# abusch/rustracer

Hardware: AMD Instinct MI355X
Metric: Msamples/s (higher is better)
Workload: dtype f32; 1 GPU; cornell-box (synthetic S1, 32 triangles, 2 area lights) 1024x1024 PathIntegrator maxdepth=5 1024spp 02sequence box-filter; sampler_mode=pixel-keyed, light_distribution=cached across frames; first-frame build 18.3 ms

## Files before the change

include/rtx_hip.h:

```cpp
#ifndef RTX_HIP_H
#define RTX_HIP_H

#include <stdint.h>

#ifdef __cplusplus
extern "C" {
#endif

#define RT_OK 0
#define RT_ERR_INVALID (-1)
#define RT_ERR_NO_DEVICE (-2)
#define RT_ERR_HIP (-3)
#define RT_ERR_OOM (-4)
#define RT_ERR_UNSUPPORTED (-5)

typedef struct rt_bvh_node {
  float bmin[3];
  float bmax[3];
  uint32_t offset;
  uint16_t n_prims;
  uint8_t axis;
  uint8_t pad;
} rt_bvh_node;

// ... 98 lines not shown
  uint32_t n_materials; const rt_material* materials;
  uint32_t n_lights; const rt_light* lights;
  uint32_t n_instances; const rt_instance* instances;
  uint32_t n_top_nodes, n_top_prims;
  uint32_t n_unlisted_lights;
} rt_scene_desc;

typedef struct rt_camera {
  float raster_to_camera[16];
  float camera_to_world[16];
  float dx_camera[3], dy_camera[3];
  float lens_radius, focal_distance;
} rt_camera;
typedef struct rt_film_desc {
  int32_t cropped_pixel_bounds[4];
  int32_t sample_bounds[4];
  float filter_radius[2];
  float filter_table[256];
  float max_sample_luminance;
} rt_film_desc;
typedef struct rt_sampler_desc {
  int32_t spp;
  int32_t dimensions;
} rt_sampler_desc;
typedef struct rt_path_desc {
  int32_t max_depth;
  float rr_threshold;
  int32_t light_strategy;
  int32_t pixel_bounds[4];
} rt_path_desc;
typedef struct rt_shard { int32_t rank, world_size; } rt_shard;
#define RT_SHARD_ROWS(H, world_size) ((world_size) > 1 ? 4 : 16)

typedef struct rt_stats {
  uint64_t camera_rays;
  uint64_t rays_closest, rays_shadow, rays_mis;
  uint64_t nodes_closest, nodes_shadow, nodes_mis;
  uint64_t tris_closest, tris_shadow, tris_mis;
  uint64_t paths_scrubbed;
  double ms_total;
  double ms_sampler, ms_raygen, ms_trace_closest, ms_trace_any, ms_trace_mis, ms_shade, ms_resolve, ms_film, ms_lightdist;
  uint64_t launches_trace_closest;
  uint64_t n_passes;
  uint64_t vertices_lambert_const, vertices_lambert, vertices_two_lobe, vertices_generic;
  double ms_shade_lambert_const, ms_shade_lambert, ms_shade_two_lobe, ms_shade_generic, ms_shade_bin, ms_shade_miss;
  uint64_t shade_section_cycles[32];
  uint64_t rays_mis_any, nodes_mis_any, tris_mis_any;
  double ms_trace_mis_any;
  double ms_gather;
  uint64_t rays_mis_not_cast;
  uint64_t rays_tail_not_cast;
  uint64_t launches_trace_path, launches_trace_shadow, launches_trace_mis, launches_trace_mis_any, launches_shade;
  uint64_t rays_shadow_not_cast;
} rt_stats;

#define RT_FLAG_COUNT_TRAVERSAL 1u
#define RT_FLAG_FILM_ON_DEVICE 2u
#define RT_FLAG_TIME_KERNELS 4u
#define RT_FLAG_COUNT_AS_RENDERED 8u
#define RT_FLAG_REF_STREAM 16u
#define RT_FLAG_FRAME_STATS 32u

typedef struct rt_scene rt_scene;

int rt_scene_create(const rt_scene_desc* desc, int device, rt_scene** out);
void rt_scene_destroy(rt_scene* scene);

int rt_bvh_build(const float* tri_p, uint32_t n_tris, int32_t max_prims_per_node, rt_bvh_node* nodes, uint32_t* n_nodes, int32_t* ordered,
                 float* ms_device );

int rt_mip_build(const float* rgb, int32_t width, int32_t height, int32_t px, int32_t py, const int32_t* s_first, const float* s_wts, const int32_t* t_first,
                 const float* t_wts, int32_t wrap, int32_t n_levels, const int32_t* lvl_w, const int32_t* lvl_h, const uint64_t* lvl_off, float* texels_out);
int rt_env_distribution(const rt_image* image, int32_t width, int32_t height, int32_t mode, int32_t il, float delta, const float* sin_theta,
                        float* func, float* cdf, float* func_int, float* marg_cdf, float* marg_func_int);

int rt_render(rt_scene* scene, const rt_camera* camera, const rt_film_desc* film, const rt_sampler_desc* sampler,
              const rt_path_desc* path, const rt_shard* shard, uint32_t flags, void* stream, float* film_xyzw, rt_stats* stats);

typedef struct rt_multi rt_multi;
int rt_multi_create(const rt_scene_desc* desc, const int32_t* devices, int32_t n_devices, rt_multi** out);
void rt_multi_destroy(rt_multi* multi);
int rt_multi_render(rt_multi* multi, const rt_camera* camera, const rt_film_desc* film, const rt_sampler_desc* sampler, const rt_path_desc* path,
                    int32_t chunks_per_device, uint32_t flags, float* film_xyzw, rt_stats* total, rt_stats* per_device);

int rt_trace_closest(rt_scene* scene, const float* rays, uint64_t n, float* hits, uint64_t counters[2]);
int rt_trace_any(rt_scene* scene, const float* rays, uint64_t n, uint32_t* occluded, uint64_t counters[2]);
int rt_trace_closest_device(rt_scene* scene, const void* d_rays, uint64_t n, void* d_hits, int reps, void* stream, float* ms_per_launch);

int rt_sampler_tables(int32_t spp, int32_t dimensions, uint64_t pixel0, uint64_t n_pixels, uint32_t* scrambles, uint16_t* perms);
int rt_sampler_tables_plain(int32_t spp, int32_t dimensions, uint64_t pixel0, uint64_t n_pixels, uint32_t* scrambles, uint16_t* perms);

int rt_offset_ray_origin(const float* p, const float* p_error, const float* n, const float* w, uint64_t count, float* out);

int rt_fourier_eval(rt_scene* scene, int32_t material, uint64_t n, const float* wo, const float* wi, const float* u, float* out);

int rt_texture_eval(rt_scene* scene, int32_t texture, uint64_t n, const float* records, float* rgb_out);

enum { RT_BSDF_FRONT_AUTO = 0, RT_BSDF_FRONT_GENERIC = 1, RT_BSDF_FRONT_LAMBERT = 2, RT_BSDF_FRONT_TWO_LOBE = 3, RT_BSDF_FRONT_TWO_LOBE_WIDE = 4 };
#define RT_BSDF_SURFACE_FLOATS 40
#define RT_BSDF_OUT_FLOATS 13
int rt_bsdf_eval(rt_scene* scene, int32_t material, int32_t front_end, uint64_t n, const float* surface, const float* wo, const float* wi, const float* u,
                 float* out);

#define RT_SAMPLES_MAX 134217728
int rt_render_samples(rt_scene* scene, const rt_camera* camera, const rt_film_desc* film, const rt_sampler_desc* sampler, const rt_path_desc* path,
                      uint32_t flags, void* stream, float* radiance, float* p_film, rt_stats* stats);

enum { RT_FRAME_XYZW = 0, RT_FRAME_RGB = 1, RT_FRAME_RGB8 = 2, RT_FRAME_STATS = 3 };
enum { RT_FRAME_SAMPLES_DONE = 0, RT_FRAME_SPP = 1, RT_FRAME_TABLES_RESIDENT = 2, RT_FRAME_STATE_BYTES = 3, RT_FRAME_SAMPLES_TAKEN = 4, RT_FRAME_ACTIVE_PIXELS = 5 };
typedef struct rt_frame rt_frame;
int rt_frame_begin(rt_scene* scene, const rt_camera* camera, const rt_film_desc* film, const rt_sampler_desc* sampler, const rt_path_desc* path,
                   const rt_shard* shard , uint32_t flags, uint64_t table_budget_bytes, rt_frame** out);
int rt_frame_advance(rt_frame* frame, int32_t n_samples, void* stream, rt_stats* stats );
int rt_frame_advance_adaptive(rt_frame* frame, int32_t n_samples, float threshold, float floor_y, int32_t min_samples, void* stream, rt_stats* stats );
int rt_frame_read(rt_frame* frame, int32_t what, float scale, uint32_t flags, void* stream, void* out);
int rt_frame_query(rt_frame* frame, int32_t what, uint64_t* value);
void rt_frame_end(rt_frame* frame);

typedef struct rt_multi_frame rt_multi_frame;
int rt_multi_frame_begin(rt_multi* multi, const rt_camera* camera, const rt_film_desc* film, const rt_sampler_desc* sampler, const rt_path_desc* path,
                         uint32_t flags, uint64_t table_budget_bytes, rt_multi_frame** out);
int rt_multi_frame_advance(rt_multi_frame* frame, int32_t n_samples, rt_stats* total , rt_stats* per_device );
int rt_multi_frame_advance_adaptive(rt_multi_frame* frame, int32_t n_samples, float threshold, float floor_y, int32_t min_samples, rt_stats* total, rt_stats* per_device);
int rt_multi_frame_read(rt_multi_frame* frame, int32_t what, float scale, uint32_t flags, void* out);
int rt_multi_frame_query(rt_multi_frame* frame, int32_t what, uint64_t* value);
void rt_multi_frame_end(rt_multi_frame* frame);

int rt_light_distribution(rt_scene* scene, int32_t n_voxels[3], float* func, float* cdf, float* func_int);

enum { RT_QUERY_LDS_RESIDENT = 0, RT_QUERY_LDS_NODES_TESTED = 1 ,
       RT_QUERY_LDS_OCCLUSION = 2 ,
       RT_QUERY_SHADOW_PAIRS = 3 ,
       RT_QUERY_SHADOW_EMPTY = 4 ,
       RT_QUERY_BSDF_LAUNCHED = 5  };
int rt_scene_query(rt_scene* scene, int32_t what);
int rt_link_tables(const rt_scene_desc* desc, int32_t mid, uint32_t* link_kept, uint32_t* link_full, uint64_t capacity_words, double* stats);
int rt_shadow_sets(const rt_scene_desc* desc, uint32_t* words, uint64_t capacity_words, int32_t n_voxels[3], uint64_t* stats);
int rt_sizeof(const char* struct_name);

const char* rt_last_error(void);
int rt_device_available(void);
const char* rt_version(void);

#ifdef __cplusplus
}
#endif
#endif
```

include/rtx_host.h:

```cpp
#ifndef RTX_HOST_H
#define RTX_HOST_H
#include <stdint.h>
#include "rtx_hip.h"

#ifdef __cplusplus
extern "C" {
#endif

typedef struct rtxh_scene rtxh_scene;

typedef struct rtxh_render_params {
  int32_t xres, yres;
  float crop[4];
  int32_t filter_kind;
  float filter_params[4];
  float film_scale, max_sample_luminance;
  float cam_to_world[16], cam_to_world_inv[16];
  float fov, lens_radius, focal_distance;
  int32_t spp, sampler_dims;
  int32_t max_depth; float rr_threshold; int32_t light_strategy;
  int32_t pixel_bounds[4];
  int32_t rank, world_size;
  uint32_t flags;
  float screen_window[4];
// ... 25 lines not shown
int rtxh_scene_add_texture_mapped(rtxh_scene*, int32_t kind, const float* value3, int32_t tex1, int32_t tex2, int32_t amount, const float* words, int32_t n_words);
int rtxh_texture_words(rtxh_scene*, int32_t texture, float* out, int32_t capacity);
int rtxh_scene_add_material(rtxh_scene*, int32_t kind, const int32_t* slots16, int32_t remap_roughness, int32_t bump_texture );
int rtxh_scene_add_light(rtxh_scene*, int32_t kind, int32_t tri, const float* rgb3, int32_t two_sided, const float* vec3, int32_t mip,
                         const float* l2w16, const float* w2l16);
int rtxh_scene_commit(rtxh_scene*, int32_t max_prims_per_node);
int rtxh_scene_commit_device_bvh(rtxh_scene*, int32_t max_prims_per_node, float* ms_device);
int rtxh_scene_upload(rtxh_scene*, int32_t device);

int rtxh_scene_bvh_sizes(rtxh_scene*, int32_t* n_nodes, int32_t* n_prims);
int rtxh_scene_bvh_get(rtxh_scene*, float* bounds6, uint32_t* offset, uint16_t* n_prims, uint8_t* axis, int32_t* ordered);
int rtxh_camera_film_setup(const rtxh_render_params*, float* raster_to_camera16, float* dxdy6, float* filter_table256, int32_t* sample_bounds4,
                           int32_t* cropped4);
int rtxh_mip_level(rtxh_scene*, int32_t mip, int32_t level, int32_t* w, int32_t* h, float* rgb_out );
enum { RTXH_TABLE_TEXTURES = 0, RTXH_TABLE_MATERIALS, RTXH_TABLE_LIGHTS, RTXH_TABLE_P, RTXH_TABLE_N, RTXH_TABLE_UV, RTXH_TABLE_S, RTXH_TABLE_INDICES,
       RTXH_TABLE_TRI_MATERIAL, RTXH_TABLE_TRI_LIGHT, RTXH_TABLE_TRI_FLAGS,
       RTXH_TABLE_ENV_FUNC, RTXH_TABLE_ENV_CDF, RTXH_TABLE_ENV_ROW_INT, RTXH_TABLE_ENV_MARG_CDF,
       RTXH_TABLE_INSTANCES,
       RTXH_TABLE_EMITTERS,
       RTXH_TABLE_QUADRICS,
       RTXH_TABLE_OBJECT_BASE = 1000 ,
       RTXH_TABLE_OBJECT_EXTRA_BASE = 100000  };
typedef struct rtxh_emitter_info { float rgb[3]; int32_t two_sided; } rtxh_emitter_info;
typedef struct rtxh_instance_info { int32_t object; float o2w[16], w2o[16]; } rtxh_instance_info;
typedef struct rtxh_light_info { int32_t kind, tri; float rgb[3]; int32_t two_sided; float vec[3]; int32_t mip; float l2w[12], w2l[12]; } rtxh_light_info;
int rtxh_scene_inspect(rtxh_scene*, int32_t table, void* out, uint64_t capacity_bytes, uint64_t* n_items);
int rtxh_look_at(const float* pos, const float* look, const float* up, float* m16, float* m_inv16);

int rtxh_render(rtxh_scene*, const rtxh_render_params*, void* hip_stream, float* film_xyzw, rt_stats* stats);
int rtxh_render_samples(rtxh_scene*, const rtxh_render_params*, void* hip_stream, float* radiance, float* p_film, rt_stats* stats);
typedef struct rtxh_frame rtxh_frame;
int rtxh_frame_begin(rtxh_scene*, const rtxh_render_params*, uint64_t table_budget_bytes, rtxh_frame** out);
int rtxh_frame_advance(rtxh_frame*, int32_t n_samples, void* hip_stream, rt_stats* stats );
int rtxh_frame_advance_adaptive(rtxh_frame*, int32_t n_samples, float threshold, float floor_y, int32_t min_samples, void* hip_stream, rt_stats* stats );
int rtxh_frame_read(rtxh_frame*, int32_t what, float scale, uint32_t flags, void* hip_stream, void* out);
int rtxh_frame_query(rtxh_frame*, int32_t what, uint64_t* value);
void rtxh_frame_end(rtxh_frame*);
int rtxh_render_multi(rtxh_scene*, const rtxh_render_params*, const int32_t* devices, int32_t n_devices, int32_t chunks_per_device, float* film_xyzw,
                      rt_stats* total, rt_stats* per_device );
typedef struct rtxh_multi_frame rtxh_multi_frame;
int rtxh_multi_frame_begin(rtxh_scene*, const rtxh_render_params*, const int32_t* devices, int32_t n_devices, uint64_t table_budget_bytes, rtxh_multi_frame** out);
int rtxh_multi_frame_advance(rtxh_multi_frame*, int32_t n_samples, rt_stats* total, rt_stats* per_device);
int rtxh_multi_frame_advance_adaptive(rtxh_multi_frame*, int32_t n_samples, float threshold, float floor_y, int32_t min_samples, rt_stats* total, rt_stats* per_device);
int rtxh_multi_frame_read(rtxh_multi_frame*, int32_t what, float scale, uint32_t flags, void* out);
int rtxh_multi_frame_query(rtxh_multi_frame*, int32_t what, uint64_t* value);
void rtxh_multi_frame_end(rtxh_multi_frame*);
int rtxh_trace(rtxh_scene*, const float* rays, uint64_t n, int32_t any_hit, float* hits4_or_occ, uint64_t counters[2]);
int rtxh_trace_device(rtxh_scene*, const void* d_rays, uint64_t n, void* d_hits, int32_t reps, void* hip_stream, float* ms_per_launch);
int rtxh_light_distribution(rtxh_scene*, int32_t n_voxels[3], float* func, float* cdf, float* func_int);
int rtxh_scene_query(rtxh_scene*, int32_t what);
int rtxh_scene_device(rtxh_scene*, rt_scene** out);
int rtxh_scene_link_tables(rtxh_scene*, int32_t mid, uint32_t* link_kept, uint32_t* link_full, uint64_t capacity_words, double* stats);
int rtxh_scene_shadow_sets(rtxh_scene*, uint32_t* words, uint64_t capacity_words, int32_t n_voxels[3], uint64_t* stats);
int rtxh_sizeof(const char* struct_name);
const char* rtxh_last_error(void);

typedef struct rtxh_ply {
  int32_t n_verts, n_tris;
  float* P;
  float* N;
  float* UV;
  int32_t* idx;
  int32_t n_dropped_faces;
} rtxh_ply;
int rtxh_ply_read(const char* path, rtxh_ply* out);
void rtxh_ply_free(rtxh_ply* ply);
int rtxh_pfm_read(const char* path, int32_t* width, int32_t* height, float** rgb);
void rtxh_free(void* p);
int rtxh_image_read(const char* path, int32_t* width, int32_t* height, float** rgb);

int rtxh_spectrum_from_sampled(const float* lambda_nm, const float* values, int32_t n, float rgb[3]);
int rtxh_spectrum_blackbody(float temperature_kelvin, float scale, float rgb[3]);
void rtxh_copper(float eta_rgb[3], float k_rgb[3]);

typedef struct rtxh_pbrt_result {
  rtxh_scene* scene;
  rtxh_render_params params;
  int32_t max_prims_per_node;
  int32_t n_warnings;
  char film_filename[512];
} rtxh_pbrt_result;
int rtxh_pbrt_load(const char* path, rtxh_pbrt_result* out);
int rtxh_pbrt_parse(const char* text, const char* base_dir, rtxh_pbrt_result* out);
int rtxh_pbrt_tokens(const char* text, char* out, uint64_t capacity);

#ifdef __cplusplus
}
#endif
#endif
```

rustracer_amd/csrc/rtx_hip.hip:

```cpp
#include <hip/hip_runtime.h>
#include <chrono>
#include <cmath>
#include <cstdio>
#include <cstring>
#include <string>
#include <vector>
#include <limits>
#include <algorithm>
#include <memory>
#include <atomic>
#include <mutex>
#include <thread>

#include "../../include/rtx_hip.h"
#include "rtx_kernels.h"
#include "rtx_shade_launch.h"
#include "rtx_ref_launch.h"

using namespace rtx;
#include "rtx_scene_plan.h"

static thread_local std::string g_err;
static int fail(int code, const std::string& msg) { g_err = msg; return code; }
static bool env_is(const char* name, char c) { const char* e = getenv(name); return e && e[0] == c; }
// ... 10 lines not shown
  hipError_t ensure(size_t n) {
    if (n <= bytes && p) return hipSuccess;
    if (p) { (void)hipFree(p); p = nullptr; bytes = 0; }
    hipError_t e = hipMalloc(&p, n > 0 ? n : 16);
    if (e == hipSuccess) bytes = n;
    return e;
  }
  void release() { if (p) (void)hipFree(p); p = nullptr; bytes = 0; }
  template <class T> T* as() const { return (T*)p; }
};

struct SamplerPlan {
  unsigned spp = 0, dims = 0, seg_len = 0, n_segs = 0;
  DevBuf segs, magic, dirty, partners;
};

struct rt_scene {
  int device = 0;
  SamplerPlan sampler_plan;
  DScene d{};
  bool small = false;
  bool lambert_materials = false;
  bool lds_records_q = false;
  bool lds_tables = false;
  bool lds_mats = false;
  bool lds_records = false;
  bool lambert_only = false;
  bool lean_qlights = false;
  bool lean_shade = false;
  int stack_depth = 64;
  unsigned n_nodes = 0, n_tris = 0; int n_lights = 0;
  DevBuf link8, link8_full; unsigned lds_nodes_tested = 0;
  DevBuf pairs, tmin_stack;
  DevBuf top_pairs, deep_stack; bool use_top = false;
  bool top_for_closest = false;
  bool use_pairs = false;
  bool deep_column = false;
  DevBuf quads; bool use_quads = false; int quad_stack_depth = 0;
  DevBuf tri_rec;
  DevBuf nodes, tri_p, tri_n, tri_uv, tri_s, tri_alpha, spheres, textures, images, materials, lights, texels, dist, guides, prim_class;
  DevBuf fourier;
  std::vector<int> mat_kind, mat_table;
  std::vector<uint64_t> fourier_at;
  bool has_spheres = false;
  bool has_instances = false;
  DevBuf instances;
  bool mid = false;
  bool general_prims = false;
  bool obj_general = false;
  bool has_masks = false;
  bool masked_emitters = false;
  DevBuf ld_func, ld_cdf, ld_int, ld_mark, ld_list, ld_slot, ld_guide, ld_rows8, ld_dense8;
  bool shadow_sets = false; RtShadowSets shadow; DevBuf ld_shadow;
  DevBuf self;
  int ld_strategy_built = -1; bool ld_all_voxels = false;
  std::mutex render_mutex;
  DevBuf ws[32];
  DevBuf film_acc, own_acc, film_out, counters, stats, filter_table, ref_samples, ref_stack;
  DevBuf samples_rad, samples_pf;
  DevBuf bsdf_self, bsdf_tris;
  int bsdf_launched = -1;
  std::vector<int> mat_class;
  DevBuf bin_words, bin_sorted, bin_at;
  unsigned n_materials = 0, n_code_classes = 0, n_lambert_classes = 0, n_small_classes = 0, n_wide_classes = 0;
  DevBuf scrambles[2], perms[2];
  hipStream_t aux_stream = nullptr;
  hipEvent_t ev_tables[2][3] = {{nullptr, nullptr, nullptr}, {nullptr, nullptr, nullptr}}, ev_batch_done[2] = {nullptr, nullptr}, ev_frame_begin = nullptr;
  int n_cu = 256;
  std::vector<hipEvent_t> event_pool;
  ~rt_scene() {
    for (hipEvent_t e : event_pool) (void)hipEventDestroy(e);
    for (int i = 0; i < 2; ++i) { for (int g = 0; g < 3; ++g) if (ev_tables[i][g]) (void)hipEventDestroy(ev_tables[i][g]); if (ev_batch_done[i]) (void)hipEventDestroy(ev_batch_done[i]); }
    if (ev_frame_begin) (void)hipEventDestroy(ev_frame_begin);
    if (aux_stream) (void)hipStreamDestroy(aux_stream);
  }
};

extern "C" const char* rt_last_error(void) { return g_err.c_str(); }
extern "C" const char* rt_version(void) { return "rtx-mi355x 0.5 (gfx950 wavefront path tracer)"; }
extern "C" int rt_sizeof(const char* name) {
  if (!name) return -1;
#define RT_SZ(T) if (!strcmp(name, #T)) return (int)sizeof(T);
  RT_SZ(rt_bvh_node) RT_SZ(rt_tri_meta) RT_SZ(rt_sphere) RT_SZ(rt_instance) RT_SZ(rt_texture) RT_SZ(rt_image) RT_SZ(rt_material) RT_SZ(rt_light) RT_SZ(rt_scene_desc)
  RT_SZ(rt_camera) RT_SZ(rt_film_desc) RT_SZ(rt_sampler_desc) RT_SZ(rt_path_desc) RT_SZ(rt_shard) RT_SZ(rt_stats)
#undef RT_SZ
  return -1;
}
extern "C" int rt_device_available(void) {
  int n = 0;
  if (hipGetDeviceCount(&n) != hipSuccess || n <= 0) return 0;
  return 1;
}

static int upload(DevBuf& b, const void* src, size_t bytes) {
  HIP_TRY(b.ensure(bytes));
  if (bytes) HIP_TRY(hipMemcpy(b.p, src, bytes, hipMemcpyHostToDevice));
  return RT_OK;
}

static void fill_ewa_lut() {
  float lut[128];
  for (int i = 0; i < 128; ++i) {
    float alpha = 2.0f;
    float r2 = (float)i / (128.0f - 1.0f);
    lut[i] = expf(-alpha * r2) - expf(-alpha);
  }
// ... 150 lines not shown
  scene->bsdf_launched = 2 * mode + (const_tex ? 1 : 0);
  HIP_TRY(hipMemcpy(out, b[3].p, no, hipMemcpyDeviceToHost));
  return RT_OK;
}
extern "C" int rt_link_tables(const rt_scene_desc* desc, int32_t mid, uint32_t* link_kept, uint32_t* link_full, uint64_t capacity_words, double* stats) {
  if (!desc || !desc->nodes || desc->n_nodes == 0 || !desc->tri_p || !desc->tri_meta || !link_kept || !link_full) return fail(RT_ERR_INVALID, "null argument");
  const size_t words = (size_t)9 * desc->n_nodes + 9;
  if (desc->n_nodes > (mid ? RT_MID_NODES : RT_SMALL_NODES) || desc->n_tris > (uint64_t)(mid ? RT_MID_TRIS : RT_SMALL_TRIS) || desc->n_instances != 0) return fail(RT_ERR_INVALID, "not an LDS-sized scene");
  if (capacity_words < words) return fail(RT_ERR_INVALID, "link table capacity too small");
  {
    const uint32_t nn = desc->n_nodes;
    std::vector<uint32_t> size(nn, 1u);
    for (uint32_t i = nn; i-- > 0;) {
      const rt_bvh_node& n = desc->nodes[i];
      if (n.n_prims != 0) {
        if ((uint64_t)n.offset + n.n_prims > desc->n_tris) return fail(RT_ERR_INVALID, "leaf range out of bounds");
        if (n.n_prims >= (1u << (15 - RT_LINK_OFF_BITS(mid ? RT_MID_NODES : RT_SMALL_NODES)))) return fail(RT_ERR_INVALID, "a leaf holds more primitives than a link word can name");
        continue;
      }
      if (i + 1 >= nn || n.offset != i + 1 + size[i + 1] || n.offset >= nn) return fail(RT_ERR_INVALID, "nodes are not a pre-order tree");
      size[i] = 1u + size[i + 1] + size[n.offset];
    }
    if (size[0] != nn) return fail(RT_ERR_INVALID, "nodes are not one tree");
    for (uint64_t t = 0; t < desc->n_tris; ++t)
      if (desc->tri_meta[t].flags & RT_PRIM_SPHERE) {
        uint32_t k; memcpy(&k, desc->tri_p + 9 * t + 6, 4);
        if (!desc->spheres || k >= desc->n_spheres) return fail(RT_ERR_INVALID, "sphere index out of range");
      }
  }
  RtLinkTables lt;
  rt_build_link_tables(desc, mid != 0, stats != nullptr, lt);
  memcpy(link_kept, lt.link_kept.data(), words * 4); memcpy(link_full, lt.link_full.data(), words * 4);
  if (stats) for (int w = 0; w < 9; ++w) { stats[w] = (double)lt.n_rays[w]; stats[9 + w] = lt.tests_all[w]; stats[18 + w] = lt.tests_kept[w]; }
  return RT_OK;
}
extern "C" int rt_shadow_sets(const rt_scene_desc* desc, uint32_t* words, uint64_t capacity_words, int32_t n_voxels[3], uint64_t* stats) {
  if (!desc || !desc->nodes || desc->n_nodes == 0 || !desc->tri_p || !desc->tri_meta) return fail(RT_ERR_INVALID, "null argument");
  bool plain = desc->n_instances == 0 && desc->n_spheres == 0 && desc->n_nodes <= RT_SMALL_NODES && desc->n_tris <= RT_SMALL_TRIS;
  for (uint32_t i = 0; i < desc->n_tris && plain; ++i) if (desc->tri_meta[i].flags & ~(uint32_t)RT_SHADOW_PLAIN_FLAGS) plain = false;
  if (!shadow_sets_apply(desc, plain)) return fail(RT_ERR_INVALID, "not a scene the shadow sets serve (LDS-resident plain triangles, two triangle lights)");
  int32_t lp[2] = {0, 0};
  for (uint32_t k = 0; k < desc->n_lights; ++k) lp[k] = desc->lights[k].prim;
  RtShadowSets ss;
  rt_build_shadow_sets(desc->tri_p, desc->n_tris, lp, (int)desc->n_lights, desc->nodes[0].bmin, desc->nodes[0].bmax, ss);
  if (n_voxels) { n_voxels[0] = ss.nvox[0]; n_voxels[1] = ss.nvox[1]; n_voxels[2] = ss.nvox[2]; }
  if (stats) { stats[0] = ss.pairs; stats[1] = ss.empty; }
  if (words) {
    if (capacity_words < ss.word.size()) return fail(RT_ERR_INVALID, "rt_shadow_sets: capacity too small");
    std::memcpy(words, ss.word.data(), ss.word.size() * 4);
  }
  return RT_OK;
}

extern "C" int rt_scene_query(rt_scene* s, int32_t what) {
  if (!s) return fail(RT_ERR_INVALID, "null scene");
  if (what == RT_QUERY_LDS_RESIDENT) return s->small ? 1 : 0;
  if (what == RT_QUERY_LDS_NODES_TESTED) return (s->small || s->mid) ? (int)s->lds_nodes_tested : 0;
  if (what == RT_QUERY_LDS_OCCLUSION) return s->mid ? 1 : 0;
  if (what == RT_QUERY_SHADOW_PAIRS) return s->shadow_sets ? (int)s->shadow.pairs : 0;
  if (what == RT_QUERY_SHADOW_EMPTY) return s->shadow_sets ? (int)s->shadow.empty : 0;
  if (what == RT_QUERY_BSDF_LAUNCHED) return s->bsdf_launched < 0 ? 0 : s->bsdf_launched + 1;
  return fail(RT_ERR_INVALID, "unknown rt_scene_query item");
}

static int build_light_distribution(rt_scene* s, int strategy, hipStream_t stream, bool all_voxels = false) {
  DScene& d = s->d;
  if (s->ld_strategy_built == strategy && (s->ld_all_voxels || !all_voxels)) return RT_OK;
  s->ld_strategy_built = -1;
  const int nl = s->n_lights;
  size_t ld_rows_built = 1;
  const bool uniform = strategy == 1 || nl == 1 || nl == 0;
  int glog = -1;
  if (nl >= 64 && nl <= 65534) { const long q = guide_quarters(); glog = 0; while (glog < 16 && (long)(2 << glog) * q <= 4l * nl) ++glog; }
  d.ld_glog = glog; d.ld_guide = nullptr;
  if (uniform) {
    const int n = nl > 0 ? nl : 1;
    std::vector<float> func(n, 1.0f), cdf(n + 1, 0.0f);
    for (int i = 1; i < n + 1; ++i) cdf[i] = cdf[i - 1] + func[i - 1] / (float)n;
    float func_int = cdf[n];
    if (func_int == 0.0f) for (int i = 1; i < n + 1; ++i) cdf[i] = (float)i / (float)n;
    else for (int i = 1; i < n + 1; ++i) cdf[i] /= func_int;
    int rc;
    if ((rc = upload(s->ld_func, func.data(), func.size() * 4)) != RT_OK) return rc;
    if ((rc = upload(s->ld_cdf, cdf.data(), cdf.size() * 4)) != RT_OK) return rc;
    if ((rc = upload(s->ld_int, &func_int, 4)) != RT_OK) return rc;
    if (glog >= 0) {
      const int G = 1 << glog; std::vector<unsigned short> g((size_t)G + 1); int i = 0;
      for (int k = 0; k <= G; ++k) { const float x = (float)k / (float)G; while (i <= n && cdf[i] <= x) ++i; g[k] = (unsigned short)i; }
      if ((rc = upload(s->ld_guide, g.data(), g.size() * 2)) != RT_OK) return rc;
    }
    d.ld_uniform = 1; d.nvox[0] = d.nvox[1] = d.nvox[2] = 1;
  } else {
    float diag[3] = {d.wb_max.x - d.wb_min.x, d.wb_max.y - d.wb_min.y, d.wb_max.z - d.wb_min.z};
    int ext = diag[0] > diag[1] ? (diag[0] > diag[2] ? 0 : 2) : (diag[1] > diag[2] ? 1 : 2);
    float b_max = diag[ext];
    size_t total = 1;
    for (int i = 0; i < 3; ++i) {
      float r = roundf(diag[i] / b_max * 64.0f);
      unsigned v = (r != r || r <= 0.0f) ? 0u : (unsigned)r;
      d.nvox[i] = (int)(v > 1u ? v : 1u);
      total *= (size_t)d.nvox[i];
    }
    d.ld_uniform = 0;
    HIP_TRY(s->ld_mark.ensure(total)); HIP_TRY(s->ld_list.ensure((total + 1) * 4)); HIP_TRY(s->ld_slot.ensure(total * 4));
    unsigned* n_list = s->ld_list.as<unsigned>(); unsigned* list = n_list + 1;
    HIP_TRY(hipMemsetAsync(s->ld_slot.p, 0xff, total * 4, stream));
    if (all_voxels) hipLaunchKernelGGL(k_lightdist_iota, dim3((unsigned)((total + 255) / 256)), dim3(256), 0, stream, (unsigned)total, list, n_list);
    else {
      HIP_TRY(hipMemsetAsync(s->ld_mark.p, 0, total, stream)); HIP_TRY(hipMemsetAsync(n_list, 0, 4, stream));
      hipLaunchKernelGGL(k_lightdist_mark, dim3((s->n_tris + 255u) / 256u), dim3(256), 0, stream, d, s->ld_mark.as<unsigned char>());
      hipLaunchKernelGGL(k_lightdist_compact, dim3((unsigned)((total + 255) / 256)), dim3(256), 0, stream, s->ld_mark.as<unsigned char>(), (unsigned)total, 0, list, n_list);
    }
    unsigned n_built = 0;
    HIP_TRY(hipMemcpyAsync(&n_built, n_list, 4, hipMemcpyDeviceToHost, stream)); HIP_TRY(hipStreamSynchronize(stream));
    const size_t rows = std::max<size_t>(n_built, 1);
    ld_rows_built = rows;
    if (s->ld_func.ensure(rows * nl * 4) != hipSuccess || s->ld_cdf.ensure(rows * (nl + 1) * 4) != hipSuccess || s->ld_int.ensure(rows * 4) != hipSuccess)
      return fail(RT_ERR_OOM, "light distribution tables do not fit (built voxels x lights)");
    if (glog >= 0 && s->ld_guide.ensure(rows * (((size_t)1 << glog) + 1) * 2) != hipSuccess) return fail(RT_ERR_OOM, "light distribution guide tables do not fit");
    d.ld_func = s->ld_func.as<float>(); d.ld_cdf = s->ld_cdf.as<float>(); d.ld_int = s->ld_int.as<float>(); d.ld_slot = s->ld_slot.as<int>();
    unsigned lights_pad = 1; while (lights_pad < (unsigned)nl) lights_pad <<= 1;
    const unsigned long long contrib_blocks = lights_pad <= 128u ? (rows + 128u / lights_pad - 1) / (128u / lights_pad) : (unsigned long long)rows * (unsigned)((nl + 127) / 128);
    if (contrib_blocks > 0x7fffffffull) return fail(RT_ERR_INVALID, "light distribution grid too large");
    if (s->has_spheres) hipLaunchKernelGGL(k_lightdist_contrib<true>, dim3((unsigned)contrib_blocks), dim3(128), 0, stream, d, list, n_list, lights_pad, (unsigned)((nl + 127) / 128), s->ld_func.as<float>());
    else hipLaunchKernelGGL(k_lightdist_contrib<false>, dim3((unsigned)contrib_blocks), dim3(128), 0, stream, d, list, n_list, lights_pad, (unsigned)((nl + 127) / 128), s->ld_func.as<float>());
    hipLaunchKernelGGL(k_lightdist_finish, dim3((unsigned)((rows + 127) / 128)), dim3(128), 0, stream, d, list, n_list, s->ld_func.as<float>(), s->ld_cdf.as<float>(), s->ld_int.as<float>(), s->ld_slot.as<int>(),
                       glog >= 0 ? s->ld_guide.as<unsigned short>() : nullptr, glog);
    HIP_TRY(hipGetLastError());
  }
  d.ld_func = s->ld_func.as<float>(); d.ld_cdf = s->ld_cdf.as<float>(); d.ld_int = s->ld_int.as<float>(); d.ld_slot = s->ld_slot.as<int>();
  d.ld_guide = glog >= 0 ? s->ld_guide.as<unsigned short>() : nullptr;
  d.ld_rows8 = nullptr; d.ld_dense8 = nullptr;
  if (nl >= 1 && nl <= 3 && !(env_is("RTX_LD_ROWS8", '0'))) {
    const size_t n_rows = ld_rows_built;
    HIP_TRY(s->ld_rows8.ensure(n_rows * 32));
    hipLaunchKernelGGL(k_lightdist_rows8, dim3((unsigned)((n_rows + 255) / 256)), dim3(256), 0, stream, s->ld_func.as<float>(), s->ld_cdf.as<float>(), s->ld_int.as<float>(), (int)nl, (unsigned)n_rows, s->ld_rows8.as<float4>());
    HIP_TRY(hipGetLastError());
    d.ld_rows8 = s->ld_rows8.as<float4>();
    const unsigned long long n_vox = (unsigned long long)d.nvox[0] * d.nvox[1] * d.nvox[2];
    const int dense_mb = env_int("RTX_LD_DENSE_MB", 16);
    if (!uniform && n_vox * 32ull <= (unsigned long long)dense_mb << 20) {
      HIP_TRY(s->ld_dense8.ensure((size_t)n_vox * 32));
      hipLaunchKernelGGL(k_lightdist_dense8, dim3((unsigned)((n_vox + 255) / 256)), dim3(256), 0, stream, s->ld_rows8.as<float4>(), s->ld_slot.as<int>(), n_vox, s->ld_dense8.as<float4>());
      HIP_TRY(hipGetLastError());
      d.ld_dense8 = s->ld_dense8.as<float4>();
    }
  }
  if (d.ld_rows8 != nullptr && !uniform && s->shadow_sets && nl == 2 && d.nvox[0] == s->shadow.nvox[0] && d.nvox[1] == s->shadow.nvox[1] && d.nvox[2] == s->shadow.nvox[2]) {
    const unsigned long long n_vox = (unsigned long long)d.nvox[0] * d.nvox[1] * d.nvox[2];
    int rc = upload(s->ld_shadow, s->shadow.word.data(), s->shadow.word.size() * 4);
    if (rc != RT_OK) return rc;
    hipLaunchKernelGGL(k_lightdist_shadow_words, dim3((unsigned)((n_vox + 255) / 256)), dim3(256), 0, stream, s->ld_shadow.as<unsigned>(), s->ld_slot.as<int>(), n_vox, s->ld_rows8.as<float4>(),
                       d.ld_dense8 != nullptr ? s->ld_dense8.as<float4>() : nullptr);
    HIP_TRY(hipGetLastError());
  }
  s->ld_strategy_built = strategy; s->ld_all_voxels = all_voxels;
  HIP_TRY(hipMemcpyAsync(s->self.p, &s->d, sizeof(DScene), hipMemcpyHostToDevice, stream));
  return RT_OK;
}

extern "C" int rt_light_distribution(rt_scene* s, int32_t n_voxels[3], float* func, float* cdf, float* func_int) {
  if (!s) return fail(RT_ERR_INVALID, "null scene");
  HIP_TRY(hipSetDevice(s->device));
  int rc = build_light_distribution(s, 0, nullptr, true);
  if (rc != RT_OK) return rc;
  HIP_TRY(hipDeviceSynchronize());
  if (s->d.ld_uniform) { n_voxels[0] = n_voxels[1] = n_voxels[2] = 0; return RT_OK; }
  n_voxels[0] = s->d.nvox[0]; n_voxels[1] = s->d.nvox[1]; n_voxels[2] = s->d.nvox[2];
  size_t total = (size_t)s->d.nvox[0] * s->d.nvox[1] * s->d.nvox[2];
  if (func) HIP_TRY(hipMemcpy(func, s->ld_func.p, total * s->n_lights * 4, hipMemcpyDeviceToHost));
  if (cdf) HIP_TRY(hipMemcpy(cdf, s->ld_cdf.p, total * (s->n_lights + 1) * 4, hipMemcpyDeviceToHost));
  if (func_int) HIP_TRY(hipMemcpy(func_int, s->ld_int.p, total * 4, hipMemcpyDeviceToHost));
  return RT_OK;
}

template <bool ANY, bool SMALL, int BLOCK, int DEPTH>
static unsigned trace_grid(const rt_scene* s, bool links = false) {
  unsigned lds = (unsigned)(DEPTH * BLOCK * (SMALL ? 2 : 4) + (SMALL ? (8 * RT_SMALL_NODES + 10 * RT_SMALL_TRIS) * 4 : 32));
  unsigned waves = 8;
  if (SMALL && links) { lds = (unsigned)((8 * RT_SMALL_NODES + 10 * RT_SMALL_TRIS) * 4 + (ANY ? 1 : 8) * RT_SMALL_NODES * 4 + 32); waves = ANY ? RT_LDS_ANY_WAVES : RT_LDS_TRACE_WAVES; }
  unsigned per_cu = (160u * 1024u) / lds; if (per_cu * BLOCK > waves * 256u) per_cu = waves * 256u / BLOCK; if (per_cu < 1) per_cu = 1;
  return (unsigned)s->n_cu * per_cu;
}
#define RT_TOP_BLOCK 512
static unsigned top_grid(const rt_scene* s, bool any = false) {
  (void)any;
  const unsigned fit = (160u * 1024u) / (16384u + (unsigned)RT_TOP_LDS_DEPTH * RT_TOP_BLOCK * 4u);
  return (unsigned)s->n_cu * std::max(1u, std::min(3u, fit));
}
static size_t tmin_stack_bytes(const rt_scene* s) {
  if (s->small || !s->use_pairs) return 0;
  const size_t a = s->stack_depth <= 32 ? (size_t)trace_grid<false, false, 128, 32>(s) * 128 * 32 * 4 : (size_t)trace_grid<false, false, 128, 64>(s) * 128 * 64 * 4;
  const size_t b = s->use_top ? (size_t)std::max(top_grid(s), top_grid(s, true)) * RT_TOP_BLOCK * (size_t)s->stack_depth * 4 : 0;
  return std::max(a, b);
}
static size_t deep_stack_bytes(const rt_scene* s) {
  if (!s->use_top) return 0;
  return (size_t)std::max(top_grid(s), top_grid(s, true)) * RT_TOP_BLOCK * (size_t)std::max(1, s->stack_depth - RT_TOP_LDS_DEPTH) * 4;
}
static int scene_from_plan(const RtScenePlan& p, const rt_scene_desc* desc, int device, rt_scene** out) {
  if (device >= 0) HIP_TRY(hipSetDevice(device));
  int dev = 0; HIP_TRY(hipGetDevice(&dev));
  std::unique_ptr<rt_scene> owner(new rt_scene());
  rt_scene* s = owner.get();
  s->device = dev;
  hipDeviceProp_t prop; if (hipGetDeviceProperties(&prop, dev) == hipSuccess) s->n_cu = prop.multiProcessorCount;
  s->n_nodes = desc->n_nodes; s->n_tris = desc->n_tris; s->n_lights = (int)desc->n_lights; s->n_materials = desc->n_materials;
  s->small = p.small; s->mid = p.mid; s->general_prims = p.general_prims; s->obj_general = p.obj_general; s->has_masks = p.has_masks; s->has_spheres = p.has_spheres;
  s->has_instances = p.has_instances; s->masked_emitters = p.masked_emitters; s->lambert_only = p.lambert_only; s->lambert_materials = p.lambert_materials;
  s->lean_shade = p.lean_shade; s->lean_qlights = p.lean_qlights; s->lds_records = p.lds_records; s->lds_records_q = p.lds_records_q; s->lds_tables = p.lds_tables;
  s->lds_mats = p.lds_mats; s->use_pairs = p.use_pairs; s->use_top = p.use_top; s->top_for_closest = p.top_for_closest; s->use_quads = p.use_quads;
  s->deep_column = p.deep_column; s->shadow_sets = p.shadow_sets; s->shadow = p.shadow; s->stack_depth = p.stack_depth; s->quad_stack_depth = p.quad_stack_depth;
  s->mat_kind = p.mat_kind; s->mat_table = p.mat_table; s->mat_class = p.mat_class; s->fourier_at = p.fourier_at;
  s->n_code_classes = p.n_code_classes; s->n_lambert_classes = p.n_lambert_classes; s->n_small_classes = p.n_small_classes; s->n_wide_classes = p.n_wide_classes;
  if (s->mid) {
    int fit_any = 0, fit_closest = 0;
    if (hipOccupancyMaxActiveBlocksPerMultiprocessor(&fit_any, (const void*)(k_trace<true, false, 1024, 16, 0, 1>), 1024, 0) != hipSuccess) fit_any = 0;
    if (hipOccupancyMaxActiveBlocksPerMultiprocessor(&fit_closest, (const void*)(k_trace<false, false, 1024, 16, 0, 1>), 1024, 0) != hipSuccess) fit_closest = 0;
    (void)hipGetLastError();
    if (fit_any < 1 || fit_closest < 1) s->mid = false;
  }
  const bool links = s->small || s->mid;
  if (links) s->lds_nodes_tested = p.links.nodes_tested;
  int rc = RT_OK;
  auto up = [&rc](DevBuf& b, const void* src, size_t bytes) { if (rc == RT_OK) rc = upload(b, src, bytes); };
  auto up_all = [&up](DevBuf& b, const auto& v) { up(b, v.data(), v.size() * sizeof(v[0])); };
  auto room = [&rc](DevBuf& b, size_t bytes, const char* what) { if (rc == RT_OK && bytes && b.ensure(bytes) != hipSuccess) rc = fail(RT_ERR_OOM, what); };
  up(s->nodes, desc->nodes, sizeof(rt_bvh_node) * (size_t)desc->n_nodes);
  up_all(s->tri_p, p.tri_p);
  if (desc->tri_n) up(s->tri_n, desc->tri_n, (size_t)desc->n_tris * 36);
  if (desc->tri_uv) up(s->tri_uv, desc->tri_uv, (size_t)desc->n_tris * 24);
  if (desc->tri_s) up(s->tri_s, desc->tri_s, (size_t)desc->n_tris * 36);
  if (p.has_masks) up(s->tri_alpha, desc->tri_alpha, (size_t)desc->n_tris * 8);
  if (p.has_spheres) up(s->spheres, desc->spheres, (size_t)desc->n_spheres * sizeof(rt_sphere));
  if (p.has_instances) up_all(s->instances, p.instances);
  up_all(s->texels, p.texels); up_all(s->fourier, p.fourier);
  std::vector<DImage> images = p.images;
  for (DImage& im : images) im.texels = s->texels.as<float4>();
  up_all(s->images, images); up_all(s->textures, p.textures); up_all(s->materials, p.materials); up_all(s->prim_class, p.prim_class);
  up_all(s->dist, p.dist); up_all(s->guides, p.guides);
  std::vector<DLight> lights = p.lights;
  for (DLight& l : lights)
    if (l.kind == RT_LIGHT_INFINITE) {
      rt_blob_rebase(l.cf, s->dist.p); rt_blob_rebase(l.func_int, s->dist.p); rt_blob_rebase(l.mfunc, s->dist.p); rt_blob_rebase(l.mcdf, s->dist.p);
      rt_blob_rebase(l.guide, s->guides.p); rt_blob_rebase(l.mguide, s->guides.p);
    }
  up_all(s->lights, lights);
  if (links) { up_all(s->link8_full, p.links.link_full); up_all(s->link8, p.links.link_kept); }
  if (p.use_pairs) up_all(s->pairs, p.pairs);
  if (p.use_top) up_all(s->top_pairs, p.top_pairs);
  if (p.use_quads) up_all(s->quads, p.quads);
  room(s->tmin_stack, tmin_stack_bytes(s), "traversal stack allocation failed");
  room(s->deep_stack, deep_stack_bytes(s), "traversal stack allocation failed");
  room(s->tri_rec, (size_t)desc->n_tris * 128, "shade record allocation failed");
  room(s->self, sizeof(DScene), "scene record allocation failed");
  if (rc != RT_OK) return rc;
  DScene& d = s->d;
  d.nodes = s->nodes.as<float4>(); d.n_nodes = desc->n_nodes;
  d.tri_p = s->tri_p.as<float4>(); d.n_tris = desc->n_tris;
  d.tri_n = s->tri_n.as<float>(); d.tri_uv = s->tri_uv.as<float>(); d.tri_s = s->tri_s.as<float>();
  d.tri_alpha = s->tri_alpha.as<int2>();
  d.spheres = s->spheres.as<DSphere>();
  d.instances = s->instances.as<DInstance>(); d.n_instances = s->has_instances ? desc->n_instances : 0u; d.n_top_prims = p.n_top_prims;
  d.textures = s->textures.as<DTexture>(); d.images = s->images.as<DImage>(); d.materials = s->materials.as<DMaterial>(); d.lights = s->lights.as<DLight>();
  d.fourier = s->fourier.as<unsigned>();
// ... 128 lines not shown
  }
  if (s->small) {
    if (s->stack_depth <= 16) hipLaunchKernelGGL((k_trace<ANY, true, 256, 16>), dim3(trace_grid<ANY, true, 256, 16>(s)), dim3(256), 0, stream, RT_KARGS, st_nodes, st_tris);
    else if (s->stack_depth <= 32) hipLaunchKernelGGL((k_trace<ANY, true, 256, 32>), dim3(trace_grid<ANY, true, 256, 32>(s)), dim3(256), 0, stream, RT_KARGS, st_nodes, st_tris);
    else hipLaunchKernelGGL((k_trace<ANY, true, 128, 64>), dim3(trace_grid<ANY, true, 128, 64>(s)), dim3(128), 0, stream, RT_KARGS, st_nodes, st_tris);
  } else {
    if (s->stack_depth <= 32) launch_trace_hbm<ANY, COUNT, 128, 32>(RT_ARGS);
    else launch_trace_hbm<ANY, COUNT, 128, 64>(RT_ARGS);
  }
#undef RT_KARGS
#undef RT_ARGS
}
template <bool ANY>
static void launch_trace(rt_scene* s, bool count, const TraceIO& io, const unsigned* queue, const unsigned* count_ptr, unsigned shard_cap, unsigned count_static,
                         unsigned long long* stats, int st_rays, int st_nodes, int st_tris, hipStream_t stream) {
  if (count) launch_trace_c<ANY, true>(s, io, queue, count_ptr, shard_cap, count_static, stats, st_rays, st_nodes, st_tris, stream);
  else launch_trace_c<ANY, false>(s, io, queue, count_ptr, shard_cap, count_static, stats, st_rays, st_nodes, st_tris, stream);
}
static TraceIO trace_io_planar(const float4* ro, const float4* rd, float4* hits, unsigned* occ) {
  TraceIO io{}; io.ray_o = ro; io.ray_d = rd; io.ray_stride = 1; io.hits = hits; io.hit_stride = 1; io.hit_b2 = 0; io.occluded = occ; io.occ_stride = 1;
  io.shadow_masks = 1;
  return io;
}

static int trace_batch(rt_scene* s, const float* rays, uint64_t n, bool any, float* hits, uint32_t* occluded, uint64_t counters[2]) {
  if (!s || !rays || n == 0 || n > 0x7fffffffull) return fail(RT_ERR_INVALID, "bad trace batch");
  HIP_TRY(hipSetDevice(s->device));
  DevBuf ro, rd, out, st;
  HIP_TRY(ro.ensure(n * 16)); HIP_TRY(rd.ensure(n * 16)); HIP_TRY(out.ensure(n * 16)); HIP_TRY(st.ensure(ST_COUNT * 8));
  std::vector<float> o(n * 4), d(n * 4);
  for (uint64_t i = 0; i < n; ++i) {
    const float* r = rays + 8 * i;
    o[4 * i] = r[0]; o[4 * i + 1] = r[1]; o[4 * i + 2] = r[2]; o[4 * i + 3] = r[3];
    d[4 * i] = r[4]; d[4 * i + 1] = r[5]; d[4 * i + 2] = r[6]; d[4 * i + 3] = 0.0f;
  }
  HIP_TRY(hipMemcpy(ro.p, o.data(), n * 16, hipMemcpyHostToDevice));
  HIP_TRY(hipMemcpy(rd.p, d.data(), n * 16, hipMemcpyHostToDevice));
  HIP_TRY(hipMemset(st.p, 0, ST_COUNT * 8));
  const TraceIO io = trace_io_planar(ro.as<float4>(), rd.as<float4>(), any ? nullptr : out.as<float4>(), any ? out.as<unsigned>() : nullptr);
  if (any) launch_trace<true>(s, counters != nullptr, io, nullptr, nullptr, 0, (unsigned)n, st.as<unsigned long long>(), ST_RAYS_SHADOW, ST_NODES_SHADOW, ST_TRIS_SHADOW, nullptr);
  else launch_trace<false>(s, counters != nullptr, io, nullptr, nullptr, 0, (unsigned)n, st.as<unsigned long long>(), ST_RAYS_CLOSEST, ST_NODES_CLOSEST, ST_TRIS_CLOSEST, nullptr);
  HIP_TRY(hipGetLastError());
  HIP_TRY(hipDeviceSynchronize());
  if (any) HIP_TRY(hipMemcpy(occluded, out.p, n * 4, hipMemcpyDeviceToHost));
  else HIP_TRY(hipMemcpy(hits, out.p, n * 16, hipMemcpyDeviceToHost));
  if (counters) {
    unsigned long long h[ST_COUNT];
    HIP_TRY(hipMemcpy(h, st.p, sizeof(h), hipMemcpyDeviceToHost));
    counters[0] = any ? h[ST_NODES_SHADOW] : h[ST_NODES_CLOSEST];
    counters[1] = any ? h[ST_TRIS_SHADOW] : h[ST_TRIS_CLOSEST];
  }
  return RT_OK;
}
extern "C" int rt_trace_closest(rt_scene* s, const float* rays, uint64_t n, float* hits, uint64_t counters[2]) { return trace_batch(s, rays, n, false, hits, nullptr, counters); }
extern "C" int rt_trace_any(rt_scene* s, const float* rays, uint64_t n, uint32_t* occluded, uint64_t counters[2]) { return trace_batch(s, rays, n, true, nullptr, occluded, counters); }

extern "C" int rt_trace_closest_device(rt_scene* s, const void* d_rays, uint64_t n, void* d_hits, int reps, void* stream_, float* ms_per_launch) {
  if (!s || !d_rays || !d_hits || n == 0 || reps <= 0) return fail(RT_ERR_INVALID, "bad arguments");
  HIP_TRY(hipSetDevice(s->device));
  hipStream_t stream = (hipStream_t)stream_;
  const float4* ro = (const float4*)d_rays; const float4* rd = ro + n;
  hipEvent_t e0, e1; HIP_TRY(hipEventCreate(&e0)); HIP_TRY(hipEventCreate(&e1));
  HIP_TRY(hipEventRecord(e0, stream));
  const TraceIO io = trace_io_planar(ro, rd, (float4*)d_hits, nullptr);
  for (int i = 0; i < reps; ++i) launch_trace<false>(s, false, io, nullptr, nullptr, 0, (unsigned)n, nullptr, 0, 0, 0, stream);
  HIP_TRY(hipEventRecord(e1, stream));
  HIP_TRY(hipEventSynchronize(e1));
  float ms = 0; HIP_TRY(hipEventElapsedTime(&ms, e0, e1));
  if (ms_per_launch) *ms_per_launch = ms / (float)reps;
  (void)hipEventDestroy(e0); (void)hipEventDestroy(e1);
  return RT_OK;
}

static unsigned next_pow2(unsigned v) { unsigned p = 1; while (p < v) p <<= 1; return p; }
static unsigned sampler_lanes_per_block(unsigned spp) {
  unsigned l = (32u * 1024u) / ((spp + 2u) * 2u);
  if (l >= 64u) return 64u;
  if (l >= 32u) return 32u;
  if (l >= 16u) return 16u;
  if (l >= 8u) return 8u;
  return 4u;
}

static void pcg_advance_constants(unsigned long long n, unsigned long long& mul, unsigned long long& sum) {
  unsigned long long cur_mul = 0x5851f42d4c957f2dULL, cur_sum = 1ull;
  mul = 1ull; sum = 0ull;
  while (n) {
    if (n & 1ull) { sum = sum * cur_mul + cur_sum; mul *= cur_mul; }
    cur_sum = (cur_mul + 1ull) * cur_sum; cur_mul *= cur_mul;
    n >>= 1;
  }
}
static int sampler_plan_prepare(SamplerPlan& pl, unsigned spp_, unsigned dims_) {
  unsigned &spp = pl.spp, &dims = pl.dims, &seg_len = pl.seg_len, &n_segs = pl.n_segs;
  DevBuf &segs = pl.segs, &magic = pl.magic, &dirty = pl.dirty;
  {
    if (spp == spp_ && dims == dims_ && segs.p) return RT_OK;
    seg_len = spp_ < 256u ? spp_ : 256u;
    const unsigned per_half = spp_ / seg_len;
    std::vector<SamplerSeg> h;
    unsigned long long pos = 0;
    for (unsigned t = 0; t < 2u * dims_; ++t) {
      const unsigned n_scr = t < dims_ ? 1u : 2u;
      for (unsigned half = 0; half < 2u; ++half)
        for (unsigned g = 0; g < per_half; ++g) {
          SamplerSeg sg{};
// ... 303 lines not shown
      else { want.push_back({&s->samples_rad, (size_t)n_window_samples * 16}); if (samples_pf) want.push_back({&s->samples_pf, (size_t)n_window_samples * 8}); }
    }
    size_t grow = 0;
    for (const Want& w : want) if (!w.buf->p || w.buf->bytes < w.bytes) grow += w.bytes;
    size_t held = 0;
    for (const Want& w : want) if (w.buf->p && w.buf->bytes < w.bytes) held += w.buf->bytes;
    size_t mem_free = 0, mem_total = 0;
    HIP_TRY(hipMemGetInfo(&mem_free, &mem_total));
    if (grow > mem_free + held - std::min<size_t>(mem_free + held, (size_t)256 << 20)) continue;
    bool ok = true;
    for (const Want& w : want) if (w.buf->ensure(w.bytes) != hipSuccess) { ok = false; break; }
    if (ok) break;
    (void)hipGetLastError();
  }
  if (!s->aux_stream) {
    int lo = 0, hi = 0; (void)hipDeviceGetStreamPriorityRange(&lo, &hi);
    HIP_TRY(hipStreamCreateWithPriority(&s->aux_stream, hipStreamNonBlocking, lo));
    for (int i = 0; i < 2; ++i) { for (int g = 0; g < 3; ++g) HIP_TRY(hipEventCreateWithFlags(&s->ev_tables[i][g], hipEventDisableTiming)); HIP_TRY(hipEventCreateWithFlags(&s->ev_batch_done[i], hipEventDisableTiming)); }
    HIP_TRY(hipEventCreateWithFlags(&s->ev_frame_begin, hipEventDisableTiming));
  }
  float4* const d_out = (flags & RT_FLAG_FILM_ON_DEVICE) ? (float4*)film_xyzw : s->film_out.as<float4>();
  float4* const d_samples_rad = (flags & RT_FLAG_FILM_ON_DEVICE) ? (float4*)samples_rad : s->samples_rad.as<float4>();
  float2* const d_samples_pf = !samples_pf ? nullptr : ((flags & RT_FLAG_FILM_ON_DEVICE) ? (float2*)samples_pf : s->samples_pf.as<float2>());
  if (!samples && !fr) {
    HIP_TRY(hipMemcpyAsync(s->filter_table.p, film->filter_table, 1024, hipMemcpyHostToDevice, stream));
    HIP_TRY(hipMemsetAsync(s->film_acc.p, 0, (size_t)cw * ch * 16, stream));
  }
  HIP_TRY(hipMemsetAsync(s->stats.p, 0, ST_COUNT * 8, stream));

  PassState ps{};
  ps.spp = spp; ps.spp_log2 = spp_log2; ps.dims = dims;
  auto gen_of = [&](int b) { PathGen g; char* p = (char*)s->ws[b].p; g.o = (float4*)p; g.d = (float4*)(p + n_slots * 16); g.beta = (float4*)(p + n_slots * 32); g.st = (uint4*)(p + n_slots * 48); return g; };
  const PathGen gen0 = gen_of(B_GEN0), gen1 = gen_of(B_GEN1);
  ps.hit = s->ws[B_HIT].as<float4>(); ps.lacc = s->ws[B_LACC].as<float4>(); ps.pfilm = s->ws[B_PFILM].as<float2>();
  { char* p = (char*)s->ws[B_SH].p; ps.sh.o = (float4*)p; ps.sh.d = (float4*)(p + cap * 16); ps.sh.add = (float4*)(p + cap * 32);
    char* q = (char*)s->ws[B_MI].p; ps.mi.o = (float4*)q; ps.mi.d = (float4*)(q + cap * 16); ps.mi.hit = (float4*)(q + cap * 32); ps.mi.a = (float4*)(q + cap * 48);
    ps.mi.b = (float4*)(q + cap * 64); ps.mi.c = (float4*)(q + cap * 80); ps.mi.flags = (unsigned*)(q + cap * 96); }
  ps.occ_sh = s->ws[B_OCCSH].as<unsigned char>(); ps.occ_mi = s->ws[B_OCCMI].as<unsigned char>();
  ps.q_shadow = s->ws[B_QSH].as<unsigned>(); ps.q_mis = s->ws[B_QMI].as<unsigned>(); ps.q_misany = s->ws[B_QMA].as<unsigned>();
  ps.own_acc = s->own_acc.as<float4>(); ps.shard_cap = shard_cap;
  ps.stats = s->stats.as<unsigned long long>();

  if ((rc = sampler_plan_prepare(s->sampler_plan, spp, dims)) != RT_OK) return rc;
  if ((rc = sampler_set_lds_limits(spp)) != RT_OK) return rc;
  TraceIO io_path{}, io_shadow{}, io_mis{}, io_mis_any{};
  {
    io_path.ray_stride = 1; io_path.hits = ps.hit; io_path.hit_stride = 1; io_path.hit_b2 = 1; io_path.queue_is_slots = 1;
    io_shadow.ray_o = ps.sh.o; io_shadow.ray_d = ps.sh.d; io_shadow.ray_stride = 1; io_shadow.occluded = (unsigned*)ps.occ_sh; io_shadow.occ_stride = 0;
    io_shadow.shadow_masks = 1; io_shadow.lacc = ps.lacc; io_shadow.lacc_stride = 1; io_shadow.direct_add = ps.sh.add; io_shadow.add_stride = 1;
    io_mis.ray_o = ps.mi.o; io_mis.ray_d = ps.mi.d; io_mis.ray_stride = 1; io_mis.hits = ps.mi.hit; io_mis.hit_stride = 1; io_mis.hit_b2 = 0;
    io_mis_any = io_mis; io_mis_any.shadow_masks = 0; io_mis_any.hits = nullptr; io_mis_any.occluded = (unsigned*)ps.occ_mi; io_mis_any.occ_stride = 0;
  }
  const bool count = (flags & RT_FLAG_COUNT_TRAVERSAL) != 0;
  const unsigned pgrid = (unsigned)s->n_cu * 8u;
  const unsigned sblock = 256u, sgrid = pgrid;
  unsigned long long* dstats = s->stats.as<unsigned long long>();

  const char* ov = getenv("RTX_K0_OVERLAP");
  hipStream_t aux = (ov && ov[0] == '0') ? stream : s->aux_stream;
  if (build_tables) {
    HIP_TRY(hipEventRecord(s->ev_frame_begin, stream));
    HIP_TRY(hipStreamWaitEvent(aux, s->ev_frame_begin, 0));
  }
  int tables_rc = RT_OK;
  std::vector<std::pair<unsigned long long, unsigned long long>> batches;
  for (unsigned long long first = 0; first < owned_pixels;) {
    const unsigned long long npx = (first == 0 && lead_pixels) ? lead_pixels : std::min(chunk_pixels, owned_pixels - first);
    batches.push_back({first, npx}); first += npx;
  }
  if (resident && !fr->tables_built) {
    fr->scr_off.clear(); fr->perm_off.clear();
    size_t so = 0, po = 0;
    for (const auto& b : batches) {
      fr->scr_off.push_back(so); fr->perm_off.push_back(po);
      so += ((size_t)b.second * 3 * dims * 4 + 255) & ~(size_t)255; po += ((size_t)(b.second * table_bytes_per_pixel) + 255) & ~(size_t)255;
    }
    if (so > fr->scrambles.bytes || po > fr->perms.bytes) return fail(RT_ERR_INVALID, "rt_frame_advance: the batches' sampler tables do not fit the frame's buffers");
  }
  if (resident && fr->scr_off.size() != batches.size()) return fail(RT_ERR_INVALID, "rt_frame_advance: the batch cut changed under resident sampler tables");
  auto scrambles_of = [&](size_t b, int buf) { return resident ? (unsigned*)((char*)fr->scrambles.p + fr->scr_off[b]) : s->scrambles[buf].as<unsigned>(); };
  auto perms_of = [&](size_t b, int buf) { return resident ? (unsigned short*)((char*)fr->perms.p + fr->perm_off[b]) : s->perms[buf].as<unsigned short>(); };
  TableGroups tgroups = table_groups_frame(dims, !(fp.lens_radius > 0.0f));
  auto launch_tables = [&](size_t b, int buf) {
    FrameParams f2 = fp; f2.chunk_first = batches[b].first;
    tm.begin(&stats.ms_sampler, aux);
    const int trc = launch_sampler_tables(s->sampler_plan, f2, (unsigned)batches[b].second, 0ull, 0, scrambles_of(b, buf), perms_of(b, buf), aux, tgroups, s->ev_tables[buf]);
    if (trc != RT_OK && tables_rc == RT_OK) tables_rc = trc;
    tm.end(aux);
  };
  if (!batches.empty() && build_tables) launch_tables(0, 0);
  for (size_t batch_no = 0; batch_no < batches.size(); ++batch_no) {
    const unsigned long long first = batches[batch_no].first, npx = batches[batch_no].second;
    const int buf = (int)(batch_no & 1ull);
    fp.chunk_first = first;
    ps.n_pixels = (unsigned)npx; ps.n_pixels_recip = npx > 1 ? (unsigned)((1ull << 32) / npx) : 0xffffffffu;
    ps.scrambles = scrambles_of(batch_no, buf); ps.perms = perms_of(batch_no, buf);
    if (build_tables && batch_no + 1 < batches.size()) {
      if (batch_no >= 1 && !resident) HIP_TRY(hipStreamWaitEvent(aux, s->ev_batch_done[buf ^ 1], 0));
      launch_tables(batch_no + 1, buf ^ 1);
    }
    const unsigned batch_pass_samples = (unsigned)std::min<unsigned long long>(spp, std::max<unsigned long long>(pass_samples, cap / npx));
    if (tables_rc != RT_OK) { (void)hipDeviceSynchronize(); return tables_rc; }
    if (build_tables) HIP_TRY(hipStreamWaitEvent(stream, s->ev_tables[buf][0], 0));
    for (unsigned s0 = s_begin; s0 < s_end; s0 += batch_pass_samples) {
      ps.s0 = s0; ps.n_samples = std::min(batch_pass_samples, s_end - s0); ps.cap = (unsigned)(npx * ps.n_samples);
      ps.q_in = nullptr; ps.in = gen1; ps.out = gen0;
// ... 56 lines not shown
        tm.end();
        tm.begin(&stats.ms_trace_mis);
        launch_trace<false>(s, count, io_mis, ps.q_mis, ps.cnt_out + 2 * RT_QSHARDS * RT_CNT_STRIDE, ps.shard_cap, 0, dstats, ST_RAYS_MIS, ST_NODES_MIS, ST_TRIS_MIS, stream);
        tm.end();
        if (ps.mis_any) {
          tm.begin(&stats.ms_trace_mis_any);
          launch_trace<true>(s, count, io_mis_any, ps.q_misany, ps.cnt_out + 3 * RT_QSHARDS * RT_CNT_STRIDE, ps.shard_cap, 0, dstats, ST_RAYS_MISANY, ST_NODES_MISANY, ST_TRIS_MISANY, stream);
          tm.end();
        }
        tm.begin(&stats.ms_resolve);
        if (s->has_spheres || s->has_instances) hipLaunchKernelGGL(k_resolve<true>, dim3(pgrid), dim3(256), 0, stream, s->d, ps);
        else hipLaunchKernelGGL(k_resolve<false>, dim3(pgrid), dim3(256), 0, stream, s->d, ps);
        tm.end();
        stats.launches_trace_closest += 2; stats.launches_trace_path += 1; stats.launches_trace_mis += 1; stats.launches_trace_shadow += 1; stats.launches_trace_mis_any += ps.mis_any ? 1 : 0;
      }
      tm.begin(&stats.ms_film);
      if (samples) hipLaunchKernelGGL(k_sample_store, dim3(pgrid), dim3(256), 0, stream, fp, ps, wx0, wy0, wx1 - wx0, d_samples_rad, d_samples_pf);
      else if (fr && fr->stats) hipLaunchKernelGGL(k_film_accumulate_frame_stats, dim3(pgrid), dim3(256), 0, stream, fp, ps, fr->filter_table.as<float>(), fr->film_acc.as<float4>(), fr->own_acc.as<float4>(), fr->moments.as<PixMoments>());
      else if (fr) hipLaunchKernelGGL(k_film_accumulate_frame, dim3(pgrid), dim3(256), 0, stream, fp, ps, fr->filter_table.as<float>(), fr->film_acc.as<float4>(), fr->own_acc.as<float4>());
      else hipLaunchKernelGGL(k_film_accumulate, dim3(pgrid), dim3(256), 0, stream, fp, ps, s->filter_table.as<float>(), s->film_acc.as<float4>());
      tm.end();
      stats.n_passes += 1;
      HIP_TRY(hipGetLastError());
    }
    HIP_TRY(hipEventRecord(s->ev_batch_done[buf], stream));
  }
  if (fr) {
    if (resident && build_tables) {
      HIP_TRY(hipStreamSynchronize(aux));
      fr->tables_built = true; fr->batch_pixels = batch_pixels; fr->lead_pixels = lead_pixels;
    }
  } else if (!samples) {
    tm.begin(&stats.ms_film);
    {
      unsigned long long n = (unsigned long long)cw * ch;
      hipLaunchKernelGGL(k_film_finalize, dim3((unsigned)((n + 255) / 256)), dim3(256), 0, stream, s->film_acc.as<float4>(), d_out, n);
    }
    tm.end();
    HIP_TRY(hipGetLastError());
    if (!(flags & RT_FLAG_FILM_ON_DEVICE)) HIP_TRY(hipMemcpyAsync(film_xyzw, d_out, (size_t)cw * ch * 16, hipMemcpyDeviceToHost, stream));
  } else if (!(flags & RT_FLAG_FILM_ON_DEVICE)) {
    HIP_TRY(hipMemcpyAsync(samples_rad, d_samples_rad, (size_t)n_window_samples * 16, hipMemcpyDeviceToHost, stream));
    if (samples_pf) HIP_TRY(hipMemcpyAsync(samples_pf, d_samples_pf, (size_t)n_window_samples * 8, hipMemcpyDeviceToHost, stream));
  }
  HIP_TRY(hipStreamSynchronize(stream));
  tm.collect();
  stats.ms_shade = stats.ms_shade_lambert_const + stats.ms_shade_lambert + stats.ms_shade_two_lobe + stats.ms_shade_generic + stats.ms_shade_bin + stats.ms_shade_miss;
  unsigned long long h[ST_COUNT];
  HIP_TRY(hipMemcpy(h, s->stats.p, sizeof(h), hipMemcpyDeviceToHost));
  { unsigned ovf = 0; HIP_TRY(hipMemcpy(&ovf, s->sampler_plan.dirty.as<unsigned>() + 1 + RT_DIRTY_CAP, 4, hipMemcpyDeviceToHost));
    if (ovf) { (void)hipMemset(s->sampler_plan.dirty.p, 0, (2 + RT_DIRTY_CAP) * 4); return fail(RT_ERR_INVALID, "sampler retry list overflow"); } }
  stats.camera_rays = h[ST_CAMERA];
  stats.rays_mis_any = h[ST_RAYS_MISANY]; stats.nodes_mis_any = h[ST_NODES_MISANY]; stats.tris_mis_any = h[ST_TRIS_MISANY];
  stats.rays_closest = h[ST_RAYS_CLOSEST] + h[ST_TAIL_UNCAST]; stats.rays_tail_not_cast = h[ST_TAIL_UNCAST]; stats.rays_shadow = h[ST_RAYS_SHADOW] + h[ST_SHADOW_SETS]; stats.rays_shadow_not_cast = h[ST_SHADOW_SETS]; stats.rays_mis = h[ST_RAYS_MIS] + h[ST_RAYS_MISANY] + h[ST_MIS_UNREACHED];
  stats.rays_mis_not_cast = h[ST_MIS_UNREACHED];
  stats.nodes_closest = h[ST_NODES_CLOSEST]; stats.nodes_shadow = h[ST_NODES_SHADOW]; stats.nodes_mis = h[ST_NODES_MIS] + h[ST_NODES_MISANY];
  stats.tris_closest = h[ST_TRIS_CLOSEST]; stats.tris_shadow = h[ST_TRIS_SHADOW]; stats.tris_mis = h[ST_TRIS_MIS] + h[ST_TRIS_MISANY];
  stats.ms_trace_mis += stats.ms_trace_mis_any;
  stats.paths_scrubbed = h[ST_SCRUBBED];
  for (int k = 0; k < 32; ++k) stats.shade_section_cycles[k] = h[ST_STAMP + k];
  stats.vertices_lambert_const = h[ST_SHADED]; stats.vertices_lambert = h[ST_SHADED + 1]; stats.vertices_two_lobe = h[ST_SHADED + 2]; stats.vertices_generic = h[ST_SHADED + 3];
  if (h[ST_UNBUILT_VOXEL]) return fail(RT_ERR_INVALID, "a path looked up a light-distribution voxel that holds no surface (voxel marking bug)");
  stats.ms_total = std::chrono::duration<double, std::milli>(std::chrono::steady_clock::now() - t_begin).count();
  if (stats_out) *stats_out = stats;
  return RT_OK;
}
extern "C" int rt_render(rt_scene* s, const rt_camera* cam, const rt_film_desc* film, const rt_sampler_desc* smp, const rt_path_desc* path,
                         const rt_shard* shard, uint32_t flags, void* stream_, float* film_xyzw, rt_stats* stats_out) {
  if (!s || !cam || !film || !smp || !path || !film_xyzw) return fail(RT_ERR_INVALID, "null argument");
  return render_frame(s, cam, film, smp, path, shard, flags, stream_, film_xyzw, stats_out, nullptr, nullptr);
}
extern "C" int rt_render_samples(rt_scene* s, const rt_camera* cam, const rt_film_desc* film, const rt_sampler_desc* smp, const rt_path_desc* path,
                                 uint32_t flags, void* stream_, float* radiance, float* p_film, rt_stats* stats_out) {
  if (!s || !cam || !film || !smp || !path || !radiance) return fail(RT_ERR_INVALID, "rt_render_samples: null argument");
  return render_frame(s, cam, film, smp, path, nullptr, flags, stream_, nullptr, stats_out, radiance, p_film);
}

extern "C" int rt_frame_begin(rt_scene* s, const rt_camera* cam, const rt_film_desc* film, const rt_sampler_desc* smp, const rt_path_desc* path, const rt_shard* shard,
                              uint32_t flags, uint64_t table_budget_bytes, rt_frame** out) {
  if (!out) return fail(RT_ERR_INVALID, "rt_frame_begin: NULL out");
  *out = nullptr;
  if (!s || !cam || !film || !smp || !path) return fail(RT_ERR_INVALID, "rt_frame_begin: null argument");
  if (flags & RT_FLAG_REF_STREAM) return fail(RT_ERR_INVALID, "rt_frame_begin: the reference-stream frame cannot be rendered in steps");
  const unsigned long long spp_r = next_pow2((unsigned)(smp->spp > 0 ? smp->spp : 1));
  if (smp->spp > 16384 || spp_r > 16384ull) return fail(RT_ERR_INVALID, "rt_frame_begin: spp > 16384 unsupported");
  const unsigned dims = (unsigned)smp->dimensions;
  if (smp->dimensions < 2 || smp->dimensions > 8) return fail(RT_ERR_INVALID, "rt_frame_begin: sampler dimensions must be in [2, 8]");
  const int rank = shard ? shard->rank : 0, world = shard ? shard->world_size : 1;
  if (world < 1 || rank < 0 || rank >= world) return fail(RT_ERR_INVALID, "rt_frame_begin: bad shard");
  const int W = film->sample_bounds[2] - film->sample_bounds[0], H = film->sample_bounds[3] - film->sample_bounds[1];
  const int cw = film->cropped_pixel_bounds[2] - film->cropped_pixel_bounds[0], ch = film->cropped_pixel_bounds[3] - film->cropped_pixel_bounds[1];
  if (W <= 0 || H <= 0 || cw <= 0 || ch <= 0) return fail(RT_ERR_INVALID, "rt_frame_begin: empty film");
  if (film->filter_radius[0] > 8.0f || film->filter_radius[1] > 8.0f) return fail(RT_ERR_INVALID, "rt_frame_begin: filter radius > 8");

  std::unique_ptr<rt_frame> fr(new rt_frame());
  fr->scene = s; fr->cam = *cam; fr->film = *film; fr->smp = *smp; fr->path = *path; fr->shard = rt_shard{rank, world}; fr->flags = flags;
  fr->spp = (unsigned)spp_r;
  const int band = RT_SHARD_ROWS(H, world);
  for (int row = 0; row < H; ++row) if (((row / band) % world) == rank) fr->owned_pixels += (unsigned long long)W;
  std::lock_guard<std::mutex> render_lock(s->render_mutex);
  HIP_TRY(hipSetDevice(s->device));
  int rc = build_light_distribution(s, path->light_strategy, nullptr);
  if (rc != RT_OK) return rc;
  HIP_TRY(hipStreamSynchronize(nullptr));
  size_t mem_free = 0, mem_total = 0;
  HIP_TRY(hipMemGetInfo(&mem_free, &mem_total));
  const unsigned long long budget = table_budget_bytes ? table_budget_bytes : std::min<unsigned long long>(32ull << 30, (unsigned long long)mem_free / 4ull);
// ... 78 lines not shown
  }
  fr->done = end; fr->samples_taken += st.camera_rays;
  if (stats_out) *stats_out = st;
  return RT_OK;
}
extern "C" int rt_frame_read(rt_frame* fr, int32_t what, float scale, uint32_t flags, void* stream_, void* out) {
  if (!fr || !out) return fail(RT_ERR_INVALID, "rt_frame_read: null argument");
  if (what != RT_FRAME_XYZW && what != RT_FRAME_RGB && what != RT_FRAME_RGB8 && what != RT_FRAME_STATS) return fail(RT_ERR_INVALID, "rt_frame_read: unknown read-out");
  if (what == RT_FRAME_STATS && !fr->stats) return fail(RT_ERR_INVALID, "rt_frame_read: RT_FRAME_STATS needs a frame begun with RT_FLAG_FRAME_STATS");
  rt_scene* s = fr->scene;
  std::lock_guard<std::mutex> render_lock(s->render_mutex);
  HIP_TRY(hipSetDevice(s->device));
  hipStream_t stream = (hipStream_t)stream_;
  const FrameParams fp = frame_pixel_params(fr);
  const unsigned long long n = (unsigned long long)(fp.crop_x1 - fp.crop_x0) * (unsigned long long)(fp.crop_y1 - fp.crop_y0);
  const size_t bytes = (size_t)n * (what == RT_FRAME_STATS ? 24 : (what == RT_FRAME_XYZW ? 16 : (what == RT_FRAME_RGB ? 12 : 3)));
  const bool on_device = (flags & RT_FLAG_FILM_ON_DEVICE) != 0;
  if (!on_device) HIP_TRY(fr->out.ensure((size_t)n * (what == RT_FRAME_STATS ? 24 : 16)));
  void* const d_out = on_device ? out : fr->out.p;
  if (what == RT_FRAME_STATS) hipLaunchKernelGGL(k_frame_stats_read, dim3((unsigned)((n + 255) / 256)), dim3(256), 0, stream, fp, fr->moments.as<PixMoments>(), (double*)d_out, n);
  else hipLaunchKernelGGL(k_frame_resolve, dim3((unsigned)((n + 255) / 256)), dim3(256), 0, stream, fp, fr->film_acc.as<float4>(), fr->own_acc.as<float4>(), (int)what, scale, d_out, n);
  HIP_TRY(hipGetLastError());
  if (!on_device) HIP_TRY(hipMemcpyAsync(out, d_out, bytes, hipMemcpyDeviceToHost, stream));
  HIP_TRY(hipStreamSynchronize(stream));
  return RT_OK;
}
extern "C" int rt_frame_query(rt_frame* fr, int32_t what, uint64_t* value) {
  if (!fr || !value) return fail(RT_ERR_INVALID, "rt_frame_query: null argument");
  switch (what) {
    case RT_FRAME_SAMPLES_DONE: *value = fr->done; return RT_OK;
    case RT_FRAME_SPP: *value = fr->spp; return RT_OK;
    case RT_FRAME_TABLES_RESIDENT: *value = fr->resident ? 1u : 0u; return RT_OK;
    case RT_FRAME_STATE_BYTES: *value = fr->state_bytes(); return RT_OK;
    case RT_FRAME_SAMPLES_TAKEN: *value = fr->samples_taken; return RT_OK;
    case RT_FRAME_ACTIVE_PIXELS: *value = fr->active_pixels; return RT_OK;
    default: return fail(RT_ERR_INVALID, "rt_frame_query: unknown query");
  }
}
extern "C" void rt_frame_end(rt_frame* fr) {
  if (!fr) return;
  std::lock_guard<std::mutex> render_lock(fr->scene->render_mutex);
  (void)hipSetDevice(fr->scene->device);
  (void)hipDeviceSynchronize();
  delete fr;
}

__global__ void k_film_add(float4* __restrict__ dst, const float4* __restrict__ src, unsigned long long n) {
  const unsigned long long i = (unsigned long long)blockIdx.x * blockDim.x + threadIdx.x;
  if (i >= n) return;
  const float4 a = dst[i], b = src[i];
  dst[i] = make_float4(a.x + b.x, a.y + b.y, a.z + b.z, a.w + b.w);
}
static void stats_add(rt_stats& a, const rt_stats& b) {
  a.camera_rays += b.camera_rays; a.rays_closest += b.rays_closest; a.rays_shadow += b.rays_shadow; a.rays_mis += b.rays_mis; a.rays_mis_not_cast += b.rays_mis_not_cast; a.rays_tail_not_cast += b.rays_tail_not_cast; a.rays_shadow_not_cast += b.rays_shadow_not_cast;
  a.nodes_closest += b.nodes_closest; a.nodes_shadow += b.nodes_shadow; a.nodes_mis += b.nodes_mis;
  a.tris_closest += b.tris_closest; a.tris_shadow += b.tris_shadow; a.tris_mis += b.tris_mis; a.paths_scrubbed += b.paths_scrubbed;
  a.ms_total += b.ms_total; a.ms_sampler += b.ms_sampler; a.ms_raygen += b.ms_raygen; a.ms_trace_closest += b.ms_trace_closest; a.ms_trace_any += b.ms_trace_any;
  a.ms_trace_mis += b.ms_trace_mis; a.ms_shade += b.ms_shade; a.ms_resolve += b.ms_resolve; a.ms_film += b.ms_film; a.ms_lightdist += b.ms_lightdist;
  a.launches_trace_closest += b.launches_trace_closest; a.n_passes += b.n_passes;
  a.launches_trace_path += b.launches_trace_path; a.launches_trace_shadow += b.launches_trace_shadow; a.launches_trace_mis += b.launches_trace_mis; a.launches_trace_mis_any += b.launches_trace_mis_any; a.launches_shade += b.launches_shade;
  a.vertices_lambert_const += b.vertices_lambert_const; a.vertices_lambert += b.vertices_lambert; a.vertices_two_lobe += b.vertices_two_lobe; a.vertices_generic += b.vertices_generic;
  a.ms_shade_lambert_const += b.ms_shade_lambert_const; a.ms_shade_lambert += b.ms_shade_lambert; a.ms_shade_two_lobe += b.ms_shade_two_lobe;
  a.ms_shade_generic += b.ms_shade_generic; a.ms_shade_bin += b.ms_shade_bin; a.ms_shade_miss += b.ms_shade_miss;
  for (int k = 0; k < 32; ++k) a.shade_section_cycles[k] += b.shade_section_cycles[k];
  a.rays_mis_any += b.rays_mis_any; a.nodes_mis_any += b.nodes_mis_any; a.tris_mis_any += b.tris_mis_any; a.ms_trace_mis_any += b.ms_trace_mis_any;
}
struct rt_multi {
  std::vector<int> devices; std::vector<rt_scene*> replicas; std::vector<hipStream_t> streams; std::vector<DevBuf*> chunk_film;
  DevBuf acc; std::vector<DevBuf*> staging;
  hipStream_t add_stream = nullptr;
  std::vector<hipEvent_t> chunk_done;
  std::vector<int> chunk_done_dev;
  std::string warnings;
  ~rt_multi() {
    for (size_t i = 0; i < replicas.size(); ++i) {
      (void)hipSetDevice(devices[i]);
      if (i < streams.size() && streams[i]) (void)hipStreamDestroy(streams[i]);
      if (i < chunk_film.size()) delete chunk_film[i];
      if (replicas[i]) rt_scene_destroy(replicas[i]);
    }
    for (size_t c = 0; c < chunk_done.size(); ++c) { (void)hipSetDevice(chunk_done_dev[c]); (void)hipEventDestroy(chunk_done[c]); }
    if (!devices.empty()) (void)hipSetDevice(devices[0]);
    if (add_stream) (void)hipStreamDestroy(add_stream);
    for (DevBuf* b : staging) delete b;
  }
};
extern "C" int rt_multi_create(const rt_scene_desc* desc, const int32_t* devices, int32_t n_devices, rt_multi** out) {
  if (!desc || !devices || n_devices < 1 || !out) return fail(RT_ERR_INVALID, "bad rt_multi_create arguments");
  RtScenePlan plan; std::string why;
  if (const int rc = rt_plan_scene(desc, plan, why)) return fail(rc, why);
  int n_visible = 0;
  if (hipGetDeviceCount(&n_visible) != hipSuccess || n_visible <= 0) return fail(RT_ERR_NO_DEVICE, "no HIP device visible; this backend has no CPU fallback");
  std::unique_ptr<rt_multi> m(new rt_multi());
  for (int i = 0; i < n_devices; ++i) {
    if (devices[i] < 0 || devices[i] >= n_visible) return fail(RT_ERR_INVALID, "device index out of range");
    m->devices.push_back(devices[i]); m->replicas.push_back(nullptr); m->streams.push_back(nullptr); m->chunk_film.push_back(new DevBuf());
  }
  for (int i = 0; i < n_devices; ++i) {
    const int rc = scene_from_plan(plan, desc, devices[i], &m->replicas[i]);
    if (rc != RT_OK) return rc;
    if (hipStreamCreateWithFlags(&m->streams[i], hipStreamNonBlocking) != hipSuccess) return fail(RT_ERR_HIP, "stream creation failed");
    if (devices[i] != devices[0]) {
      int can = 0; (void)hipDeviceCanAccessPeer(&can, devices[i], devices[0]);
      hipError_t e = can ? hipDeviceEnablePeerAccess(devices[0], 0) : hipErrorPeerAccessUnsupported;
      if (e != hipSuccess) (void)hipGetLastError();
      if (e != hipSuccess && e != hipErrorPeerAccessAlreadyEnabled)
        m->warnings += "device " + std::to_string(devices[i]) + " cannot write into device " + std::to_string(devices[0]) + " directly (" + hipGetErrorString(e) + "): film rows are staged by the runtime; ";
// ... 299 lines not shown
```

rustracer_amd/csrc/rtx_host.cpp:

```cpp
#include "../../include/rtx_host.h"

#include <algorithm>
#include <array>
#include <initializer_list>
#include <map>
#include <atomic>
#include <thread>
#include <cmath>
#include <cstdio>
#include <cstdlib>
#include <cstring>
#include <limits>
#include <sstream>
#include <string>
#include <vector>

namespace {

thread_local std::string g_err;
int fail(int code, const std::string& m) { g_err = m; return code; }

struct Box { float lo[3], hi[3]; };
const float kFmax = std::numeric_limits<float>::max();
inline Box box_empty() { return Box{{kFmax, kFmax, kFmax}, {-kFmax, -kFmax, -kFmax}}; }
// ... 1320 lines not shown
  if (!f || !value) return fail(RT_ERR_INVALID, "rtxh_multi_frame_query: null argument");
  g_err.clear();
  return rt_multi_frame_query(f->f, what, value);
}
void rtxh_multi_frame_end(rtxh_multi_frame* f) {
  if (!f) return;
  rt_multi_frame_end(f->f);
  f->scene->multi_frames -= 1;
  delete f;
}
int rtxh_trace(rtxh_scene* s, const float* rays, uint64_t n, int32_t any_hit, float* out, uint64_t counters[2]) {
  if (!s) return fail(RT_ERR_INVALID, "null scene");
  g_err.clear();
  if (!s->dev) { int rc = rtxh_scene_upload(s, -1); if (rc != RT_OK) return rc; }
  return any_hit ? rt_trace_any(s->dev, rays, n, (uint32_t*)out, counters) : rt_trace_closest(s->dev, rays, n, out, counters);
}
int rtxh_trace_device(rtxh_scene* s, const void* d_rays, uint64_t n, void* d_hits, int32_t reps, void* stream, float* ms) {
  if (!s) return fail(RT_ERR_INVALID, "null scene");
  g_err.clear();
  if (!s->dev) { int rc = rtxh_scene_upload(s, -1); if (rc != RT_OK) return rc; }
  return rt_trace_closest_device(s->dev, d_rays, n, d_hits, reps, stream, ms);
}
int rtxh_light_distribution(rtxh_scene* s, int32_t n_voxels[3], float* func, float* cdf, float* func_int) {
  if (!s) return fail(RT_ERR_INVALID, "null scene");
  g_err.clear();
  if (!s->dev) { int rc = rtxh_scene_upload(s, -1); if (rc != RT_OK) return rc; }
  return rt_light_distribution(s->dev, n_voxels, func, cdf, func_int);
}
int rtxh_scene_query(rtxh_scene* s, int32_t what) {
  if (!s) return fail(RT_ERR_INVALID, "null scene");
  g_err.clear();
  if (!s->dev) { int rc = rtxh_scene_upload(s, -1); if (rc != RT_OK) return rc; }
  return rt_scene_query(s->dev, what);
}
int rtxh_scene_device(rtxh_scene* s, rt_scene** out) {
  if (!s || !out) return fail(RT_ERR_INVALID, "null argument");
  g_err.clear();
  if (!s->dev) { int rc = rtxh_scene_upload(s, -1); if (rc != RT_OK) return rc; }
  *out = s->dev;
  return RT_OK;
}
int rtxh_scene_link_tables(rtxh_scene* s, int32_t mid, uint32_t* link_kept, uint32_t* link_full, uint64_t capacity_words, double* stats) {
  if (!s || !s->committed) return fail(RT_ERR_INVALID, "scene not committed");
  g_err.clear();
  rt_scene_desc d = make_desc(s);
  return rt_link_tables(&d, mid, link_kept, link_full, capacity_words, stats);
}
int rtxh_scene_shadow_sets(rtxh_scene* s, uint32_t* words, uint64_t capacity_words, int32_t n_voxels[3], uint64_t* stats) {
  if (!s || !s->committed) return fail(RT_ERR_INVALID, "scene not committed");
  g_err.clear();
  rt_scene_desc d = make_desc(s);
  return rt_shadow_sets(&d, words, capacity_words, n_voxels, stats);
}
int rtxh_sizeof(const char* name) {
  if (!name) return -1;
#define RTXH_SZ(T) if (!strcmp(name, #T)) return (int)sizeof(T);
  RTXH_SZ(rtxh_render_params) RTXH_SZ(rtxh_emitter_info) RTXH_SZ(rtxh_instance_info) RTXH_SZ(rtxh_light_info) RTXH_SZ(rtxh_ply) RTXH_SZ(rtxh_pbrt_result)
#undef RTXH_SZ
  return rt_sizeof(name);
}


namespace {
struct PlyProp { std::string name; int type = -1; bool is_list = false; int count_type = -1; };
struct PlyElem { std::string name; size_t count = 0; std::vector<PlyProp> props; };
int ply_type_id(const std::string& t) {
  static const char* names[][2] = {{"char", "int8"}, {"uchar", "uint8"}, {"short", "int16"}, {"ushort", "uint16"}, {"int", "int32"}, {"uint", "uint32"}, {"float", "float32"}, {"double", "float64"}};
  for (int i = 0; i < 8; ++i) if (t == names[i][0] || t == names[i][1]) return i;
  return -1;
}
const int kPlySize[8] = {1, 1, 2, 2, 4, 4, 4, 8};
struct PlyReader {
  FILE* f = nullptr; int format = 0;
  bool read_scalar(int type, double& out) {
    if (format == 0) { return fscanf(f, "%lf", &out) == 1; }
    unsigned char b[8]; const int n = kPlySize[type];
    if (fread(b, 1, (size_t)n, f) != (size_t)n) return false;
    if (format == 2) for (int i = 0; i < n / 2; ++i) std::swap(b[i], b[n - 1 - i]);
    switch (type) {
      case 0: { int8_t v; memcpy(&v, b, 1); out = v; break; }
      case 1: { uint8_t v; memcpy(&v, b, 1); out = v; break; }
      case 2: { int16_t v; memcpy(&v, b, 2); out = v; break; }
      case 3: { uint16_t v; memcpy(&v, b, 2); out = v; break; }
      case 4: { int32_t v; memcpy(&v, b, 4); out = v; break; }
      case 5: { uint32_t v; memcpy(&v, b, 4); out = v; break; }
      case 6: { float v; memcpy(&v, b, 4); out = v; break; }
      default: { double v; memcpy(&v, b, 8); out = v; break; }
    }
    return true;
  }
};
}

static int ply_read_unguarded(const char* path, rtxh_ply* out);
int rtxh_ply_read(const char* path, rtxh_ply* out) {
  if (!path || !out) return fail(RT_ERR_INVALID, "null argument");
  g_err.clear();
  memset(out, 0, sizeof(*out));
  try { return ply_read_unguarded(path, out); }
  catch (const std::bad_alloc&) { rtxh_ply_free(out); return fail(RT_ERR_OOM, std::string("out of memory while reading ") + path); }
  catch (const std::exception& e) { rtxh_ply_free(out); return fail(RT_ERR_INVALID, std::string(e.what()) + " (" + path + ")"); }
}
static int ply_read_unguarded(const char* path, rtxh_ply* out) {
  PlyReader rd; rd.f = fopen(path, "rb");
  if (!rd.f) return fail(RT_ERR_INVALID, std::string("cannot open ") + path);
  struct Closer { FILE* f; ~Closer() { if (f) fclose(f); } } closer{rd.f};
// ... 180 lines not shown
```

rustracer_amd/csrc/rtx_kernels.h:

```cpp
#pragma once
#include <type_traits>
#include "rtx_dev_shading.h"

namespace rtx {


#ifndef RT_NT_STREAMS
#define RT_NT_STREAMS 1
#endif
#if RT_NT_STREAMS
typedef float nt_v4f __attribute__((ext_vector_type(4)));
typedef unsigned nt_v4u __attribute__((ext_vector_type(4)));
typedef float nt_v2f __attribute__((ext_vector_type(2)));
RT_DEV float4 nt_ld(const float4* p) { const nt_v4f v = __builtin_nontemporal_load((const nt_v4f*)p); return make_float4(v.x, v.y, v.z, v.w); }
RT_DEV uint4 nt_ld(const uint4* p) { const nt_v4u v = __builtin_nontemporal_load((const nt_v4u*)p); return make_uint4(v.x, v.y, v.z, v.w); }
RT_DEV float2 nt_ld(const float2* p) { const nt_v2f v = __builtin_nontemporal_load((const nt_v2f*)p); return make_float2(v.x, v.y); }
RT_DEV unsigned nt_ld(const unsigned* p) { return __builtin_nontemporal_load(p); }
RT_DEV unsigned char nt_ld(const unsigned char* p) { return __builtin_nontemporal_load(p); }
RT_DEV void nt_st(float4 a, float4* p) { nt_v4f v; v.x = a.x; v.y = a.y; v.z = a.z; v.w = a.w; __builtin_nontemporal_store(v, (nt_v4f*)p); }
RT_DEV void nt_st(uint4 a, uint4* p) { nt_v4u v; v.x = a.x; v.y = a.y; v.z = a.z; v.w = a.w; __builtin_nontemporal_store(v, (nt_v4u*)p); }
RT_DEV void nt_st(float2 a, float2* p) { nt_v2f v; v.x = a.x; v.y = a.y; __builtin_nontemporal_store(v, (nt_v2f*)p); }
RT_DEV void nt_st(unsigned a, unsigned* p) { __builtin_nontemporal_store(a, p); }
RT_DEV void nt_st(unsigned char a, unsigned char* p) { __builtin_nontemporal_store(a, p); }
template <class T> struct NtRef {
// ... 14 lines not shown
};
template <class T> using SPtr = NtPtr<T>;
#define RT_SPTR_R(T) NtPtr<T>
template <class T> __host__ __device__ T* sraw(NtPtr<T> q) { return q.p; }
template <bool NT, class T> RT_DEV typename std::conditional<NT, NtPtr<T>, T*>::type sp(NtPtr<T> q) { if constexpr (NT) return q; else return q.p; }
#else
template <class T> using SPtr = T*;
#define RT_SPTR_R(T) T* __restrict__
template <class T> __host__ __device__ T* sraw(T* q) { return q; }
template <bool NT, class T> RT_DEV T* sp(T* q) { return q; }
#endif
struct PathGen { SPtr<float4> o; SPtr<float4> d; SPtr<float4> beta; SPtr<uint4> st; };
struct ShadowPlanes { SPtr<float4> o; SPtr<float4> d; SPtr<float4> add; };
struct MisPlanes { SPtr<float4> o; SPtr<float4> d; SPtr<float4> hit; SPtr<float4> a; SPtr<float4> b; SPtr<float4> c; SPtr<unsigned> flags; };
#define RT_PEND_SHADOW 1u
#define RT_PEND_MIS_ANY 0x40000000u
struct PassState {
  unsigned cap;
  unsigned spp, spp_log2, dims;
  unsigned n_pixels;
  unsigned n_pixels_recip;
  unsigned s0, n_samples;
  float4* own_acc;
  const unsigned* scrambles;
  const unsigned short* perms;
  PathGen in, out;
  SPtr<float4> hit;
  float4* lacc;
  SPtr<float2> pfilm;
  ShadowPlanes sh; MisPlanes mi;
  unsigned char* occ_sh; unsigned char* occ_mi;
  const unsigned* q_in; unsigned* q_shadow; unsigned* q_mis; unsigned* q_misany;
  const unsigned* cnt_in; unsigned* cnt_out; unsigned shard_cap;
  int all_in_bounds;
  int fresh;
#ifndef RT_FRESH_RECORDS
#define RT_FRESH_RECORDS 3
#endif
#ifndef RT_FRESH_RECORDS_LDS
#define RT_FRESH_RECORDS_LDS 2
#endif
#define RT_FRESH_BETA(ps) (((ps).fresh & 1) != 0)
#define RT_FRESH_ST(ps) (((ps).fresh & 2) != 0)
  int shadow_sets;
  int mis_any;
  int skip_unreachable_mis;
  int skip_dead_tail;
  const unsigned* range;
  unsigned long long* stats;
};
#define RT_NQ 4
#define RT_SHADOW_WALK 0u
#define RT_SHADOW_EMPTY 1u
#define RT_SHADOW_KIND(w) ((w) & 3u)
enum { ST_CAMERA = 0, ST_RAYS_CLOSEST, ST_RAYS_SHADOW, ST_RAYS_MIS, ST_NODES_CLOSEST, ST_NODES_SHADOW, ST_NODES_MIS,
       ST_TRIS_CLOSEST, ST_TRIS_SHADOW, ST_TRIS_MIS, ST_SCRUBBED, ST_UNBUILT_VOXEL,
       ST_RAYS_MISANY, ST_NODES_MISANY, ST_TRIS_MISANY,
       ST_MIS_UNREACHED,
       ST_TAIL_UNCAST,
       ST_SHADED,
       ST_STAMP = ST_SHADED + 4,
       ST_SHADOW_SETS = ST_STAMP + 32,
       ST_COUNT };
#ifdef RT_ABLATE
#define RT_STAMP(k) do { const unsigned long long t_ = clock64(); stamp_acc[k] += t_ - stamp_last; stamp_last = t_; } while (0)
#else
#define RT_STAMP(k) do { } while (0)
#endif

RT_DEV void split_path_id(const PassState& ps, unsigned pid, unsigned& sl, unsigned& pix) {
  unsigned q = __umulhi(pid, ps.n_pixels_recip), r = pid - q * ps.n_pixels;
  if (r >= ps.n_pixels) { q += 1u; r -= ps.n_pixels; }
  sl = q; pix = r;
}

struct FrameParams {
  float r2c[16]; float c2w[16]; f3 dx_camera, dy_camera; float lens_radius, focal_distance;
  int crop_x0, crop_y0, crop_x1, crop_y1; int sb_x0, sb_y0, sb_x1, sb_y1;
  float radius_x, radius_y, max_sample_luminance;
  int max_depth; float rr_threshold; int pb_x0, pb_y0, pb_x1, pb_y1;
  int rank, world, shard_log2;
  unsigned long long chunk_first;
  unsigned w_recip;
};

#define RT_STATE_OUT_OF_BOUNDS (1u << 17)
RT_DEV unsigned pack_state(int bounces, bool spec, int c1, int c2) { return (unsigned)bounces | ((unsigned)spec << 8) | ((unsigned)c1 << 9) | ((unsigned)c2 << 13); }

RT_DEV unsigned wave_push(unsigned* counter, bool pred) {
  unsigned long long mask = __ballot(pred);
  if (mask == 0ull) return 0u;
  unsigned lane = __lane_id();
  int leader = __ffsll((long long)mask) - 1;
  unsigned base = 0;
  if ((int)lane == leader) base = atomicAdd(counter, (unsigned)__popcll(mask));
  base = __shfl(base, leader);
  return base + (unsigned)__popcll(mask & ((1ull << lane) - 1ull));
}

#define RT_QSHARDS 8
#ifndef RT_CNT_STRIDE
#define RT_CNT_STRIDE 64
#endif
struct QView {
  const unsigned* ids; unsigned pre[RT_QSHARDS + 1]; unsigned shard_cap;
  RT_DEV void init(const unsigned* ids_, const unsigned* counts, unsigned cap) {
    ids = ids_; shard_cap = cap; pre[0] = 0;
#pragma unroll
    for (int k = 0; k < RT_QSHARDS; ++k) pre[k + 1] = pre[k] + counts[k * RT_CNT_STRIDE];
  }
  RT_DEV unsigned total() const { return pre[RT_QSHARDS]; }
  RT_DEV unsigned get(unsigned i) const {
    unsigned k = 0, base = 0;
#pragma unroll
    for (int j = 1; j < RT_QSHARDS; ++j) { const bool ge = i >= pre[j]; k += ge ? 1u : 0u; base = ge ? pre[j] : base; }
// ... 480 lines not shown
    const float4 v = sc.nodes[i]; const unsigned n = i >> 1, h = (i & 1u) * 4u;
    if (h == 0u) { s_nodes[n] = v.x; s_nodes[2 * N + n] = v.y; s_nodes[4 * N + n] = v.z; s_nodes[N + n] = v.w; }
    else if (BOUNDS_ONLY) { s_nodes[3 * N + n] = v.x; s_nodes[5 * N + n] = v.y; }
    else { s_nodes[3 * N + n] = v.x; s_nodes[5 * N + n] = v.y; s_nodes[6 * N + n] = v.z; s_nodes[7 * N + n] = __uint_as_float(lds_node_ctl(__float_as_uint(v.w))); }
  }
  if (BOUNDS_ONLY) return;
  for (unsigned i = threadIdx.x; i < 3u * sc.n_tris; i += BLOCK) {
    const float4 v = sc.tri_p[i]; const unsigned t = i / 3u, r = i - 3u * t;
    s_tris[(3u * r) * T + t] = v.x; s_tris[(3u * r + 1u) * T + t] = v.y; s_tris[(3u * r + 2u) * T + t] = v.z;
    if (r == 2u) s_tris[9 * T + t] = v.w;
  }
}

#ifndef RT_ANY_EARLY_SIGN
#define RT_ANY_EARLY_SIGN 1
#endif
#define RT_LINK_OFF_BITS(N) ((N) > 256 ? 11 : 7)
#define RT_LINK_LEAF_OFF(lk, N) ((int)(((lk) >> 16) & ((1u << RT_LINK_OFF_BITS(N)) - 1u)))
#define RT_LINK_LEAF_N(lk, N) ((int)(((lk) & 0x7fffffffu) >> (16 + RT_LINK_OFF_BITS(N))))
template <int N, int T, bool FINITE, int GENERAL = 0>
RT_DEV bool occluded_small_links(const float* __restrict__ s_nodes, const float* __restrict__ s_tris, const unsigned* __restrict__ link , const int n_nodes, const int start, const Ray ray, const GeneralCtx gen = GeneralCtx{nullptr, false}) {
  const f3 inv_dir = mk3(1.0f / ray.d.x, 1.0f / ray.d.y, 1.0f / ray.d.z);
  const RayPre rp = ray_pre(ray);
  const float* const tpx = s_tris + rp.kx * T; const float* const tpy = s_tris + rp.ky * T; const float* const tpz = s_tris + rp.kz * T;
  const f3 op = permute(ray.o, rp.kx, rp.ky, rp.kz);
  bool found = false;
  int cur = start;
  for (;;) {
    if (cur < n_nodes) {
      const float* nd = s_nodes + cur;
      const float4 n0 = make_float4(nd[0], nd[2 * N], nd[4 * N], nd[N]), n1 = make_float4(nd[3 * N], nd[5 * N], 0.0f, 0.0f);
      const unsigned lk = link[cur];
      const bool hit = slab_test_t<FINITE>(n0, n1, ray, inv_dir, inv_dir.x < 0.0f, inv_dir.y < 0.0f, inv_dir.z < 0.0f);
      int next = (int)(lk & 0xffffu);
      if (hit) {
        const int n_prims = (int)(lk >> 31) * RT_LINK_LEAF_N(lk, N);
        if (n_prims != 0) {
          const int off = RT_LINK_LEAF_OFF(lk, N);
          for (int i = 0; i < n_prims; ++i) {
            const int t = off + i;
            TriHit h;
            if (GENERAL) { if (leaf_prim_test<GENERAL>(LdsSrcT<N, T>{s_nodes, s_tris}, gen, t, ray, rp, h)) { found = true; next = n_nodes; break; } }
            else { const f3 p0t = mk3(tpx[t] - op.x, tpy[t] - op.y, tpz[t] - op.z), p1t = mk3(tpx[3 * T + t] - op.x, tpy[3 * T + t] - op.y, tpz[3 * T + t] - op.z), p2t = mk3(tpx[6 * T + t] - op.x, tpy[6 * T + t] - op.y, tpz[6 * T + t] - op.z);
              if (tri_test_permuted<RT_ANY_EARLY_SIGN != 0>(p0t, p1t, p2t, rp.sx, rp.sy, rp.sz, ray.t_max, h)) { found = true; next = n_nodes; break; } }
          }
        } else next = (int)(lk >> 16);
      }
      cur = next;
    }
    if (__ballot(cur < n_nodes) == 0ull) break;
  }
  return found;
}
template <int N, int T, bool FINITE, int LEAF_MIN, int GENERAL = 0, bool TRIS_GLOBAL = false>
RT_DEV bool closest_small_links(const float* __restrict__ s_nodes, const float* __restrict__ s_tris, const unsigned* __restrict__ link8 , const int row, const int n_nodes, Ray ray, int& prim_out, TriHit& hit_out, const GeneralCtx gen = GeneralCtx{nullptr, false}, const float4* __restrict__ tri_p = nullptr) {
  const f3 inv_dir = mk3(1.0f / ray.d.x, 1.0f / ray.d.y, 1.0f / ray.d.z);
  const int neg_x = inv_dir.x < 0.0f, neg_y = inv_dir.y < 0.0f, neg_z = inv_dir.z < 0.0f;
  const unsigned oct = (neg_x ? 1u : 0u) | (neg_y ? 2u : 0u) | (neg_z ? 4u : 0u);
  const unsigned* const link = link8 + oct * row;
  const RayPre rp = ray_pre(ray);
  const float* const tpx = s_tris + rp.kx * T; const float* const tpy = s_tris + rp.ky * T; const float* const tpz = s_tris + rp.kz * T;
  const f3 op = permute(ray.o, rp.kx, rp.ky, rp.kz);
  bool found = false;
  int cur = (int)link8[8 * row + oct], leaf_off = 0, leaf_n = 0;
  for (;;) {
    unsigned long long holders = 0ull;
    for (;;) {
      if (leaf_n == 0 && cur < n_nodes) {
        const float* nd = s_nodes + cur;
        const float4 n0 = make_float4(nd[0], nd[2 * N], nd[4 * N], nd[N]), n1 = make_float4(nd[3 * N], nd[5 * N], 0.0f, 0.0f);
        const unsigned lk = link[cur];
        int next = (int)(lk & 0xffffu);
        if (slab_test_t<FINITE>(n0, n1, ray, inv_dir, neg_x, neg_y, neg_z)) {
          if ((int)lk < 0) { leaf_off = RT_LINK_LEAF_OFF(lk, N); leaf_n = RT_LINK_LEAF_N(lk, N); }
          else next = (int)(lk >> 16);
        }
        cur = next;
      }
      holders = __ballot(leaf_n > 0);
      if (__ballot(leaf_n == 0 && cur < n_nodes) == 0ull) break;
      if (__builtin_popcount((unsigned)holders) + __builtin_popcount((unsigned)(holders >> 32)) >= LEAF_MIN) break;
    }
    if (holders == 0ull) break;
    if (leaf_n > 0) {
      const int t = leaf_off;
      TriHit h;
      if (GENERAL) { if (leaf_prim_test<GENERAL>(LdsSrcT<N, T>{s_nodes, s_tris}, gen, t, ray, rp, h)) { found = true; ray.t_max = h.t; prim_out = t; hit_out = h; } }
      else if (TRIS_GLOBAL) { f3 q0, q1, q2; load_tri(tri_p, t, q0, q1, q2); if (tri_test_pre(q0, q1, q2, ray, rp, h)) { found = true; ray.t_max = h.t; prim_out = t; hit_out = h; } }
      else { const f3 p0t = mk3(tpx[t] - op.x, tpy[t] - op.y, tpz[t] - op.z), p1t = mk3(tpx[3 * T + t] - op.x, tpy[3 * T + t] - op.y, tpz[3 * T + t] - op.z), p2t = mk3(tpx[6 * T + t] - op.x, tpy[6 * T + t] - op.y, tpz[6 * T + t] - op.z);
        if (tri_test_permuted(p0t, p1t, p2t, rp.sx, rp.sy, rp.sz, ray.t_max, h)) { found = true; ray.t_max = h.t; prim_out = t; hit_out = h; } }
      leaf_off += 1; leaf_n -= 1;
    }
  }
  return found;
}
template <int N, int T, bool FINITE, int LEAF_MIN, int GENERAL = 0>
RT_DEV bool occluded_small_links_rounds(const float* __restrict__ s_nodes, const float* __restrict__ s_tris, const unsigned* __restrict__ link, const int n_nodes, const int start, const Ray ray, const GeneralCtx gen = GeneralCtx{nullptr, false}) {
  const f3 inv_dir = mk3(1.0f / ray.d.x, 1.0f / ray.d.y, 1.0f / ray.d.z);
  const int neg_x = inv_dir.x < 0.0f, neg_y = inv_dir.y < 0.0f, neg_z = inv_dir.z < 0.0f;
  const RayPre rp = ray_pre(ray);
  const float* const tpx = s_tris + rp.kx * T; const float* const tpy = s_tris + rp.ky * T; const float* const tpz = s_tris + rp.kz * T;
  const f3 op = permute(ray.o, rp.kx, rp.ky, rp.kz);
  bool found = false;
  int cur = start, leaf_off = 0, leaf_n = 0;
  for (;;) {
    unsigned long long holders = 0ull;
    for (;;) {
      if (leaf_n == 0 && cur < n_nodes) {
        const float* nd = s_nodes + cur;
        const float4 n0 = make_float4(nd[0], nd[2 * N], nd[4 * N], nd[N]), n1 = make_float4(nd[3 * N], nd[5 * N], 0.0f, 0.0f);
        const unsigned lk = link[cur];
        int next = (int)(lk & 0xffffu);
        if (slab_test_t<FINITE>(n0, n1, ray, inv_dir, neg_x, neg_y, neg_z)) {
          if ((int)lk < 0) { leaf_off = RT_LINK_LEAF_OFF(lk, N); leaf_n = RT_LINK_LEAF_N(lk, N); }
          else next = (int)(lk >> 16);
        }
        cur = next;
      }
      holders = __ballot(leaf_n > 0);
      if (__ballot(leaf_n == 0 && cur < n_nodes) == 0ull) break;
      if (__builtin_popcount((unsigned)holders) + __builtin_popcount((unsigned)(holders >> 32)) >= LEAF_MIN) break;
    }
    if (holders == 0ull) break;
    if (leaf_n > 0) {
      const int t = leaf_off;
      TriHit h;
      leaf_off += 1; leaf_n -= 1;
      if (GENERAL) { if (leaf_prim_test<GENERAL>(LdsSrcT<N, T>{s_nodes, s_tris}, gen, t, ray, rp, h)) { found = true; cur = n_nodes; leaf_n = 0; } }
      else { const f3 p0t = mk3(tpx[t] - op.x, tpy[t] - op.y, tpz[t] - op.z), p1t = mk3(tpx[3 * T + t] - op.x, tpy[3 * T + t] - op.y, tpz[3 * T + t] - op.z), p2t = mk3(tpx[6 * T + t] - op.x, tpy[6 * T + t] - op.y, tpz[6 * T + t] - op.z);
        if (tri_test_permuted<RT_ANY_EARLY_SIGN != 0>(p0t, p1t, p2t, rp.sx, rp.sy, rp.sz, ray.t_max, h)) { found = true; cur = n_nodes; leaf_n = 0; } }
    }
  }
  return found;
}


struct TraceIO {
  SPtr<const float4> ray_o; SPtr<const float4> ray_d; unsigned ray_stride;
  SPtr<float4> hits; unsigned hit_stride; int hit_b2;
  unsigned* occluded; unsigned occ_stride;
  float4* lacc; unsigned lacc_stride; SPtr<const float4> direct_add; unsigned add_stride;
  int shadow_masks;
  int queue_is_slots;
};
template <class AddPtr>
RT_DEV void trace_write_any(float4* __restrict__ lacc, size_t ls, const AddPtr direct_add, size_t as, unsigned* __restrict__ occluded, size_t os,
                            unsigned pid, float dw, bool found) {
  if (lacc != nullptr && (__float_as_uint(dw) >> 31) != 0u) {
    if (!found) { const size_t path = __float_as_uint(dw) & 0x7fffffffu; float4 a = direct_add[pid * as]; float4 l = lacc[path * ls]; lacc[path * ls] = make_float4(l.x + a.x, l.y + a.y, l.z + a.z, l.w); }
  } else if (os == 0) ((unsigned char*)occluded)[pid] = found ? (unsigned char)1 : (unsigned char)0;
  else occluded[pid * os] = found ? 1u : 0u;
}

#ifndef RT_LDS_TRACE_WAVES
#define RT_LDS_TRACE_WAVES 7
#endif
#ifndef RT_LDS_ANY_WAVES
#define RT_LDS_ANY_WAVES 8
#endif
#ifndef RT_MID_LEAF_MIN_ANY
#define RT_MID_LEAF_MIN_ANY 8
#endif
#ifndef RT_LDS_LEAF_MIN_CLOSEST_GENERAL
#define RT_LDS_LEAF_MIN_CLOSEST_GENERAL 16
#endif
#ifndef RT_LDS_LEAF_MIN_ANY_GENERAL
#define RT_LDS_LEAF_MIN_ANY_GENERAL 56
#endif
#ifndef RT_MID_LEAF_MIN_CLOSEST
#define RT_MID_LEAF_MIN_CLOSEST 16
#endif
#define RT_MID_NODES 2816
#define RT_MID_TRIS 1408
template <bool ANY, bool COUNT, int BLOCK, int DEPTH, int GENERAL = 0, int MID = 0>
__global__ void __launch_bounds__(BLOCK, MID ? 4 : ((GENERAL == 0 && !COUNT) ? (ANY ? RT_LDS_ANY_WAVES : RT_LDS_TRACE_WAVES) : RT_GEN_MIN_WAVES(GENERAL))) k_trace(DScene sc, TraceIO io, const unsigned* __restrict__ queue, const unsigned* __restrict__ shard_counts, unsigned shard_cap,
                                                 unsigned count_static, unsigned long long* stats, int st_rays, int st_nodes, int st_tris) {
  const float4* __restrict__ ray_o = sraw(io.ray_o); const float4* __restrict__ ray_d = sraw(io.ray_d); const size_t rs = io.ray_stride;
  float4* __restrict__ hits = sraw(io.hits); const size_t hs = io.hit_stride; const bool hit_b2 = io.hit_b2 != 0;
  unsigned* __restrict__ occluded = io.occluded; const size_t os = io.occ_stride;
  float4* __restrict__ lacc = io.lacc; const size_t ls = io.lacc_stride; const float4* __restrict__ direct_add = sraw(io.direct_add); const size_t as = io.add_stride;
  typedef unsigned short StackT;
  constexpr bool LINKS = !COUNT;
  __shared__ StackT stack[LINKS ? 1 : DEPTH * BLOCK];
  constexpr int NN = MID ? RT_MID_NODES : RT_SMALL_NODES, NT = MID ? RT_MID_TRIS : RT_SMALL_TRIS;
  static_assert(!MID || (!COUNT && GENERAL == 0), "mid-size LDS scenes: plain triangles, no visit counts");
  constexpr bool MIDC = MID != 0 && !ANY;
  typedef LdsSrcT<NN, NT> LdsS;
  __shared__ float s_nodes[(MIDC ? 6 : 8) * NN];
  __shared__ float s_tris[MIDC ? 1 : 10 * NT];
  QView qv; if (queue) qv.init(io.queue_is_slots ? nullptr : queue, shard_counts, shard_cap);
  const unsigned count = queue ? qv.total() : count_static;
  if (blockIdx.x * BLOCK >= count) return;
  __shared__ unsigned s_link[LINKS ? (ANY ? 1 : 8) * NN + 8 : 1];
  stage_small_scene<BLOCK, NN, NT, MIDC>(sc, s_nodes, s_tris); __syncthreads();
  if (LINKS) {
    if (ANY) { for (unsigned k = threadIdx.x; k < sc.n_nodes; k += BLOCK) s_link[k] = sc.link8[8u * sc.n_nodes + 8u + k]; if (threadIdx.x == 0u) s_link[NN] = sc.link8[9u * sc.n_nodes + 8u]; }
    else {
      for (unsigned i = threadIdx.x; i < 8u * sc.n_nodes; i += BLOCK) { const unsigned o = i / sc.n_nodes, k = i - o * sc.n_nodes; s_link[o * NN + k] = sc.link8[i]; }
      if (threadIdx.x < 8u) s_link[8 * NN + threadIdx.x] = sc.link8[8u * sc.n_nodes + threadIdx.x];
    }
    __syncthreads();
  }
  const unsigned stride = gridDim.x * BLOCK;
  unsigned n_nodes = 0, n_tris = 0, n_rays = 0;
  auto trace_one = [&](unsigned pid) {
    float4 o4 = ray_o[pid * rs], d4 = ray_d[pid * rs];
    Ray ray; ray.o = mk3(o4.x, o4.y, o4.z); ray.d = mk3(d4.x, d4.y, d4.z); ray.t_max = o4.w;
    int prim = -1; TriHit h; h.t = kInf; h.b0 = h.b1 = h.b2 = 0.0f;
    bool found;
    constexpr int LM = ANY ? (MID ? RT_MID_LEAF_MIN_ANY : (GENERAL ? RT_LDS_LEAF_MIN_ANY_GENERAL : RT_LDS_LEAF_MIN_ANY)) : (MID ? RT_MID_LEAF_MIN_CLOSEST : (GENERAL ? RT_LDS_LEAF_MIN_CLOSEST_GENERAL : RT_LDS_LEAF_MIN_CLOSEST));
    const GeneralCtx gen{sc.self, ANY && io.shadow_masks != 0};
    constexpr bool FIN_FORMS = !COUNT;
    const bool fin = FIN_FORMS && __ballot(!inv_dir_finite(mk3(1.0f / ray.d.x, 1.0f / ray.d.y, 1.0f / ray.d.z))) == 0ull;
    if (LINKS) {
      static_assert(!LINKS || ANY || (LM > 1 && LM < 64), "the closest-hit link walk tests its leaves in phases: 1 < LEAF_MIN < 64");
      if (!ANY) {
        if (fin) found = closest_small_links<NN, NT, true, LM, GENERAL, MIDC>(s_nodes, s_tris, s_link, NN, (int)sc.n_nodes, ray, prim, h, gen, sc.tri_p);
        else found = closest_small_links<NN, NT, false, LM, GENERAL, MIDC>(s_nodes, s_tris, sc.link8_full, (int)sc.n_nodes, (int)sc.n_nodes, ray, prim, h, gen, sc.tri_p);
      } else if (LM > 1 && LM < 64) {
        found = fin ? occluded_small_links_rounds<NN, NT, true, LM, GENERAL>(s_nodes, s_tris, s_link, (int)sc.n_nodes, (int)s_link[NN], ray, gen)
                    : occluded_small_links_rounds<NN, NT, false, LM, GENERAL>(s_nodes, s_tris, sc.link8_full + 8u * sc.n_nodes + 8u, (int)sc.n_nodes, (int)sc.link8_full[9u * sc.n_nodes + 8u], ray, gen);
      } else {
        found = fin ? occluded_small_links<NN, NT, true, GENERAL>(s_nodes, s_tris, s_link, (int)sc.n_nodes, (int)s_link[NN], ray, gen)
                    : occluded_small_links<NN, NT, false, GENERAL>(s_nodes, s_tris, sc.link8_full + 8u * sc.n_nodes + 8u, (int)sc.n_nodes, (int)sc.link8_full[9u * sc.n_nodes + 8u], ray, gen);
      }
    }
    else {
      LdsS src{s_nodes, s_tris};
      found = traverse<ANY, COUNT, LdsS, StackT, GENERAL>(src, ray, stack + threadIdx.x, BLOCK, prim, h, n_nodes, n_tris, gen);
    }
    n_rays += 1;
    if (ANY) trace_write_any(lacc, ls, direct_add, as, occluded, os, pid, d4.w, found);
    else hits[pid * hs] = make_float4(hit_b2 ? h.b2 : (found ? h.t : kInf), __int_as_float(found ? prim : -1), h.b0, h.b1);
  };
  for (unsigned i = blockIdx.x * BLOCK + threadIdx.x; i < count; i += stride) trace_one(queue ? qv.get(i) : i);
  if (stats) {
    for (int off = 32; off > 0; off >>= 1) { n_rays += __shfl_down(n_rays, off); if (COUNT) { n_nodes += __shfl_down(n_nodes, off); n_tris += __shfl_down(n_tris, off); } }
    if ((threadIdx.x & 63u) == 0u) {
      if (n_rays) atomicAdd(&stats[st_rays], (unsigned long long)n_rays);
      if (COUNT) { atomicAdd(&stats[st_nodes], (unsigned long long)n_nodes); atomicAdd(&stats[st_tris], (unsigned long long)n_tris); }
    }
  }
}

struct TraceOut { SPtr<float4> hits; size_t hs; bool hit_b2; unsigned* occluded; size_t os; float4* lacc; size_t ls; SPtr<const float4> direct_add; size_t as; };
RT_DEV TraceOut trace_out_of(const TraceIO& io) {
  TraceOut o; o.hits = io.hits; o.hs = io.hit_stride; o.hit_b2 = io.hit_b2 != 0; o.occluded = io.occluded; o.os = io.occ_stride;
  o.lacc = io.lacc; o.ls = io.lacc_stride; o.direct_add = io.direct_add; o.as = io.add_stride; return o;
}

#ifndef RT_REFILL_MIN
#define RT_REFILL_MIN 16
#endif
struct NestedCtx { const float4* pairs; float* tstack; size_t grid_lanes; };
template <bool ANY, class StackT>
RT_DEV bool nested_pair_walk(const float4* __restrict__ pairs, const float4* __restrict__ nodes, const float4* __restrict__ tri_p, Ray& r, StackT* stack, int stack_stride,
                             float* tstack, size_t grid_lanes, int& prim_out, TriHit& hit_out);
struct ObjWalkOut { int found, prim; float t, b0, b1, b2; unsigned n_nodes, n_tris; };
template <bool ANY, bool COUNT, class StackT, int G>
RT_DEVN ObjWalkOut object_walk_general(const DScene* self, unsigned node_base, unsigned prim_base, float ox, float oy, float oz, float dx, float dy, float dz, float t_max,
                                       StackT* stack, int stack_stride, bool shadow_masks) {
  const DScene& sc = *self;
  Ray r; r.o = mk3(ox, oy, oz); r.d = mk3(dx, dy, dz); r.t_max = t_max;
  const GlobalSrc src{sc.nodes + 2 * (size_t)node_base, sc.tri_p + 3 * (size_t)prim_base};
  const GeneralCtx gen{self, shadow_masks, (int)prim_base};
  ObjWalkOut o{}; TriHit h; h.t = kInf; h.b0 = h.b1 = h.b2 = 0.0f;
  o.found = traverse<ANY, COUNT, GlobalSrc, StackT, G>(src, r, stack, stack_stride, o.prim, h, o.n_nodes, o.n_tris, gen) ? 1 : 0;
  o.t = h.t; o.b0 = h.b0; o.b1 = h.b1; o.b2 = h.b2;
  return o;
}
template <bool ANY, bool COUNT, class StackT, bool MASKS = false, bool QUADRICS = false>
RT_DEV bool instance_intersect(const DScene& sc, unsigned inst, f3 o, f3 d, float& t_max, int& prim_out, TriHit& hit_out, unsigned& n_nodes, unsigned& n_tris,
                               StackT* stack, int stack_stride, NestedCtx nc = NestedCtx{nullptr, nullptr, 0}, bool shadow_masks = false) {
  const DInstance& in = sc.instances[inst];
  Ray r; r.o = xf34_point(in.w2o, o); r.d = xf34_vector(in.w2o, d); r.t_max = t_max;
  bool found;
  constexpr int OBJ_GENERAL = MASKS ? RT_GEN_ALL : (QUADRICS ? RT_GEN_NO_MASKS : 0);
  if (in.n_nodes == 0u) {
    const float4 pa = sc.tri_p[3 * (size_t)in.prim_base], pb = sc.tri_p[3 * (size_t)in.prim_base + 1], pc = sc.tri_p[3 * (size_t)in.prim_base + 2];
    const f3 p0 = mk3(pa.x, pa.y, pa.z), p1 = mk3(pb.x, pb.y, pb.z), p2 = mk3(pc.x, pc.y, pc.z);
    const unsigned flags = __float_as_uint(pc.w);
    if (COUNT) n_tris += 1;
    TriHit h;
    if (OBJ_GENERAL != 0 && (flags & (RT_FLAG_SPHERE | RT_FLAG_GENERAL_TRI))) found = general_prim_test<MASKS, QUADRICS>(*sc.self, (int)in.prim_base, p0, p1, p2, flags, r, ray_pre(r), shadow_masks, h);
    else found = tri_test(p0, p1, p2, r, h);
    if (found) { prim_out = 0; hit_out = h; r.t_max = h.t; }
  } else if (OBJ_GENERAL != 0 && sc.obj_general) {
    const ObjWalkOut w = object_walk_general<ANY, COUNT, StackT, OBJ_GENERAL>(sc.self, in.node_base, in.prim_base, r.o.x, r.o.y, r.o.z, r.d.x, r.d.y, r.d.z, r.t_max, stack, stack_stride, shadow_masks);
    found = w.found != 0;
    if (COUNT) { n_nodes += w.n_nodes; n_tris += w.n_tris; }
    if (found) { prim_out = w.prim; hit_out.t = w.t; hit_out.b0 = w.b0; hit_out.b1 = w.b1; hit_out.b2 = w.b2; if (!ANY) r.t_max = w.t; }
  } else {
    if (!COUNT && nc.pairs != nullptr) {
// ... 1437 lines not shown
```

rustracer_amd/csrc/rtx_scene_plan.h:

```cpp
#pragma once
#include <map>
#include <string>
#include "rtx_link_tables.h"
#include "rtx_shadow_sets.h"

struct RtScenePlan {
  std::vector<float> tri_p;
  std::vector<DInstance> instances;
  std::vector<float> texels; std::vector<DImage> images;
  std::vector<uint32_t> fourier; std::vector<uint64_t> fourier_at;
  std::vector<DTexture> textures;
  std::vector<DMaterial> materials; std::vector<int> mat_kind, mat_table, mat_class;
  unsigned n_code_classes = 0, n_lambert_classes = 0, n_small_classes = 0, n_wide_classes = 0;
  std::vector<uint16_t> prim_class;
  std::vector<DLight> lights; std::vector<float> dist; std::vector<unsigned short> guides;
  int n_infinite = 0, infinite_ids[4] = {0, 0, 0, 0};
  std::vector<float> pairs, top_pairs, quads;
  RtLinkTables links; RtShadowSets shadow;
  uint32_t n_top_nodes = 0, n_top_prims = 0, n_all_lights = 0;
  int stack_depth = 64, quad_stack_depth = 0, needs_differentials = 0, obj_pairs = 0, route_quadric_hits = 0;
  bool small = false, mid = false, general_prims = false, obj_general = false, has_masks = false, has_spheres = false, has_instances = false, masked_emitters = false;
  bool lambert_only = false, lambert_materials = false, lean_shade = false, lean_qlights = false, lds_records = false, lds_records_q = false, lds_tables = false, lds_mats = false;
  bool use_pairs = false, use_top = false, top_for_closest = false, use_quads = false, deep_column = false, shadow_sets = false;
};

static int rt_refuse(std::string& why, int code, const std::string& msg) { why = msg; return code; }
template <class T> static const T* rt_blob_offset(size_t n) { return reinterpret_cast<const T*>(n * sizeof(T)); }
template <class T> static void rt_blob_rebase(const T*& p, const void* blob) { p = reinterpret_cast<const T*>((const char*)blob + reinterpret_cast<uintptr_t>(p)); }
static bool is_const_texture(const rt_scene_desc* desc, int id) { return id >= 0 && (uint32_t)id < desc->n_textures && desc->textures[id].kind == RT_TEX_CONST; }
static long guide_quarters() { return 4; }

static bool sphere_lights_clear(const rt_scene_desc* desc) {
  std::vector<uint32_t> emitters;
  for (uint32_t i = 0; i < desc->n_lights; ++i) {
    const rt_light& l = desc->lights[i];
    if (l.kind != RT_LIGHT_DIFFUSE_AREA || l.prim < 0 || (uint32_t)l.prim >= desc->n_tris) continue;
    if (!(desc->tri_meta[l.prim].flags & RT_PRIM_SPHERE)) continue;
    uint32_t k; memcpy(&k, &desc->tri_p[9 * (size_t)l.prim + 6], 4);
    if (k >= desc->n_spheres || desc->spheres[k].kind != 0) return false;
    emitters.push_back(k);
  }
  if ((double)emitters.size() * (double)desc->n_tris > 2e8) return false;
  for (uint32_t k : emitters) {
    const rt_sphere& sp = desc->spheres[k];
    const double c[3] = {sp.o2w[3], sp.o2w[7], sp.o2w[11]};
    const double r = (double)sp.radius * 1.001 + 1e-6 * std::max(std::max(fabs(c[0]), fabs(c[1])), fabs(c[2])), r2 = r * r;
    for (uint32_t t = 0; t < desc->n_tris; ++t) {
      if (desc->tri_meta[t].flags & (RT_PRIM_SPHERE | RT_PRIM_INSTANCE)) continue;
      const float* q = desc->tri_p + 9 * (size_t)t;
      double a[3], b[3], cc[3];
      for (int j = 0; j < 3; ++j) { a[j] = q[j] - c[j]; b[j] = q[3 + j] - c[j]; cc[j] = q[6 + j] - c[j]; }
      auto dot3 = [](const double* x, const double* y) { return x[0] * y[0] + x[1] * y[1] + x[2] * y[2]; };
      double ab[3], ac[3]; for (int j = 0; j < 3; ++j) { ab[j] = b[j] - a[j]; ac[j] = cc[j] - a[j]; }
      double best[3];
      const double d1 = -dot3(ab, a), d2 = -dot3(ac, a);
      const double d3 = -dot3(ab, b), d4 = -dot3(ac, b), d5 = -dot3(ab, cc), d6 = -dot3(ac, cc);
      const double vc = d1 * d4 - d3 * d2, vb = d5 * d2 - d1 * d6, va = d3 * d6 - d5 * d4;
      if (d1 <= 0 && d2 <= 0) { for (int j = 0; j < 3; ++j) best[j] = a[j]; }
      else if (d3 >= 0 && d4 <= d3) { for (int j = 0; j < 3; ++j) best[j] = b[j]; }
      else if (vc <= 0 && d1 >= 0 && d3 <= 0) { const double v = d1 / (d1 - d3); for (int j = 0; j < 3; ++j) best[j] = a[j] + v * ab[j]; }
      else if (d6 >= 0 && d5 <= d6) { for (int j = 0; j < 3; ++j) best[j] = cc[j]; }
      else if (vb <= 0 && d2 >= 0 && d6 <= 0) { const double w = d2 / (d2 - d6); for (int j = 0; j < 3; ++j) best[j] = a[j] + w * ac[j]; }
      else if (va <= 0 && (d4 - d3) >= 0 && (d5 - d6) >= 0) { const double w = (d4 - d3) / ((d4 - d3) + (d5 - d6)); for (int j = 0; j < 3; ++j) best[j] = b[j] + w * (cc[j] - b[j]); }
      else { const double den = 1.0 / (va + vb + vc), v = vb * den, w = vc * den; for (int j = 0; j < 3; ++j) best[j] = a[j] + ab[j] * v + ac[j] * w; }
      if (!(dot3(best, best) > r2)) return false;
    }
  }
  return true;
}

#define RT_SHADOW_PLAIN_FLAGS (RT_TRI_FLIP | RT_TRI_HAS_N | RT_TRI_HAS_UV | RT_TRI_HAS_S)
static bool shadow_sets_apply(const rt_scene_desc* desc, bool plain) {
  if (!plain || desc->n_lights != 2 || !desc->lights) return false;
  for (uint32_t k = 0; k < desc->n_lights; ++k) {
    const rt_light& l = desc->lights[k];
    if (l.kind != 0 || l.prim < 0 || (uint32_t)l.prim >= desc->n_tris || (desc->tri_meta[l.prim].flags & ~(uint32_t)RT_SHADOW_PLAIN_FLAGS)) return false;
  }
  return true;
}

#define RT_FOURIER_MAX_WORDS (1ull << 28)
static std::string fourier_table_error(const rt_image& im, uint64_t& words) {
  if (!im.texels) return "Fourier BSDF table without words";
  if (im.n_texels > RT_FOURIER_MAX_WORDS) return "Fourier BSDF table larger than 2^28 words";
  const uint64_t cap = 3 * im.n_texels;
  if (cap < 5) return "Fourier BSDF table shorter than its header";
  const uint32_t* w = (const uint32_t*)im.texels;
  const uint64_t n_mu = w[0], m_max = w[1], n_ch = w[2], n_coeffs = w[3];
  float eta; memcpy(&eta, &w[4], 4);
  if (n_mu < 2 || n_mu > 8192) return "Fourier BSDF table: nMu must lie in [2, 8192]";
  if (n_ch != 1 && n_ch != 3) return "Fourier BSDF table: nChannels must be 1 or 3";
  if (n_coeffs > RT_FOURIER_MAX_WORDS) return "Fourier BSDF table: nCoeffs larger than 2^28";
  if (!std::isfinite(eta)) return "Fourier BSDF table: eta is not finite";
  words = 5 + n_mu + 3 * n_mu * n_mu + n_coeffs;
  if ((words + 2) / 3 != im.n_texels) return "Fourier BSDF table: sizes do not add up (" + std::to_string(words) + " words for " + std::to_string(im.n_texels) + " texels)";
  const float* mu = (const float*)(w + 5);
  for (uint64_t i = 0; i < n_mu; ++i) if (!std::isfinite(mu[i]) || (i > 0 && !(mu[i - 1] < mu[i]))) return "Fourier BSDF table: mu is not strictly ascending";
  const uint32_t* ol = w + 5 + n_mu + n_mu * n_mu;
  for (uint64_t c = 0; c < n_mu * n_mu; ++c) {
    const uint64_t off = ol[2 * c], len = ol[2 * c + 1];
    if (len > m_max) return "Fourier BSDF table: a cell's length exceeds mMax";
    if (off + len * n_ch > n_coeffs) return "Fourier BSDF table: a cell's coefficients run past nCoeffs";
  }
  return "";
}
static bool tex_mapped(int kind) { return kind == RT_TEX_CHECKER_PLANAR || kind == RT_TEX_FBM_MAPPED; }
static std::vector<char> word_blocks(const rt_scene_desc* desc) {
  std::vector<char> b(desc->images ? desc->n_images : 0, 0);
  for (uint32_t i = 0; i < desc->n_textures && desc->textures; ++i) {
    const rt_texture& t = desc->textures[i];
    if (tex_mapped(t.kind) && t.image >= 0 && (size_t)t.image < b.size()) b[t.image] = 1;
  }
  return b;
}
static std::string fourier_desc_error(const rt_scene_desc* desc) {
  const std::vector<char> block = word_blocks(desc);
  auto is_block = [&](int id) { return id >= 0 && (size_t)id < block.size() && block[id]; };
  auto is_table = [&](int id) { return id >= 0 && (uint32_t)id < desc->n_images && desc->images && desc->images[id].n_levels == 0 && !is_block(id); };
  uint64_t total = 0;
  for (uint32_t i = 0; i < desc->n_images; ++i) {
    if (!desc->images || desc->images[i].n_levels != 0 || is_block((int)i)) continue;
    uint64_t words = 0;
    const std::string why = fourier_table_error(desc->images[i], words);
    if (!why.empty()) return "image " + std::to_string(i) + ": " + why;
// ... 453 lines not shown
    if (desc->lights[i].kind != RT_LIGHT_DIFFUSE_AREA) all_area_lights = false;
    else if (desc->tri_meta[desc->lights[i].prim].flags & RT_TRI_HAS_ALPHA) p.masked_emitters = true;
  }
  if (p.has_spheres || p.has_instances) p.masked_emitters = true;
  p.lean_shade = !p.masked_emitters && all_area_lights && all_const_textures;
  p.lean_qlights = p.has_spheres && !p.has_instances && !p.has_masks && all_area_lights && all_const_textures && sphere_lights_clear(desc);
  if (!all_area_lights || p.masked_emitters) p.lambert_only = false;
  p.route_quadric_hits = (p.lean_qlights && p.n_code_classes > 1 && !p.lambert_materials) ? 1 : 0;
  p.small = desc->n_nodes <= RT_SMALL_NODES && desc->n_tris <= RT_SMALL_TRIS && !p.has_instances;
  p.mid = !p.small && !p.general_prims && !p.has_instances && desc->n_nodes <= RT_MID_NODES && desc->n_tris <= RT_MID_TRIS;
  for (uint32_t i = 0; i < desc->n_nodes && p.mid; ++i) if (desc->nodes[i].n_prims > 15) p.mid = false;
  const char* ldsrec = getenv("RTX_SHADE_LDSREC");
  p.lds_mats = desc->n_materials <= RT_LDS_MATERIALS && desc->n_textures <= RT_LDS_TEXTURES && !(ldsrec && ldsrec[0] == '0');
  p.lds_tables = p.lds_mats && p.n_all_lights <= RT_LDS_LIGHTS && desc->n_images <= RT_LDS_IMAGES;
  p.lds_records_q = p.lds_mats && p.n_all_lights <= RT_LDS_LIGHTS && desc->n_tris <= RT_SMALL_TRIS && !p.has_instances;
  p.lds_records = p.lds_records_q && p.small && !p.has_spheres;
}

static void pair_record(const rt_bvh_node& a, const rt_bvh_node& b, uint32_t ca, uint32_t cb, float* q) {
  q[0] = a.bmin[0]; q[1] = a.bmin[1]; q[2] = a.bmin[2]; q[3] = a.bmax[0]; q[4] = a.bmax[1]; q[5] = a.bmax[2]; memcpy(q + 6, &ca, 4); memcpy(q + 7, &cb, 4);
  q[8] = b.bmin[0]; q[9] = b.bmin[1]; q[10] = b.bmin[2]; q[11] = b.bmax[0]; q[12] = b.bmax[1]; q[13] = b.bmax[2];
}
static int plan_trees(const rt_scene_desc* desc, RtScenePlan& p, std::string& why) {
  const uint32_t n_top_nodes = p.n_top_nodes, n_top_prims = p.n_top_prims;
  auto tree_depth = [&](uint32_t base, uint32_t nn, uint32_t np, int& maxd) -> bool {
    std::vector<int> depth(nn, 0); maxd = 0;
    for (uint32_t i = 0; i < nn; ++i) {
      const rt_bvh_node& n = desc->nodes[base + i];
      if (n.n_prims == 0) {
        if (i + 1 >= nn || n.offset >= nn || n.offset <= i) return false;
        depth[i + 1] = depth[i] + 1; depth[n.offset] = depth[i] + 1;
      } else if ((uint64_t)n.offset + n.n_prims > np) return false;
      if (depth[i] > maxd) maxd = depth[i];
    }
    return true;
  };
  int maxd = 0;
  if (!tree_depth(0, n_top_nodes, n_top_prims, maxd)) return rt_refuse(why, RT_ERR_INVALID, "malformed BVH");
  if (maxd + 1 > 64) return rt_refuse(why, RT_ERR_INVALID, "BVH deeper than the 64-entry traversal stack");
  int max_obj_depth = 0;
  for (uint32_t k = 0; k < desc->n_instances; ++k) {
    const rt_instance& in = desc->instances[k];
    int od = 0;
    if (in.n_nodes && (!tree_depth(in.node_base, in.n_nodes, in.n_prims, od) || od + 1 > 64)) return rt_refuse(why, RT_ERR_INVALID, "malformed or too deep object BVH");
    if (in.n_nodes) max_obj_depth = std::max(max_obj_depth, od + 1);
  }
  p.stack_depth = maxd + 1 + max_obj_depth;
  p.deep_column = p.stack_depth > 64;
  if (p.small || p.mid) rt_build_link_tables(desc, p.mid, false, p.links);
  const char* sets = getenv("RTX_SHADOW_SETS");
  if (shadow_sets_apply(desc, p.small && !p.general_prims && !p.has_instances) && !(sets && sets[0] == '0')) {
    int32_t lp[2] = {0, 0};
    for (uint32_t k = 0; k < desc->n_lights; ++k) lp[k] = desc->lights[k].prim;
    rt_build_shadow_sets(desc->tri_p, desc->n_tris, lp, (int)desc->n_lights, desc->nodes[0].bmin, desc->nodes[0].bmax, p.shadow);
    p.shadow_sets = p.shadow.empty > 0;
  }
  if (p.small || p.deep_column) return RT_OK;
  const uint32_t n_pair_nodes = n_top_nodes;
  const bool gen = p.general_prims;
  auto general_leaf = [&](const rt_bvh_node& n) {
    for (uint32_t t = n.offset; t < n.offset + n.n_prims; ++t)
      if (desc->tri_meta[t].flags & (RT_TRI_HAS_ALPHA | RT_TRI_HAS_SHADOW_ALPHA | RT_PRIM_SPHERE | RT_PRIM_INSTANCE)) return true;
    return false;
  };
  bool ok = n_pair_nodes < (1u << 29) && n_top_prims < (gen ? (1u << 25) : (1u << 26)) && desc->nodes[0].n_prims <= 32;
  auto code_of = [&](uint32_t base, uint32_t c, bool& good) -> uint32_t {
    const rt_bvh_node& n = desc->nodes[base + c];
    if (n.n_prims > 0) { if (n.n_prims > 32) good = false; return 0x80000000u | n.offset | ((uint32_t)(n.n_prims - 1) << 26) | (base == 0 && gen && general_leaf(n) ? RT_PAIR_GENERAL : 0u); }
    return c | ((uint32_t)n.axis << 29);
  };
  auto pair_tree = [&](uint32_t base, uint32_t nn, bool& good) {
    for (uint32_t i = 0; i < nn && good; ++i) {
      const rt_bvh_node& n = desc->nodes[base + i];
      if (n.n_prims != 0) continue;
      const uint32_t ca = code_of(base, i + 1, good), cb = code_of(base, n.offset, good);
      pair_record(desc->nodes[base + i + 1], desc->nodes[base + n.offset], ca, cb, p.pairs.data() + (size_t)(base + i) * 16);
    }
  };
  p.pairs.assign((size_t)(p.has_instances ? desc->n_nodes : n_pair_nodes) * 16, 0.0f);
  pair_tree(0, n_pair_nodes, ok);
  bool obj_ok = ok && p.has_instances;
  if (obj_ok) {
    std::vector<char> done(desc->n_nodes, 0);
    for (uint32_t k = 0; k < desc->n_instances && obj_ok; ++k) {
      const rt_instance& in = desc->instances[k];
      if (in.n_nodes == 0 || done[in.node_base]) continue;
      done[in.node_base] = 1;
      if (in.n_nodes >= (1u << 29) || in.n_prims >= (1u << 26) || desc->nodes[in.node_base].n_prims > 32) { obj_ok = false; break; }
      pair_tree(in.node_base, in.n_nodes, obj_ok);
    }
  }
  if (!ok) { p.pairs.clear(); return RT_OK; }
  p.use_pairs = true;
  p.obj_pairs = (obj_ok && !p.obj_general) ? 1 : 0;
  if (n_pair_nodes < (1u << 28) && desc->nodes[0].n_prims == 0 && !p.has_instances) {
    std::vector<uint32_t> top; std::vector<int> slot_of(n_pair_nodes, -1);
    top.push_back(0); slot_of[0] = 0;
    for (size_t head = 0; head < top.size(); ++head) {
      const uint32_t P = top[head]; const uint32_t kids[2] = {P + 1, desc->nodes[P].offset};
      for (uint32_t c : kids)
        if (desc->nodes[c].n_prims == 0 && top.size() < RT_TOP_MAX) { slot_of[c] = (int)top.size(); top.push_back(c); }
    }
    p.top_pairs.assign(top.size() * 16, 0.0f);
    for (size_t k = 0; k < top.size(); ++k) {
      uint32_t code[2]; memcpy(code, p.pairs.data() + (size_t)top[k] * 16 + 6, 8);
      for (int side = 0; side < 2; ++side)
        if (!(code[side] & 0x80000000u) && slot_of[code[side] & 0x0fffffffu] >= 0) code[side] = (code[side] & 0x60000000u) | RT_PAIR_TOP | (uint32_t)slot_of[code[side] & 0x0fffffffu];
      pair_record(desc->nodes[top[k] + 1], desc->nodes[desc->nodes[top[k]].offset], code[0], code[1], p.top_pairs.data() + 16 * k);
// ... 51 lines not shown
```

rustracer_amd/csrc/rtx_shade_kernels.h:

```cpp
#pragma once
#include "rtx_kernels.h"

namespace rtx {

struct PathSampler {
  Tables tb; unsigned pix, s; int c1, c2; Pcg32 rng;
  RT_DEV float get_1d() {
    if (c1 < (int)tb.dims) return table_1d(tb, pix, (unsigned)c1++, s);
    return rng.next_f32();
  }
  RT_DEV f2 get_2d() {
    if (c2 < (int)tb.dims) return table_2d(tb, pix, (unsigned)c2++, s);
    float x = rng.next_f32();
    float y = rng.next_f32();
    return mk2(y, x);
  }
};

struct GenericBsdf {
  Bsdf b;
  RT_DEV void build(const DScene& sc, int mat, SurfaceInteraction& si) { build_bsdf(sc, mat, si, b); }
  RT_DEV int num_nonspecular() const { return bsdf_num_components(b, BSDF_ALL & ~BSDF_SPECULAR); }
  RT_DEV rgb3 f(f3 wo, f3 wi, unsigned flags) const { return bsdf_f(b, wo, wi, flags); }
  RT_DEV float pdf(f3 wo, f3 wi, unsigned flags) const { return bsdf_pdf(b, wo, wi, flags); }
// ... 317 lines not shown
        }
        else if (MODE != 0) tri_fill_interaction_inl<MODE == 1 || MODE == 3>(sc, prim, ray_d, th, si);
        else tri_fill_interaction(gsc, prim, ray_d, th, si);
      }
      RT_STAMP(0);
      if (bounces == 0 || specular_bounce) {
        if (found) {
          int li = rec_light(sc.tri_rec, prim);
          if (li >= 0) { const float4 l4 = ps.lacc[pid]; const rgb3 L = mkc(l4.x, l4.y, l4.z) + beta * area_light_l(sc.lights[li], si.hit.n, -ray_d); ps.lacc[pid] = make_float4(L.r, L.g, L.b, l4.w); }
        } else if ((MODE != 1 && !LEAN) && sc.n_infinite > 0) {
          const float4 l4 = ps.lacc[pid]; rgb3 L = mkc(l4.x, l4.y, l4.z);
          for (int k = 0; k < sc.n_infinite; ++k) L = L + beta * infinite_le<BOUNCED>(sc, sc.lights[k == 0 ? sc.infinite_ids[0] : (k == 1 ? sc.infinite_ids[1] : (k == 2 ? sc.infinite_ids[2] : sc.infinite_ids[3]))], ray_d);
          ps.lacc[pid] = make_float4(L.r, L.g, L.b, l4.w);
        }
      }
      if (found && bounces < fp.max_depth) {
        if ((MODE != 1 && !LEAN && !BOUNCED) && bounces == 0 && sc.needs_differentials && !RT_DBG(sc, 16)) {
          f2 pf; { float2 t = pfilm_[pid]; pf = mk2(t.x, t.y); }
          const f2 pl = fp.lens_radius > 0.0f ? table_2d(smp.tb, pix, 1, s) : mk2(0.0f, 0.0f);
          CameraRay cr = generate_camera_ray(fp, pf, pl, 1.0f / sqrtf((float)ps.spp));
          if (MODE == 0) compute_differential_call(si, cr.rx_o, cr.ry_o, cr.rx_d, cr.ry_d); else compute_differential(si, cr.rx_o, cr.ry_o, cr.rx_d, cr.ry_d);
        }
        typename std::conditional<MODE == 1, SingleLambert, typename std::conditional<MODE == 3, SingleLambertT<!LEAN, BOUNCED>,
                                  typename std::conditional<MODE == 5, SmallBsdfT<false, LEAN>, typename std::conditional<MODE == 6, SmallBsdfT<true, LEAN>, GenericBsdf>::type>::type>::type>::type bsdf;
        RT_STAMP(1);
        if (MODE == 0) bsdf.build(gsc, rec_material(sc.tri_rec, prim), si); else bsdf.build(sc, rec_material(sc.tri_rec, prim), si);
        RT_STAMP(2);
        const float* ld_func; const float* ld_cdf; float ld_int; long ld_row = 0;
        float4 ld_r0 = make_float4(0, 0, 0, 0), ld_r1 = ld_r0;
        const bool rows8 = sc.ld_rows8 != nullptr;
        if (sc.ld_uniform) { ld_func = sc.ld_func; ld_cdf = sc.ld_cdf; if (rows8) { ld_r0 = sc.ld_rows8[0]; ld_r1 = sc.ld_rows8[1]; ld_int = ld_r0.x; } else ld_int = sc.ld_int[0]; }
        else if (sc.ld_dense8 != nullptr) {
          const long v = voxel_of(sc, si.hit.p);
          ld_r0 = sc.ld_dense8[2 * v]; ld_r1 = sc.ld_dense8[2 * v + 1]; ld_int = ld_r0.x; ld_func = sc.ld_func; ld_cdf = sc.ld_cdf;
        }
        else {
          const long slot = sc.ld_slot[voxel_of(sc, si.hit.p)];
          if (slot >= 0) {
            ld_func = sc.ld_func + slot * sc.n_lights; ld_cdf = sc.ld_cdf + slot * (sc.n_lights + 1); ld_row = slot;
            if (rows8) { ld_r0 = sc.ld_rows8[2 * slot]; ld_r1 = sc.ld_rows8[2 * slot + 1]; ld_int = ld_r0.x; } else ld_int = sc.ld_int[slot];
          }
          else { ld_func = sc.ld_func; ld_cdf = sc.ld_cdf; ld_int = -1.0f; }
        }
        const unsigned nonspec = BSDF_ALL & ~BSDF_SPECULAR;
        const bool voxel_ok = !(ld_int < 0.0f);
        if (!voxel_ok) atomicAdd(&ps.stats[ST_UNBUILT_VOXEL], 1ull);
        if (voxel_ok && bsdf.num_nonspecular() > 0 && sc.n_lights > 0) {
          float su = smp.get_1d();
          int light_num; float light_pdf;
          if (RT_DBG(sc, 128)) { light_num = clampi((int)(su * (float)sc.n_lights), 0, sc.n_lights - 1); light_pdf = 1.0f / (float)sc.n_lights; }
          else if (rows8) d1_sample_discrete_row8(ld_r0, ld_r1, sc.n_lights, su, light_num, light_pdf);
          else if (MODE != 1 && sc.ld_glog >= 0) d1_sample_discrete_guided(ld_func, ld_cdf, ld_int, sc.n_lights, su, sc.ld_guide + ld_row * ((1 << sc.ld_glog) + 1), sc.ld_glog, light_num, light_pdf);
          else d1_sample_discrete(ld_func, ld_cdf, ld_int, sc.n_lights, su, light_num, light_pdf);
          const bool ld_empty = MODE == 1 && ps.shadow_sets && RT_SHADOW_KIND(__float_as_uint(light_num == 0 ? ld_r0.w : ld_r1.w)) == RT_SHADOW_EMPTY;
          RT_STAMP(3);
          if (light_pdf != 0.0f) {
            f2 u_light = smp.get_2d();
            f2 u_scattering = smp.get_2d();
            const DLight& light = sc.lights[RT_DBG(sc, 256) ? 0 : light_num];
            rgb3 ld1 = mkc(0, 0, 0); f3 sh_dir = mk3(0, 0, 0);
            const bool q_light = QLIGHTS && (tri_flags(sc.tri_p, light.prim) & RT_FLAG_SPHERE) != 0u;
            f3 q_center = mk3(0, 0, 0);
            LiSample ls;
            if (q_light) {
              const DSphere& sp = sc.spheres[prim_sphere_index(sc.tri_p, light.prim)];
              q_center = xf34_point(sp.o2w, mk3(0, 0, 0));
              float pdf; const SpherePoint pt = sphere_cone_sample_si(sp, q_center, si.hit, u_light, pdf);
              ls.p1.p = pt.p; ls.p1.p_error = pt.p_error; ls.p1.n = pt.n;
              ls.wi = normalize(pt.p - si.hit.p); ls.pdf = pdf; ls.li = area_light_l(light, pt.n, -ls.wi);
            } else ls = (MODE == 1 || LEAN) ? area_light_sample_li(sc, light, si.hit, u_light) : light_sample_li_full<GENERAL, false, BOUNCED>(gsc, light, si.hit, u_light);
            if (ls.pdf > 0.0f && !is_black(ls.li)) {
              rgb3 f = bsdf.f(si.hit.wo, ls.wi, nonspec) * fabsf(dot(ls.wi, si.sh_n));
              float scattering_pdf = ((MODE != 1 && !LEAN) && light_is_delta(light)) ? 0.0f : bsdf.pdf(si.hit.wo, ls.wi, nonspec);
              if (!is_black(f)) {
                Ray sr = spawn_ray_to_interaction(si.hit, ls.p1);
                if (!ld_empty) sh_o[i] = make_float4(sr.o.x, sr.o.y, sr.o.z, sr.t_max);
                sh_dir = sr.d;
                want_shadow = true;
                if (light_is_delta(light)) ld1 = vdiv(f * ls.li, ls.pdf);
                else ld1 = vdiv(f * ls.li * power_heuristic1(ls.pdf, scattering_pdf), ls.pdf);
              }
            }
            RT_STAMP(4);
            rgb3 f2v = mkc(0, 0, 0); float w2 = 0.0f, spdf2 = 1.0f;
            if (!light_is_delta(light) && !RT_DBG(sc, 8)) {
              LobeSample bs = bsdf.sample_f(si.hit.wo, u_scattering, nonspec);
              rgb3 f = bs.f * fabsf(dot(bs.wi, si.sh_n));
              if (!is_black(f) && bs.pdf > 0.0f) {
                float weight = 1.0f; bool go = true;
                if (!(bs.type & BSDF_SPECULAR)) {
                  float lp;
                  if (q_light) lp = sphere_cone_pdf_wi(sc.spheres[prim_sphere_index(sc.tri_p, light.prim)], q_center, si.hit);
                  else if (RT_DBG(sc, 512)) lp = 1.0f;
                  else lp = (MODE == 1 || LEAN) ? area_light_pdf_li<false>(sc, light, si.hit, bs.wi) : light_pdf_li<GENERAL, BOUNCED>(gsc, light, si.hit, bs.wi);
                  if (lp == 0.0f) go = false;
                  else weight = power_heuristic1(bs.pdf, lp);
                  if ((GENERAL || QLIGHTS) && go && ps.skip_unreachable_mis && light.kind == 0 && (tri_flags(sc.tri_p, light.prim) & RT_FLAG_SPHERE)) {
                    const float4 b0 = sc.tri_p[3 * (size_t)light.prim], b1 = sc.tri_p[3 * (size_t)light.prim + 1];
                    if (!ray_may_reach_box(mk3(b0.x, b0.y, b0.z), mk3(b1.x, b1.y, b1.z), si.hit.p, bs.wi)) { go = false; n_unreached += 1u; }
                  }
                }
                if (go) {
                  Ray mr = spawn_ray(si.hit, bs.wi);
                  mi_o[i] = make_float4(mr.o.x, mr.o.y, mr.o.z, kInf);
                  mi_d[i] = make_float4(mr.d.x, mr.d.y, mr.d.z, __uint_as_float(pid));
                  want_mis = true; f2v = f; w2 = weight; spdf2 = bs.pdf;
                  mis_occlusion_only = (MODE != 1 && !LEAN) && ps.mis_any && light.kind == 3;
                }
              }
            }
            no_walk = want_shadow && ld_empty;
            if (want_mis) {
              mi_a[i] = make_float4(ld1.r, ld1.g, ld1.b, light_pdf);
              mi_b[i] = make_float4(f2v.r, f2v.g, f2v.b, w2);
              mi_c[i] = make_float4(beta.r, beta.g, beta.b, spdf2);
              mi_flags[i] = (want_shadow ? RT_PEND_SHADOW : 0u) | 2u | ((unsigned)light_num << 2) | (mis_occlusion_only ? RT_PEND_MIS_ANY : 0u);
              if (!want_shadow || no_walk) ps.occ_sh[i] = no_walk ? (unsigned char)0 : (unsigned char)1;
            } else if (want_shadow) {
              rgb3 add = beta * vdiv(mkc(0, 0, 0) + ld1, light_pdf);
              if (no_walk) { const float4 l4 = ps.lacc[pid]; ps.lacc[pid] = make_float4(l4.x + add.r, l4.y + add.g, l4.z + add.b, l4.w); }
              else sh_add[i] = make_float4(add.r, add.g, add.b, 0.0f);
            }
            if (want_shadow && !no_walk) sh_d[i] = make_float4(sh_dir.x, sh_dir.y, sh_dir.z, __uint_as_float((want_mis ? 0u : 0x80000000u) | pid));
            want_shadow = want_shadow && !no_walk;
          }
        }
        RT_STAMP(5);
        f3 wo = -ray_d;
        LobeSample bs = bsdf.sample_f(wo, smp.get_2d(), BSDF_ALL);
        if (!(is_black(bs.f) || bs.pdf <= 0.0f)) {
          beta = vdiv(beta * bs.f * fabsf(dot(bs.wi, si.sh_n)), bs.pdf);
          specular_bounce = (bs.type & BSDF_SPECULAR) != 0u;
          if ((bs.type & BSDF_SPECULAR) && (bs.type & BSDF_TRANSMISSION)) {
            float eta = bsdf.eta();
            eta_scale *= dot(wo, si.hit.n) > 0.0f ? eta * eta : vdiv(1.0f, eta * eta);
          }
          cont = true;
          rgb3 rr_beta = beta * eta_scale;
          if (max_component_value(rr_beta) < fp.rr_threshold && bounces > 3) {
            float q = fmaxf(1.0f - max_component_value(rr_beta), 0.05f);
            if (smp.get_1d() < q) cont = false;
            else beta = vdiv(beta, 1.0f - q);
          }
          if (cont) bounces += 1;
          if (cont && ps.skip_dead_tail && bounces >= fp.max_depth && !specular_bounce) { cont = false; tail = true; }
          if (cont) { const Ray nr = spawn_ray(si.hit, bs.wi); nr_o = nr.o; nr_d = nr.d; }
        }
      }
      st_out = pack_state(bounces, specular_bounce, smp.c1, smp.c2); rng_out = smp.rng.state;
    }
    RT_STAMP(6);
    n_tail += (unsigned)__popcll(__ballot(tail));
    n_no_walk += (unsigned)__popcll(__ballot(no_walk));
    constexpr int NQ = (MODE == 1 || LEAN) ? 3 : 4;
    const int ci[4] = {0, 1, 2, 3}; const bool pr[4] = {cont, want_shadow, want_mis && !mis_occlusion_only, want_mis && mis_occlusion_only}; unsigned slot[4];
    block_push<NQ>(ps.cnt_out, ps.shard_cap, ci, pr, slot);
    if (cont) {
      out_o[slot[0]] = make_float4(nr_o.x, nr_o.y, nr_o.z, kInf);
      out_d[slot[0]] = make_float4(nr_d.x, nr_d.y, nr_d.z, 0.0f);
      out_beta[slot[0]] = make_float4(beta.r, beta.g, beta.b, eta_scale);
      out_st[slot[0]] = make_uint4(st_out, pid, (unsigned)rng_out, (unsigned)(rng_out >> 32));
    }
    if (want_shadow) ps.q_shadow[slot[1]] = i;
    if (pr[2]) ps.q_mis[slot[2]] = i;
    if (NQ == 4 && pr[3]) ps.q_misany[slot[3]] = i;
  };
  if (MODE != 1) {
    for (unsigned base = first + blockIdx.x * blockDim.x; base < count; base += stride) {
      const unsigned i = base + threadIdx.x;
      const bool lane_live = i < count;
      n_shaded += lane_live ? 1u : 0u;
      shade_vertex(lane_live, i, lane_live ? (ps.cnt_in ? qv.get(i) : i) : 0u);
    }
  } else {
// ... 47 lines not shown
```

rustracer_amd/csrc/rtx_shadow_sets.h:

```cpp
#pragma once
#include <algorithm>
#include <cmath>
#include <cstdint>
#include <vector>


struct RtShadowSets {
  int nvox[3] = {1, 1, 1};
  int n_lights = 0;
  std::vector<uint32_t> word;
  uint64_t pairs = 0, empty = 0;
};

namespace rtss {
struct D3 { double x, y, z; };
static inline D3 sub(D3 a, D3 b) { return D3{a.x - b.x, a.y - b.y, a.z - b.z}; }
static inline D3 crs(D3 a, D3 b) { return D3{a.y * b.z - a.z * b.y, a.z * b.x - a.x * b.z, a.x * b.y - a.y * b.x}; }
static inline double dot(D3 a, D3 b) { return a.x * b.x + a.y * b.y + a.z * b.z; }
static inline double l1(D3 a) { return std::fabs(a.x) + std::fabs(a.y) + std::fabs(a.z); }
static inline D3 unit(D3 a) { const double l = std::sqrt(dot(a, a)); return l > 0.0 ? D3{a.x / l, a.y / l, a.z / l} : D3{0, 0, 0}; }
struct Box { D3 lo, hi; };
static inline double box_min(const Box& b, D3 a) { return (a.x < 0 ? b.hi.x : b.lo.x) * a.x + (a.y < 0 ? b.hi.y : b.lo.y) * a.y + (a.z < 0 ? b.hi.z : b.lo.z) * a.z; }
static inline double box_max(const Box& b, D3 a) { return (a.x < 0 ? b.lo.x : b.hi.x) * a.x + (a.y < 0 ? b.lo.y : b.hi.y) * a.y + (a.z < 0 ? b.lo.z : b.hi.z) * a.z; }
}

static void rt_shadow_grid(const float wb_min[3], const float wb_max[3], int nvox[3]) {
  const float diag[3] = {wb_max[0] - wb_min[0], wb_max[1] - wb_min[1], wb_max[2] - wb_min[2]};
  const int ext = diag[0] > diag[1] ? (diag[0] > diag[2] ? 0 : 2) : (diag[1] > diag[2] ? 1 : 2);
  for (int i = 0; i < 3; ++i) {
    const float r = roundf(diag[i] / diag[ext] * 64.0f);
    const unsigned v = (r != r || r <= 0.0f) ? 0u : (unsigned)r;
    nvox[i] = (int)(v > 1u ? v : 1u);
  }
}

static void rt_build_shadow_sets(const float* tri_p, uint32_t n_tris, const int32_t* light_prims, int n_lights, const float wb_min[3], const float wb_max[3], RtShadowSets& out) {
  using namespace rtss;
  rt_shadow_grid(wb_min, wb_max, out.nvox);
  out.n_lights = n_lights;
  const int nx = out.nvox[0], ny = out.nvox[1], nz = out.nvox[2];
  const size_t total = (size_t)nx * ny * nz;
  out.word.assign(total * 2, RT_SHADOW_WALK);
  out.pairs = out.empty = 0;
  if (n_lights != 2 || n_tris == 0) return;
  const D3 wmin{wb_min[0], wb_min[1], wb_min[2]}, wmax{wb_max[0], wb_max[1], wb_max[2]};
  const D3 ext = sub(wmax, wmin);
  const double scale = std::max(ext.x, std::max(ext.y, ext.z));
  const double mag = std::max(scale, std::max(std::max(std::fabs(wmin.x), std::fabs(wmax.x)), std::max(std::max(std::fabs(wmin.y), std::fabs(wmax.y)), std::max(std::fabs(wmin.z), std::fabs(wmax.z)))));
  if (!(scale > 0.0) || !(mag <= 64.0 * scale)) return;
  const double PAD_V = 1e-4 * scale + 1e-5 * mag, PAD_O = 2e-4 * mag, PAD_L = 1e-4 * mag, SEP = 1e-4 * mag, COPLANAR = 1e-9 * mag;
  const double ONE_MINUS_TMAX = 0.99e-4;
  const double T_GAP = 5e-5;
  auto vtx = [&](uint32_t t, int k) { const float* p = tri_p + 9 * (size_t)t + 3 * k; return D3{p[0], p[1], p[2]}; };
  std::vector<Box> tbox(n_tris);
  std::vector<D3> tn(n_tris);
  for (uint32_t t = 0; t < n_tris; ++t) {
    const D3 a = vtx(t, 0), b = vtx(t, 1), c = vtx(t, 2);
    tbox[t].lo = D3{std::min(a.x, std::min(b.x, c.x)), std::min(a.y, std::min(b.y, c.y)), std::min(a.z, std::min(b.z, c.z))};
    tbox[t].hi = D3{std::max(a.x, std::max(b.x, c.x)), std::max(a.y, std::max(b.y, c.y)), std::max(a.z, std::max(b.z, c.z))};
    tn[t] = unit(crs(sub(b, a), sub(c, a)));
  }
  auto sdist = [&](uint32_t t, D3 x) { return dot(tn[t], sub(x, vtx(t, 0))); };
  auto coplanar = [&](uint32_t t, uint32_t s) {
    if (dot(tn[t], tn[t]) == 0.0) return false;
    for (int k = 0; k < 3; ++k) if (std::fabs(sdist(t, vtx(s, k))) > COPLANAR) return false;
    return true;
  };
  std::vector<uint32_t> surf;
  for (int z = 0; z < nz; ++z)
    for (int y = 0; y < ny; ++y)
      for (int x = 0; x < nx; ++x) {
        const size_t v = ((size_t)z * ny + y) * nx + x;
        Box vb;
        vb.lo = D3{wmin.x + ext.x * x / nx - PAD_V, wmin.y + ext.y * y / ny - PAD_V, wmin.z + ext.z * z / nz - PAD_V};
        vb.hi = D3{wmin.x + ext.x * (x + 1) / nx + PAD_V, wmin.y + ext.y * (y + 1) / ny + PAD_V, wmin.z + ext.z * (z + 1) / nz + PAD_V};
        surf.clear();
        for (uint32_t t = 0; t < n_tris; ++t) {
          const Box& b = tbox[t];
          if (b.lo.x <= vb.hi.x + PAD_O && b.hi.x >= vb.lo.x - PAD_O && b.lo.y <= vb.hi.y + PAD_O && b.hi.y >= vb.lo.y - PAD_O && b.lo.z <= vb.hi.z + PAD_O && b.hi.z >= vb.lo.z - PAD_O)
            surf.push_back(t);
        }
        if (surf.empty()) continue;
        Box ob;
        ob.lo = D3{vb.lo.x - PAD_O, vb.lo.y - PAD_O, vb.lo.z - PAD_O}; ob.hi = D3{vb.hi.x + PAD_O, vb.hi.y + PAD_O, vb.hi.z + PAD_O};
        for (int l = 0; l < n_lights; ++l) {
          out.pairs += 1;
          const uint32_t lp = (uint32_t)light_prims[l];
          if (lp >= n_tris) continue;
          const D3 L[3] = {vtx(lp, 0), vtx(lp, 1), vtx(lp, 2)};
          auto separated = [&](uint32_t t) {
            const D3 T[3] = {vtx(t, 0), vtx(t, 1), vtx(t, 2)};
            const D3 te[3] = {sub(T[1], T[0]), sub(T[2], T[1]), sub(T[0], T[2])}, le[3] = {sub(L[1], L[0]), sub(L[2], L[1]), sub(L[0], L[2])};
            const D3 ax3[3] = {D3{1, 0, 0}, D3{0, 1, 0}, D3{0, 0, 1}};
            const D3 oc{0.5 * (ob.lo.x + ob.hi.x), 0.5 * (ob.lo.y + ob.hi.y), 0.5 * (ob.lo.z + ob.hi.z)};
            const D3 lc{(L[0].x + L[1].x + L[2].x) / 3.0, (L[0].y + L[1].y + L[2].y) / 3.0, (L[0].z + L[1].z + L[2].z) / 3.0};
            auto test = [&](D3 a) {
              a = unit(a);
              if (dot(a, a) == 0.0) return false;
              double h0 = box_min(ob, a), h1 = box_max(ob, a);
              const double lpad = PAD_L * l1(a);
              for (int k = 0; k < 3; ++k) { const double p = dot(a, L[k]); h0 = std::min(h0, p - lpad); h1 = std::max(h1, p + lpad); }
              double t0 = dot(a, T[0]), t1 = t0;
              for (int k = 1; k < 3; ++k) { const double p = dot(a, T[k]); t0 = std::min(t0, p); t1 = std::max(t1, p); }
              return t1 < h0 - SEP || t0 > h1 + SEP;
            };
            for (int k = 0; k < 3; ++k) if (test(ax3[k])) return true;
            if (test(tn[t]) || test(tn[lp])) return true;
            for (int i = 0; i < 3; ++i) {
              for (int k = 0; k < 3; ++k) if (test(crs(te[i], ax3[k])) || test(crs(te[i], le[k]))) return true;
              if (test(crs(te[i], sub(lc, oc)))) return true;
              for (int k = 0; k < 3; ++k) if (test(crs(te[i], sub(L[k], oc)))) return true;
            }
            return false;
          };
          auto behind = [&](uint32_t t) {
            if (dot(tn[t], tn[t]) == 0.0) return false;
            for (int sg = -1; sg <= 1; sg += 2) {
              auto s = [&](D3 p) { return sg * sdist(t, p); };
              const bool l_in = coplanar(t, lp);
              double st_min = l_in ? 0.0 : std::min(s(L[0]), std::min(s(L[1]), s(L[2]))) - PAD_L * std::sqrt(3.0);
              if (!l_in && !(st_min > 0.0)) continue;
              double so_min = HUGE_VAL, so_max = -HUGE_VAL; bool ok = true;
              for (uint32_t si : surf) {
                if (coplanar(t, si)) {
                  if (l_in) { ok = false; break; }
                  so_min = std::min(so_min, 0.0); so_max = std::max(so_max, PAD_O);
                  continue;
                }
                Box c;
                c.lo = D3{std::max(tbox[si].lo.x - PAD_O, ob.lo.x), std::max(tbox[si].lo.y - PAD_O, ob.lo.y), std::max(tbox[si].lo.z - PAD_O, ob.lo.z)};
                c.hi = D3{std::min(tbox[si].hi.x + PAD_O, ob.hi.x), std::min(tbox[si].hi.y + PAD_O, ob.hi.y), std::min(tbox[si].hi.z + PAD_O, ob.hi.z)};
                const D3 a{sg * tn[t].x, sg * tn[t].y, sg * tn[t].z};
                const double off = sg * dot(tn[t], vtx(t, 0));
                const double mn = box_min(c, a) - off, mx = box_max(c, a) - off;
                if (!(mn >= 0.0)) { ok = false; break; }
                so_min = std::min(so_min, mn); so_max = std::max(so_max, mx);
              }
              if (!ok) continue;
              const double se_min = ONE_MINUS_TMAX * so_min + (1.0 - ONE_MINUS_TMAX) * st_min;
              if (se_min > 0.0 && se_min >= T_GAP * so_max) return true;
            }
            return false;
          };
          bool empty = true;
          for (uint32_t t = 0; t < n_tris && empty; ++t) if (!behind(t) && !separated(t)) empty = false;
          if (empty) { out.word[2 * v + l] = RT_SHADOW_EMPTY; out.empty += 1; }
        }
      }
}
```

rustracer_amd/host.py:

```python
from __future__ import annotations

import ctypes as C
import os
import subprocess

import numpy as np

_HERE = os.path.dirname(os.path.abspath(__file__))
_CSRC = os.path.join(_HERE, "csrc")
_BUILD = os.path.join(_CSRC, "_build")
HOST_LIB = os.path.join(_BUILD, "librtx_host.so")
HIP_LIB = os.path.join(_BUILD, "librtx_hip.so")

RT_FLAG_COUNT_TRAVERSAL = 1
RT_FLAG_FILM_ON_DEVICE = 2
RT_FLAG_TIME_KERNELS = 4
RT_FLAG_COUNT_AS_RENDERED = 8
RT_FLAG_REF_STREAM = 16
RT_FLAG_FRAME_STATS = 32
RT_BSDF_FRONT_AUTO, RT_BSDF_FRONT_GENERIC, RT_BSDF_FRONT_LAMBERT, RT_BSDF_FRONT_TWO_LOBE, RT_BSDF_FRONT_TWO_LOBE_WIDE = range(5)
RT_BSDF_SURFACE_FLOATS = 40
RT_BSDF_OUT_FLOATS = 13
RT_SAMPLES_MAX = 1 << 27
RT_QUERY_BSDF_LAUNCHED = 5
# ... 4 lines not shown


class BackendError(RuntimeError):
    pass


STAMP = os.path.join(_BUILD, "source.sha")


def source_sha() -> str:
    import hashlib
    h = hashlib.sha256()
    files = [os.path.join(_CSRC, f) for f in sorted(os.listdir(_CSRC)) if f.endswith((".h", ".hip", ".cpp", ".inl")) or f == "Makefile"]
    files += [os.path.join(_HERE, "..", "include", f) for f in ("rtx_hip.h", "rtx_host.h")]
    for f in files:
        h.update(os.path.basename(f).encode() + b"\0")
        h.update(open(f, "rb").read())
    return h.hexdigest()


def build(force: bool = False) -> None:
    sha = source_sha()
    stamped = open(STAMP).read().strip() if os.path.exists(STAMP) else None
    if force or stamped != sha or not (os.path.exists(HOST_LIB) and os.path.exists(HIP_LIB)):
        subprocess.check_call(["make", "-C", _CSRC, "-s"] + (["-B"] if force or (stamped is not None and stamped != sha) else []))
        with open(STAMP, "w") as f:
            f.write(sha + "\n")


class RenderParams(C.Structure):
    _fields_ = [
        ("xres", C.c_int32), ("yres", C.c_int32), ("crop", C.c_float * 4),
        ("filter_kind", C.c_int32), ("filter_params", C.c_float * 4),
        ("film_scale", C.c_float), ("max_sample_luminance", C.c_float),
        ("cam_to_world", C.c_float * 16), ("cam_to_world_inv", C.c_float * 16),
        ("fov", C.c_float), ("lens_radius", C.c_float), ("focal_distance", C.c_float),
        ("spp", C.c_int32), ("sampler_dims", C.c_int32),
        ("max_depth", C.c_int32), ("rr_threshold", C.c_float), ("light_strategy", C.c_int32),
        ("pixel_bounds", C.c_int32 * 4), ("rank", C.c_int32), ("world_size", C.c_int32), ("flags", C.c_uint32),
        ("screen_window", C.c_float * 4), ("has_pixel_bounds", C.c_int32),
    ]


class Stats(C.Structure):
    _fields_ = ([(n, C.c_uint64) for n in (
        "camera_rays", "rays_closest", "rays_shadow", "rays_mis", "nodes_closest", "nodes_shadow", "nodes_mis",
        "tris_closest", "tris_shadow", "tris_mis", "paths_scrubbed")] +
        [(n, C.c_double) for n in ("ms_total", "ms_sampler", "ms_raygen", "ms_trace_closest", "ms_trace_any", "ms_trace_mis",
                                   "ms_shade", "ms_resolve", "ms_film", "ms_lightdist")] +
        [(n, C.c_uint64) for n in ("launches_trace_closest", "n_passes", "vertices_lambert_const", "vertices_lambert", "vertices_two_lobe", "vertices_generic")] +
        [(n, C.c_double) for n in ("ms_shade_lambert_const", "ms_shade_lambert", "ms_shade_two_lobe", "ms_shade_generic", "ms_shade_bin", "ms_shade_miss")] +
        [("shade_section_cycles", C.c_uint64 * 32)] +
        [(n, C.c_uint64) for n in ("rays_mis_any", "nodes_mis_any", "tris_mis_any")] + [("ms_trace_mis_any", C.c_double), ("ms_gather", C.c_double), ("rays_mis_not_cast", C.c_uint64), ("rays_tail_not_cast", C.c_uint64)] +
        [(n, C.c_uint64) for n in ("launches_trace_path", "launches_trace_shadow", "launches_trace_mis", "launches_trace_mis_any", "launches_shade", "rays_shadow_not_cast")])

    def as_dict(self):
        return {n: (list(getattr(self, n)) if n == "shade_section_cycles" else getattr(self, n)) for n, _ in self._fields_}


_lib = None
_hip = None


def lib():
    global _lib, _hip
    if _lib is None:
        if not os.path.exists(HOST_LIB):
            raise BackendError(f"{HOST_LIB} missing: run `python -c 'import __graft_entry__ as g; g.build()'`")
        _hip = C.CDLL(HIP_LIB, mode=C.RTLD_GLOBAL)
        _lib = C.CDLL(HOST_LIB)
        L = _lib
        L.rtxh_scene_new.restype = C.c_void_p
        L.rtxh_scene_free.argtypes = [C.c_void_p]
        L.rtxh_last_error.restype = C.c_char_p
        _hip.rt_last_error.restype = C.c_char_p
        _hip.rt_version.restype = C.c_char_p
        for name, mirror in (("rt_stats", Stats), ("rtxh_render_params", RenderParams), ("rtxh_pbrt_result", PbrtResult)):
            n = L.rtxh_sizeof(name.encode())
            if n != C.sizeof(mirror):
                _lib = _hip = None
                raise BackendError(f"{HOST_LIB}: sizeof({name}) = {n}, the ctypes mirror {mirror.__name__} has {C.sizeof(mirror)} bytes - rebuild (make -C rustracer_amd/csrc)")
    return _lib


def hip_lib():
    lib()
    return _hip


def device_available() -> bool:
    return bool(hip_lib().rt_device_available())


def _p(a, t=C.c_float):
    return None if a is None else a.ctypes.data_as(C.POINTER(t))


def _check(rc, what):
    if rc < 0:
        msg = lib().rtxh_last_error()
        raise BackendError(f"{what} failed ({rc}): {msg.decode(errors='replace') if msg else '?'}")
    return rc


def look_at(pos, look, up):
    m = np.zeros((4, 4), np.float32)
    mi = np.zeros((4, 4), np.float32)
# ... 95 lines not shown
            w2l = None if l.w2l is None else np.ascontiguousarray(l.w2l, np.float32)
            tri = l.tri if getattr(l, "sphere", -1) < 0 else -2 - l.sphere
            _check(L.rtxh_scene_add_light(self.h, l.kind, tri, _p(np.float32(l.rgb)), int(l.two_sided), _p(np.float32(l.vec)), l.mip, _p(l2w), _p(w2l)), "add_light")
        self.bvh_build_ms = None
        if device_bvh:
            ms = C.c_float()
            _check(L.rtxh_scene_commit_device_bvh(self.h, desc.max_prims_per_node, C.byref(ms)), "commit_device_bvh")
            self.bvh_build_ms = ms.value
        else:
            _check(L.rtxh_scene_commit(self.h, desc.max_prims_per_node), "commit")

    def __del__(self):
        try:
            lib().rtxh_scene_free(self.h)
        except Exception:
            pass

    def bvh(self):
        L = lib()
        nn, npr = C.c_int32(), C.c_int32()
        L.rtxh_scene_bvh_sizes(self.h, C.byref(nn), C.byref(npr))
        bounds = np.zeros((nn.value, 6), np.float32)
        offset = np.zeros(nn.value, np.uint32)
        nprims = np.zeros(nn.value, np.uint16)
        axis = np.zeros(nn.value, np.uint8)
        ordered = np.zeros(npr.value, np.int32)
        L.rtxh_scene_bvh_get(self.h, _p(bounds), _p(offset, C.c_uint32), _p(nprims, C.c_uint16), _p(axis, C.c_uint8), _p(ordered, C.c_int32))
        return dict(bounds=bounds, offset=offset, n_prims=nprims, axis=axis, ordered=ordered)

    def bvh_sizes(self):
        nn, npr = C.c_int32(), C.c_int32()
        lib().rtxh_scene_bvh_sizes(self.h, C.byref(nn), C.byref(npr))
        return nn.value, npr.value

    def link_tables(self, mid=False):
        nn = self.bvh_sizes()[0]
        words = 9 * nn + 9
        kept, full, stats = np.zeros(words, np.uint32), np.zeros(words, np.uint32), np.zeros(27, np.float64)
        _check(lib().rtxh_scene_link_tables(self.h, C.c_int32(1 if mid else 0), _p(kept, C.c_uint32), _p(full, C.c_uint32), C.c_uint64(words), _p(stats, C.c_double)), "rtxh_scene_link_tables")

        def split(t):
            rows = np.concatenate([t[:8 * nn].reshape(8, nn), t[8 * nn + 8:9 * nn + 8].reshape(1, nn)])
            return rows, np.concatenate([t[8 * nn:8 * nn + 8], t[9 * nn + 8:9 * nn + 9]])
        (rk, sk), (rf, sf) = split(kept), split(full)
        return dict(kept=rk, full=rf, start_kept=sk, start_full=sf, rays=stats[:9], tests_all=stats[9:18], tests_kept=stats[18:27])

    def shadow_sets(self):
        nv, st = np.zeros(3, np.int32), np.zeros(2, np.uint64)
        _check(lib().rtxh_scene_shadow_sets(self.h, None, C.c_uint64(0), _p(nv, C.c_int32), _p(st, C.c_uint64)), "rtxh_scene_shadow_sets")
        words = np.zeros(2 * int(np.prod(nv)), np.uint32)
        _check(lib().rtxh_scene_shadow_sets(self.h, _p(words, C.c_uint32), C.c_uint64(words.size), _p(nv, C.c_int32), _p(st, C.c_uint64)), "rtxh_scene_shadow_sets")
        return dict(nvox=tuple(int(x) for x in nv), kind=(words & 3).reshape(int(nv[2]), int(nv[1]), int(nv[0]), 2), pairs=int(st[0]), empty=int(st[1]))

    def scene_query(self, what):
        return _check(lib().rtxh_scene_query(self.h, C.c_int32(what)), "scene_query")

    def lds_resident(self):
        return bool(_check(lib().rtxh_scene_query(self.h, 0), "scene_query"))

    def _render_params(self, **kw):
        return render_params(self.desc, **kw)

    def n_lights(self):
        return len(self.desc.lights)

    def table(self, name):
        return scene_table(self.h, name)

    def setup(self, **kw):
        p = self._render_params(**kw)
        r2c = np.zeros((4, 4), np.float32)
        dxdy = np.zeros(6, np.float32)
        table = np.zeros(256, np.float32)
        sb = np.zeros(4, np.int32)
        cr = np.zeros(4, np.int32)
        _check(lib().rtxh_camera_film_setup(C.byref(p), _p(r2c), _p(dxdy), _p(table), _p(sb, C.c_int32), _p(cr, C.c_int32)), "camera_film_setup")
        return dict(raster_to_camera=r2c, dx_camera=dxdy[:3].copy(), dy_camera=dxdy[3:].copy(), filter_table=table, sample_bounds=sb, cropped=cr, params=p)

    def mip_levels(self, mip):
        L = lib()
        w, h = C.c_int32(), C.c_int32()
        n = _check(L.rtxh_mip_level(self.h, mip, 0, C.byref(w), C.byref(h), None), "mip_level")
        out = []
        for lvl in range(n):
            L.rtxh_mip_level(self.h, mip, lvl, C.byref(w), C.byref(h), None)
            a = np.zeros((h.value, w.value, 3), np.float32)
            L.rtxh_mip_level(self.h, mip, lvl, C.byref(w), C.byref(h), _p(a))
            out.append(a)
        return out

    def upload(self, device=-1):
        _check(lib().rtxh_scene_upload(self.h, device), "upload")

    def render(self, rank=0, world_size=1, count_traversal=False, time_kernels=False, device_out=None, stream=0, count_as_rendered=False, ref_stream=False):
        flags = ((RT_FLAG_COUNT_TRAVERSAL if count_traversal else 0) | (RT_FLAG_TIME_KERNELS if time_kernels else 0) |
                 (RT_FLAG_COUNT_AS_RENDERED if count_as_rendered else 0) | (RT_FLAG_REF_STREAM if ref_stream else 0))
        st = self.setup(rank=rank, world_size=world_size)
        cr = st["cropped"]
        w, h = int(cr[2] - cr[0]), int(cr[3] - cr[1])
        p = st["params"]
        stats = Stats()
        if device_out is not None:
            assert tuple(device_out.shape) == (h, w, 4) and device_out.is_contiguous()
            p.flags = flags | RT_FLAG_FILM_ON_DEVICE
            _check(lib().rtxh_render(self.h, C.byref(p), C.c_void_p(stream), C.c_void_p(device_out.data_ptr()), C.byref(stats)), "render")
            return device_out, stats.as_dict()
# ... 456 lines not shown
```

Before: 2082 Msamples/s.

## Add per-voxel shadow candidate lists to skip BVH walk for shadow rays

```diff
diff --git a/include/rtx_hip.h b/include/rtx_hip.h
--- a/include/rtx_hip.h
+++ b/include/rtx_hip.h
@@ -174,6 +174,7 @@
   uint64_t rays_tail_not_cast;
   uint64_t launches_trace_path, launches_trace_shadow, launches_trace_mis, launches_trace_mis_any, launches_shade;
   uint64_t rays_shadow_not_cast;
+  uint64_t rays_shadow_listed;
 } rt_stats;
 
 #define RT_FLAG_COUNT_TRAVERSAL 1u
@@ -254,10 +255,14 @@
        RT_QUERY_LDS_OCCLUSION = 2 ,
        RT_QUERY_SHADOW_PAIRS = 3 ,
        RT_QUERY_SHADOW_EMPTY = 4 ,
+       RT_QUERY_SHADOW_LISTS = 6 ,
+       RT_QUERY_SHADOW_LISTED = 7 ,
        RT_QUERY_BSDF_LAUNCHED = 5  };
 int rt_scene_query(rt_scene* scene, int32_t what);
 int rt_link_tables(const rt_scene_desc* desc, int32_t mid, uint32_t* link_kept, uint32_t* link_full, uint64_t capacity_words, double* stats);
 int rt_shadow_sets(const rt_scene_desc* desc, uint32_t* words, uint64_t capacity_words, int32_t n_voxels[3], uint64_t* stats);
+int rt_shadow_lists(const rt_scene_desc* desc, int32_t* pair_list, uint64_t capacity_pairs, uint8_t* lists, uint64_t capacity_lists, int32_t n_voxels[3], uint64_t* stats);
+int rt_trace_any_listed(rt_scene* scene, uint64_t n, const float* rays, const uint32_t* words, uint8_t* occluded);
 int rt_sizeof(const char* struct_name);
 
 const char* rt_last_error(void);
diff --git a/include/rtx_host.h b/include/rtx_host.h
--- a/include/rtx_host.h
+++ b/include/rtx_host.h
@@ -101,6 +101,8 @@
 int rtxh_scene_device(rtxh_scene*, rt_scene** out);
 int rtxh_scene_link_tables(rtxh_scene*, int32_t mid, uint32_t* link_kept, uint32_t* link_full, uint64_t capacity_words, double* stats);
 int rtxh_scene_shadow_sets(rtxh_scene*, uint32_t* words, uint64_t capacity_words, int32_t n_voxels[3], uint64_t* stats);
+int rtxh_scene_shadow_lists(rtxh_scene*, int32_t* pair_list, uint64_t capacity_pairs, uint8_t* lists, uint64_t capacity_lists, int32_t n_voxels[3], uint64_t* stats);
+int rtxh_trace_any_listed(rtxh_scene*, uint64_t n, const float* rays, const uint32_t* words, uint8_t* occluded);
 int rtxh_sizeof(const char* struct_name);
 const char* rtxh_last_error(void);
 
diff --git a/rustracer_amd/csrc/rtx_hip.hip b/rustracer_amd/csrc/rtx_hip.hip
--- a/rustracer_amd/csrc/rtx_hip.hip
+++ b/rustracer_amd/csrc/rtx_hip.hip
@@ -86,6 +86,7 @@
   bool masked_emitters = false;
   DevBuf ld_func, ld_cdf, ld_int, ld_mark, ld_list, ld_slot, ld_guide, ld_rows8, ld_dense8;
   bool shadow_sets = false; RtShadowSets shadow; DevBuf ld_shadow;
+  std::vector<uint8_t> prim_leaf; DevBuf sh_lists, sh_prim_leaf; bool lists_uploaded = false;
   DevBuf self;
   int ld_strategy_built = -1; bool ld_all_voxels = false;
   std::mutex render_mutex;
@@ -342,6 +343,31 @@
   return RT_OK;
 }
 
+extern "C" int rt_shadow_lists(const rt_scene_desc* desc, int32_t* pair_list, uint64_t capacity_pairs, uint8_t* lists, uint64_t capacity_lists, int32_t n_voxels[3], uint64_t* stats) {
+  if (!desc || !desc->nodes || desc->n_nodes == 0 || !desc->tri_p || !desc->tri_meta) return fail(RT_ERR_INVALID, "null argument");
+  bool plain = desc->n_instances == 0 && desc->n_spheres == 0 && desc->n_nodes <= RT_SMALL_NODES && desc->n_tris <= RT_SMALL_TRIS;
+  for (uint32_t i = 0; i < desc->n_tris && plain; ++i) if (desc->tri_meta[i].flags & ~(uint32_t)RT_SHADOW_PLAIN_FLAGS) plain = false;
+  if (!shadow_sets_apply(desc, plain)) return fail(RT_ERR_INVALID, "not a scene the shadow sets serve (LDS-resident plain triangles, two triangle lights)");
+  int32_t lp[2] = {0, 0};
+  for (uint32_t k = 0; k < desc->n_lights; ++k) lp[k] = desc->lights[k].prim;
+  RtShadowSets ss; std::vector<uint8_t> prim_leaf;
+  rt_build_shadow_sets(desc->tri_p, desc->n_tris, lp, (int)desc->n_lights, desc->nodes[0].bmin, desc->nodes[0].bmax, ss, shadow_lists_apply(desc, prim_leaf));
+  if (n_voxels) { n_voxels[0] = ss.nvox[0]; n_voxels[1] = ss.nvox[1]; n_voxels[2] = ss.nvox[2]; }
+  if (stats) { stats[0] = ss.pairs; stats[1] = ss.empty; stats[2] = ss.listed; stats[3] = ss.n_lists(); }
+  if (pair_list) {
+    if (capacity_pairs < ss.word.size()) return fail(RT_ERR_INVALID, "rt_shadow_lists: pair capacity too small");
+    for (size_t i = 0; i < ss.word.size(); ++i) {
+      const uint32_t w = ss.word[i], k = RT_SHADOW_KIND(w);
+      pair_list[i] = k == RT_SHADOW_LIST ? (int32_t)(w >> 2) : (k == RT_SHADOW_EMPTY ? -2 : -1);
+    }
+  }
+  if (lists) {
+    if (capacity_lists < ss.n_lists()) return fail(RT_ERR_INVALID, "rt_shadow_lists: list capacity too small");
+    if (!ss.lists.empty()) std::memcpy(lists, ss.lists.data(), ss.lists.size());
+  }
+  return RT_OK;
+}
+
 extern "C" int rt_scene_query(rt_scene* s, int32_t what) {
   if (!s) return fail(RT_ERR_INVALID, "null scene");
   if (what == RT_QUERY_LDS_RESIDENT) return s->small ? 1 : 0;
@@ -349,10 +375,19 @@
   if (what == RT_QUERY_LDS_OCCLUSION) return s->mid ? 1 : 0;
   if (what == RT_QUERY_SHADOW_PAIRS) return s->shadow_sets ? (int)s->shadow.pairs : 0;
   if (what == RT_QUERY_SHADOW_EMPTY) return s->shadow_sets ? (int)s->shadow.empty : 0;
+  if (what == RT_QUERY_SHADOW_LISTS) return s->shadow_sets ? (int)s->shadow.n_lists() : 0;
+  if (what == RT_QUERY_SHADOW_LISTED) return s->shadow_sets ? (int)s->shadow.listed : 0;
   if (what == RT_QUERY_BSDF_LAUNCHED) return s->bsdf_launched < 0 ? 0 : s->bsdf_launched + 1;
   return fail(RT_ERR_INVALID, "unknown rt_scene_query item");
 }
 
+static int shadow_lists_upload(rt_scene* s) {
+  if (s->lists_uploaded || !s->shadow_sets || s->shadow.listed == 0) return RT_OK;
+  int rc = upload(s->sh_lists, s->shadow.lists.data(), s->shadow.lists.size());
+  if (rc == RT_OK) rc = upload(s->sh_prim_leaf, s->prim_leaf.data(), s->prim_leaf.size());
+  if (rc == RT_OK) s->lists_uploaded = true;
+  return rc;
+}
 static int build_light_distribution(rt_scene* s, int strategy, hipStream_t stream, bool all_voxels = false) {
   DScene& d = s->d;
   if (s->ld_strategy_built == strategy && (s->ld_all_voxels || !all_voxels)) return RT_OK;
@@ -439,6 +474,7 @@
   if (d.ld_rows8 != nullptr && !uniform && s->shadow_sets && nl == 2 && d.nvox[0] == s->shadow.nvox[0] && d.nvox[1] == s->shadow.nvox[1] && d.nvox[2] == s->shadow.nvox[2]) {
     const unsigned long long n_vox = (unsigned long long)d.nvox[0] * d.nvox[1] * d.nvox[2];
     int rc = upload(s->ld_shadow, s->shadow.word.data(), s->shadow.word.size() * 4);
+    if (rc == RT_OK) rc = shadow_lists_upload(s);
     if (rc != RT_OK) return rc;
     hipLaunchKernelGGL(k_lightdist_shadow_words, dim3((unsigned)((n_vox + 255) / 256)), dim3(256), 0, stream, s->ld_shadow.as<unsigned>(), s->ld_slot.as<int>(), n_vox, s->ld_rows8.as<float4>(),
                        d.ld_dense8 != nullptr ? s->ld_dense8.as<float4>() : nullptr);
@@ -500,7 +536,7 @@
   s->has_instances = p.has_instances; s->masked_emitters = p.masked_emitters; s->lambert_only = p.lambert_only; s->lambert_materials = p.lambert_materials;
   s->lean_shade = p.lean_shade; s->lean_qlights = p.lean_qlights; s->lds_records = p.lds_records; s->lds_records_q = p.lds_records_q; s->lds_tables = p.lds_tables;
   s->lds_mats = p.lds_mats; s->use_pairs = p.use_pairs; s->use_top = p.use_top; s->top_for_closest = p.top_for_closest; s->use_quads = p.use_quads;
-  s->deep_column = p.deep_column; s->shadow_sets = p.shadow_sets; s->shadow = p.shadow; s->stack_depth = p.stack_depth; s->quad_stack_depth = p.quad_stack_depth;
+  s->deep_column = p.deep_column; s->shadow_sets = p.shadow_sets; s->shadow = p.shadow; s->prim_leaf = p.prim_leaf; s->stack_depth = p.stack_depth; s->quad_stack_depth = p.quad_stack_depth;
   s->mat_kind = p.mat_kind; s->mat_table = p.mat_table; s->mat_class = p.mat_class; s->fourier_at = p.fourier_at;
   s->n_code_classes = p.n_code_classes; s->n_lambert_classes = p.n_lambert_classes; s->n_small_classes = p.n_small_classes; s->n_wide_classes = p.n_wide_classes;
   if (s->mid) {
@@ -735,6 +771,38 @@
   }
   return RT_OK;
 }
+extern "C" int rt_trace_any_listed(rt_scene* s, uint64_t n, const float* rays, const uint32_t* words, uint8_t* occluded) {
+  if (!s || !rays || !words || !occluded || n == 0 || n > 0x7fffffffull) return fail(RT_ERR_INVALID, "bad trace batch");
+  if (!s->small || s->general_prims) return fail(RT_ERR_INVALID, "rt_trace_any_listed: not an LDS-resident scene of plain triangles");
+  const uint64_t n_lists = s->shadow_sets ? s->shadow.n_lists() : 0;
+  for (uint64_t i = 0; i < n; ++i)
+    if (RT_SHADOW_KIND(words[i]) == RT_SHADOW_LIST && (words[i] >> 2) >= n_lists) return fail(RT_ERR_INVALID, "rt_trace_any_listed: a word names a list the scene does not have");
+  HIP_TRY(hipSetDevice(s->device));
+  int rc = shadow_lists_upload(s);
+  if (rc != RT_OK) return rc;
+  DevBuf ro, rd, add, out, st;
+  HIP_TRY(ro.ensure(n * 16)); HIP_TRY(rd.ensure(n * 16)); HIP_TRY(add.ensure(n * 16)); HIP_TRY(out.ensure(n)); HIP_TRY(st.ensure(ST_COUNT * 8));
+  std::vector<float> o(n * 4), d(n * 4), a(n * 4, 0.0f);
+  for (uint64_t i = 0; i < n; ++i) {
+    const float* r = rays + 8 * i;
+    const uint32_t dw = 0x80000000u | (uint32_t)i;
+    o[4 * i] = r[0]; o[4 * i + 1] = r[1]; o[4 * i + 2] = r[2]; o[4 * i + 3] = r[3];
+    d[4 * i] = r[4]; d[4 * i + 1] = r[5]; d[4 * i + 2] = r[6]; std::memcpy(&d[4 * i + 3], &dw, 4);
+    std::memcpy(&a[4 * i + 3], &words[i], 4);
+  }
+  HIP_TRY(hipMemcpy(ro.p, o.data(), n * 16, hipMemcpyHostToDevice));
+  HIP_TRY(hipMemcpy(rd.p, d.data(), n * 16, hipMemcpyHostToDevice));
+  HIP_TRY(hipMemcpy(add.p, a.data(), n * 16, hipMemcpyHostToDevice));
+  HIP_TRY(hipMemset(st.p, 0, ST_COUNT * 8));
+  TraceIO io = trace_io_planar(ro.as<float4>(), rd.as<float4>(), nullptr, out.as<unsigned>());
+  io.occ_stride = 0; io.direct_add = add.as<float4>(); io.add_stride = 1;
+  if (s->lists_uploaded) { io.lists = s->sh_lists.as<unsigned>(); io.prim_leaf = s->sh_prim_leaf.as<unsigned char>(); }
+  launch_trace<true>(s, false, io, nullptr, nullptr, 0, (unsigned)n, st.as<unsigned long long>(), ST_RAYS_SHADOW, ST_NODES_SHADOW, ST_TRIS_SHADOW, nullptr);
+  HIP_TRY(hipGetLastError());
+  HIP_TRY(hipDeviceSynchronize());
+  HIP_TRY(hipMemcpy(occluded, out.p, n, hipMemcpyDeviceToHost));
+  return RT_OK;
+}
 extern "C" int rt_trace_closest(rt_scene* s, const float* rays, uint64_t n, float* hits, uint64_t counters[2]) { return trace_batch(s, rays, n, false, hits, nullptr, counters); }
 extern "C" int rt_trace_any(rt_scene* s, const float* rays, uint64_t n, uint32_t* occluded, uint64_t counters[2]) { return trace_batch(s, rays, n, true, nullptr, occluded, counters); }
 
@@ -1144,6 +1212,7 @@
     io_mis_any = io_mis; io_mis_any.shadow_masks = 0; io_mis_any.hits = nullptr; io_mis_any.occluded = (unsigned*)ps.occ_mi; io_mis_any.occ_stride = 0;
   }
   const bool count = (flags & RT_FLAG_COUNT_TRAVERSAL) != 0;
+  if (!count && s->lists_uploaded && s->lambert_only) { io_shadow.lists = s->sh_lists.as<unsigned>(); io_shadow.prim_leaf = s->sh_prim_leaf.as<unsigned char>(); }
   const unsigned pgrid = (unsigned)s->n_cu * 8u;
   const unsigned sblock = 256u, sgrid = pgrid;
   unsigned long long* dstats = s->stats.as<unsigned long long>();
@@ -1306,7 +1375,7 @@
     if (ovf) { (void)hipMemset(s->sampler_plan.dirty.p, 0, (2 + RT_DIRTY_CAP) * 4); return fail(RT_ERR_INVALID, "sampler retry list overflow"); } }
   stats.camera_rays = h[ST_CAMERA];
   stats.rays_mis_any = h[ST_RAYS_MISANY]; stats.nodes_mis_any = h[ST_NODES_MISANY]; stats.tris_mis_any = h[ST_TRIS_MISANY];
-  stats.rays_closest = h[ST_RAYS_CLOSEST] + h[ST_TAIL_UNCAST]; stats.rays_tail_not_cast = h[ST_TAIL_UNCAST]; stats.rays_shadow = h[ST_RAYS_SHADOW] + h[ST_SHADOW_SETS]; stats.rays_shadow_not_cast = h[ST_SHADOW_SETS]; stats.rays_mis = h[ST_RAYS_MIS] + h[ST_RAYS_MISANY] + h[ST_MIS_UNREACHED];
+  stats.rays_closest = h[ST_RAYS_CLOSEST] + h[ST_TAIL_UNCAST]; stats.rays_tail_not_cast = h[ST_TAIL_UNCAST]; stats.rays_shadow = h[ST_RAYS_SHADOW] + h[ST_SHADOW_SETS]; stats.rays_shadow_not_cast = h[ST_SHADOW_SETS]; stats.rays_shadow_listed = h[ST_SHADOW_LISTED]; stats.rays_mis = h[ST_RAYS_MIS] + h[ST_RAYS_MISANY] + h[ST_MIS_UNREACHED];
   stats.rays_mis_not_cast = h[ST_MIS_UNREACHED];
   stats.nodes_closest = h[ST_NODES_CLOSEST]; stats.nodes_shadow = h[ST_NODES_SHADOW]; stats.nodes_mis = h[ST_NODES_MIS] + h[ST_NODES_MISANY];
   stats.tris_closest = h[ST_TRIS_CLOSEST]; stats.tris_shadow = h[ST_TRIS_SHADOW]; stats.tris_mis = h[ST_TRIS_MIS] + h[ST_TRIS_MISANY];
@@ -1491,7 +1560,7 @@
   dst[i] = make_float4(a.x + b.x, a.y + b.y, a.z + b.z, a.w + b.w);
 }
 static void stats_add(rt_stats& a, const rt_stats& b) {
-  a.camera_rays += b.camera_rays; a.rays_closest += b.rays_closest; a.rays_shadow += b.rays_shadow; a.rays_mis += b.rays_mis; a.rays_mis_not_cast += b.rays_mis_not_cast; a.rays_tail_not_cast += b.rays_tail_not_cast; a.rays_shadow_not_cast += b.rays_shadow_not_cast;
+  a.camera_rays += b.camera_rays; a.rays_closest += b.rays_closest; a.rays_shadow += b.rays_shadow; a.rays_mis += b.rays_mis; a.rays_mis_not_cast += b.rays_mis_not_cast; a.rays_tail_not_cast += b.rays_tail_not_cast; a.rays_shadow_not_cast += b.rays_shadow_not_cast; a.rays_shadow_listed += b.rays_shadow_listed;
   a.nodes_closest += b.nodes_closest; a.nodes_shadow += b.nodes_shadow; a.nodes_mis += b.nodes_mis;
   a.tris_closest += b.tris_closest; a.tris_shadow += b.tris_shadow; a.tris_mis += b.tris_mis; a.paths_scrubbed += b.paths_scrubbed;
   a.ms_total += b.ms_total; a.ms_sampler += b.ms_sampler; a.ms_raygen += b.ms_raygen; a.ms_trace_closest += b.ms_trace_closest; a.ms_trace_any += b.ms_trace_any;
diff --git a/rustracer_amd/csrc/rtx_host.cpp b/rustracer_amd/csrc/rtx_host.cpp
--- a/rustracer_amd/csrc/rtx_host.cpp
+++ b/rustracer_amd/csrc/rtx_host.cpp
@@ -1396,6 +1396,18 @@
   rt_scene_desc d = make_desc(s);
   return rt_shadow_sets(&d, words, capacity_words, n_voxels, stats);
 }
+int rtxh_scene_shadow_lists(rtxh_scene* s, int32_t* pair_list, uint64_t capacity_pairs, uint8_t* lists, uint64_t capacity_lists, int32_t n_voxels[3], uint64_t* stats) {
+  if (!s || !s->committed) return fail(RT_ERR_INVALID, "scene not committed");
+  g_err.clear();
+  rt_scene_desc d = make_desc(s);
+  return rt_shadow_lists(&d, pair_list, capacity_pairs, lists, capacity_lists, n_voxels, stats);
+}
+int rtxh_trace_any_listed(rtxh_scene* s, uint64_t n, const float* rays, const uint32_t* words, uint8_t* occluded) {
+  if (!s) return fail(RT_ERR_INVALID, "null scene");
+  g_err.clear();
+  if (!s->dev) { int rc = rtxh_scene_upload(s, -1); if (rc != RT_OK) return rc; }
+  return rt_trace_any_listed(s->dev, n, rays, words, occluded);
+}
 int rtxh_sizeof(const char* name) {
   if (!name) return -1;
 #define RTXH_SZ(T) if (!strcmp(name, #T)) return (int)sizeof(T);
diff --git a/rustracer_amd/csrc/rtx_kernels.h b/rustracer_amd/csrc/rtx_kernels.h
--- a/rustracer_amd/csrc/rtx_kernels.h
+++ b/rustracer_amd/csrc/rtx_kernels.h
@@ -90,7 +90,9 @@
 #define RT_NQ 4
 #define RT_SHADOW_WALK 0u
 #define RT_SHADOW_EMPTY 1u
+#define RT_SHADOW_LIST 2u
 #define RT_SHADOW_KIND(w) ((w) & 3u)
+#define RT_SHADOW_LIST_LEN 15u
 enum { ST_CAMERA = 0, ST_RAYS_CLOSEST, ST_RAYS_SHADOW, ST_RAYS_MIS, ST_NODES_CLOSEST, ST_NODES_SHADOW, ST_NODES_MIS,
        ST_TRIS_CLOSEST, ST_TRIS_SHADOW, ST_TRIS_MIS, ST_SCRUBBED, ST_UNBUILT_VOXEL,
        ST_RAYS_MISANY, ST_NODES_MISANY, ST_TRIS_MISANY,
@@ -99,6 +101,7 @@
        ST_SHADED,
        ST_STAMP = ST_SHADED + 4,
        ST_SHADOW_SETS = ST_STAMP + 32,
+       ST_SHADOW_LISTED,
        ST_COUNT };
 #ifdef RT_ABLATE
 #define RT_STAMP(k) do { const unsigned long long t_ = clock64(); stamp_acc[k] += t_ - stamp_last; stamp_last = t_; } while (0)
@@ -685,6 +688,35 @@
   }
   return found;
 }
+template <int N, int T>
+RT_DEV bool occluded_list(const float* __restrict__ s_nodes, const float* __restrict__ s_tris, const unsigned* __restrict__ lists, const unsigned char* __restrict__ prim_leaf, const bool active, const unsigned index, const Ray ray) {
+  const unsigned e4 = 4u * (active ? index : 0u);
+  unsigned w = active ? lists[e4] : 0u;
+  const unsigned n = w & 0xffu;
+  const RayPre rp = ray_pre(ray);
+  const float* const tpx = s_tris + rp.kx * T; const float* const tpy = s_tris + rp.ky * T; const float* const tpz = s_tris + rp.kz * T;
+  const f3 op = permute(ray.o, rp.kx, rp.ky, rp.kz);
+  bool found = false;
+  for (unsigned b = 1u; b <= RT_SHADOW_LIST_LEN; ++b) {
+    const bool go = b <= n && !found;
+    if (__ballot(go) == 0ull) break;
+    if ((b & 3u) == 0u && go) w = lists[e4 + (b >> 2)];
+    if (go) {
+      const int t = (int)((w >> ((b & 3u) * 8u)) & 0xffu);
+      TriHit h;
+      const f3 p0t = mk3(tpx[t] - op.x, tpy[t] - op.y, tpz[t] - op.z), p1t = mk3(tpx[3 * T + t] - op.x, tpy[3 * T + t] - op.y, tpz[3 * T + t] - op.z), p2t = mk3(tpx[6 * T + t] - op.x, tpy[6 * T + t] - op.y, tpz[6 * T + t] - op.z);
+      if (tri_test_permuted<RT_ANY_EARLY_SIGN != 0>(p0t, p1t, p2t, rp.sx, rp.sy, rp.sz, ray.t_max, h)) {
+        const float* nd = s_nodes + (int)prim_leaf[t];
+        const float4 n0 = make_float4(nd[0], nd[2 * N], nd[4 * N], nd[N]), n1 = make_float4(nd[3 * N], nd[5 * N], 0.0f, 0.0f);
+        Ray lr = ray;
+        asm volatile("" : "+v"(lr.d.x), "+v"(lr.d.y), "+v"(lr.d.z), "+v"(lr.o.x), "+v"(lr.o.y), "+v"(lr.o.z));
+        const f3 inv_dir = mk3(1.0f / lr.d.x, 1.0f / lr.d.y, 1.0f / lr.d.z);
+        if (slab_test_t<true>(n0, n1, lr, inv_dir, 0, 0, 0)) found = true;
+      }
+    }
+  }
+  return found;
+}
 template <int N, int T, bool FINITE, int LEAF_MIN, int GENERAL = 0, bool TRIS_GLOBAL = false>
 RT_DEV bool closest_small_links(const float* __restrict__ s_nodes, const float* __restrict__ s_tris, const unsigned* __restrict__ link8 , const int row, const int n_nodes, Ray ray, int& prim_out, TriHit& hit_out, const GeneralCtx gen = GeneralCtx{nullptr, false}, const float4* __restrict__ tri_p = nullptr) {
   const f3 inv_dir = mk3(1.0f / ray.d.x, 1.0f / ray.d.y, 1.0f / ray.d.z);
@@ -775,6 +807,7 @@
   float4* lacc; unsigned lacc_stride; SPtr<const float4> direct_add; unsigned add_stride;
   int shadow_masks;
   int queue_is_slots;
+  const unsigned* lists; const unsigned char* prim_leaf;
 };
 template <class AddPtr>
 RT_DEV void trace_write_any(float4* __restrict__ lacc, size_t ls, const AddPtr direct_add, size_t as, unsigned* __restrict__ occluded, size_t os,
@@ -836,15 +869,20 @@
   }
   const unsigned stride = gridDim.x * BLOCK;
   unsigned n_nodes = 0, n_tris = 0, n_rays = 0;
+  constexpr bool LISTS = ANY && !COUNT && GENERAL == 0 && MID == 0 && RT_LDS_LEAF_MIN_ANY == 1;
+  unsigned n_listed = 0;
   auto trace_one = [&](unsigned pid) {
     float4 o4 = ray_o[pid * rs], d4 = ray_d[pid * rs];
+    unsigned pair_word = 0u;
+    if (LISTS) { if (io.lists != nullptr) pair_word = __float_as_uint(direct_add[pid * as].w); }
     Ray ray; ray.o = mk3(o4.x, o4.y, o4.z); ray.d = mk3(d4.x, d4.y, d4.z); ray.t_max = o4.w;
     int prim = -1; TriHit h; h.t = kInf; h.b0 = h.b1 = h.b2 = 0.0f;
     bool found;
     constexpr int LM = ANY ? (MID ? RT_MID_LEAF_MIN_ANY : (GENERAL ? RT_LDS_LEAF_MIN_ANY_GENERAL : RT_LDS_LEAF_MIN_ANY)) : (MID ? RT_MID_LEAF_MIN_CLOSEST : (GENERAL ? RT_LDS_LEAF_MIN_CLOSEST_GENERAL : RT_LDS_LEAF_MIN_CLOSEST));
     const GeneralCtx gen{sc.self, ANY && io.shadow_masks != 0};
     constexpr bool FIN_FORMS = !COUNT;
-    const bool fin = FIN_FORMS && __ballot(!inv_dir_finite(mk3(1.0f / ray.d.x, 1.0f / ray.d.y, 1.0f / ray.d.z))) == 0ull;
+    bool fin = false;
+    if (!(LINKS && LISTS)) fin = FIN_FORMS && __ballot(!inv_dir_finite(mk3(1.0f / ray.d.x, 1.0f / ray.d.y, 1.0f / ray.d.z))) == 0ull;
     if (LINKS) {
       static_assert(!LINKS || ANY || (LM > 1 && LM < 64), "the closest-hit link walk tests its leaves in phases: 1 < LEAF_MIN < 64");
       if (!ANY) {
@@ -853,6 +891,18 @@
       } else if (LM > 1 && LM < 64) {
         found = fin ? occluded_small_links_rounds<NN, NT, true, LM, GENERAL>(s_nodes, s_tris, s_link, (int)sc.n_nodes, (int)s_link[NN], ray, gen)
                     : occluded_small_links_rounds<NN, NT, false, LM, GENERAL>(s_nodes, s_tris, sc.link8_full + 8u * sc.n_nodes + 8u, (int)sc.n_nodes, (int)sc.link8_full[9u * sc.n_nodes + 8u], ray, gen);
+      } else if (LISTS) {
+        const bool d_ok = (fabsf(ray.d.x) >= 0x1p-120f) & (fabsf(ray.d.y) >= 0x1p-120f) & (fabsf(ray.d.z) >= 0x1p-120f);
+        const bool listed = io.lists != nullptr && RT_SHADOW_KIND(pair_word) == RT_SHADOW_LIST && d_ok;
+        const unsigned long long lm = __ballot(listed);
+        found = false;
+        if (lm != 0ull) { found = occluded_list<NN, NT>(s_nodes, s_tris, io.lists, io.prim_leaf, listed, pair_word >> 2, ray); n_listed += (unsigned)__popcll(lm); }
+        if (__ballot(!listed) != 0ull) {
+          fin = __ballot(!inv_dir_finite(mk3(1.0f / ray.d.x, 1.0f / ray.d.y, 1.0f / ray.d.z))) == 0ull;
+          const bool w = fin ? occluded_small_links<NN, NT, true, GENERAL>(s_nodes, s_tris, s_link, (int)sc.n_nodes, listed ? (int)sc.n_nodes : (int)s_link[NN], ray, gen)
+                             : occluded_small_links<NN, NT, false, GENERAL>(s_nodes, s_tris, sc.link8_full + 8u * sc.n_nodes + 8u, (int)sc.n_nodes, listed ? (int)sc.n_nodes : (int)sc.link8_full[9u * sc.n_nodes + 8u], ray, gen);
+          found = listed ? found : w;
+        }
       } else {
         found = fin ? occluded_small_links<NN, NT, true, GENERAL>(s_nodes, s_tris, s_link, (int)sc.n_nodes, (int)s_link[NN], ray, gen)
                     : occluded_small_links<NN, NT, false, GENERAL>(s_nodes, s_tris, sc.link8_full + 8u * sc.n_nodes + 8u, (int)sc.n_nodes, (int)sc.link8_full[9u * sc.n_nodes + 8u], ray, gen);
@@ -872,6 +922,7 @@
     if ((threadIdx.x & 63u) == 0u) {
       if (n_rays) atomicAdd(&stats[st_rays], (unsigned long long)n_rays);
       if (COUNT) { atomicAdd(&stats[st_nodes], (unsigned long long)n_nodes); atomicAdd(&stats[st_tris], (unsigned long long)n_tris); }
+      if (LISTS && n_listed) atomicAdd(&stats[ST_SHADOW_LISTED], (unsigned long long)n_listed);
     }
   }
 }
diff --git a/rustracer_amd/csrc/rtx_scene_plan.h b/rustracer_amd/csrc/rtx_scene_plan.h
--- a/rustracer_amd/csrc/rtx_scene_plan.h
+++ b/rustracer_amd/csrc/rtx_scene_plan.h
@@ -22,6 +22,7 @@
   bool small = false, mid = false, general_prims = false, obj_general = false, has_masks = false, has_spheres = false, has_instances = false, masked_emitters = false;
   bool lambert_only = false, lambert_materials = false, lean_shade = false, lean_qlights = false, lds_records = false, lds_records_q = false, lds_tables = false, lds_mats = false;
   bool use_pairs = false, use_top = false, top_for_closest = false, use_quads = false, deep_column = false, shadow_sets = false;
+  std::vector<uint8_t> prim_leaf;
 };
 
 static int rt_refuse(std::string& why, int code, const std::string& msg) { why = msg; return code; }
@@ -70,6 +71,27 @@
 }
 
 #define RT_SHADOW_PLAIN_FLAGS (RT_TRI_FLIP | RT_TRI_HAS_N | RT_TRI_HAS_UV | RT_TRI_HAS_S)
+static bool shadow_lists_apply(const rt_scene_desc* desc, std::vector<uint8_t>& prim_leaf) {
+  prim_leaf.assign(256, 0);
+  if (desc->n_nodes > 256 || desc->n_tris > 256) return false;
+  std::vector<uint8_t> seen(desc->n_tris, 0);
+  auto inside = [](const rt_bvh_node& c, const rt_bvh_node& n) {
+    for (int k = 0; k < 3; ++k) if (!(c.bmin[k] >= n.bmin[k] && c.bmax[k] <= n.bmax[k])) return false;
+    return true;
+  };
+  for (uint32_t i = 0; i < desc->n_nodes; ++i) {
+    const rt_bvh_node& n = desc->nodes[i];
+    if (n.n_prims != 0) {
+      if ((uint64_t)n.offset + n.n_prims > desc->n_tris) return false;
+      for (uint32_t t = n.offset; t < n.offset + n.n_prims; ++t) { prim_leaf[t] = (uint8_t)i; seen[t] = 1; }
+    } else {
+      if (i + 1 >= desc->n_nodes || n.offset >= desc->n_nodes) return false;
+      if (!inside(desc->nodes[i + 1], n) || !inside(desc->nodes[n.offset], n)) return false;
+    }
+  }
+  for (uint32_t t = 0; t < desc->n_tris; ++t) if (!seen[t]) return false;
+  return true;
+}
 static bool shadow_sets_apply(const rt_scene_desc* desc, bool plain) {
   if (!plain || desc->n_lights != 2 || !desc->lights) return false;
   for (uint32_t k = 0; k < desc->n_lights; ++k) {
@@ -629,8 +651,10 @@
   if (shadow_sets_apply(desc, p.small && !p.general_prims && !p.has_instances) && !(sets && sets[0] == '0')) {
     int32_t lp[2] = {0, 0};
     for (uint32_t k = 0; k < desc->n_lights; ++k) lp[k] = desc->lights[k].prim;
-    rt_build_shadow_sets(desc->tri_p, desc->n_tris, lp, (int)desc->n_lights, desc->nodes[0].bmin, desc->nodes[0].bmax, p.shadow);
-    p.shadow_sets = p.shadow.empty > 0;
+    const char* lists = getenv("RTX_SHADOW_LISTS");
+    const bool want_lists = !(lists && lists[0] == '0') && shadow_lists_apply(desc, p.prim_leaf);
+    rt_build_shadow_sets(desc->tri_p, desc->n_tris, lp, (int)desc->n_lights, desc->nodes[0].bmin, desc->nodes[0].bmax, p.shadow, want_lists);
+    p.shadow_sets = p.shadow.empty > 0 || p.shadow.listed > 0;
   }
   if (p.small || p.deep_column) return RT_OK;
   const uint32_t n_pair_nodes = n_top_nodes;
diff --git a/rustracer_amd/csrc/rtx_shade_kernels.h b/rustracer_amd/csrc/rtx_shade_kernels.h
--- a/rustracer_amd/csrc/rtx_shade_kernels.h
+++ b/rustracer_amd/csrc/rtx_shade_kernels.h
@@ -393,7 +393,8 @@
           else if (rows8) d1_sample_discrete_row8(ld_r0, ld_r1, sc.n_lights, su, light_num, light_pdf);
           else if (MODE != 1 && sc.ld_glog >= 0) d1_sample_discrete_guided(ld_func, ld_cdf, ld_int, sc.n_lights, su, sc.ld_guide + ld_row * ((1 << sc.ld_glog) + 1), sc.ld_glog, light_num, light_pdf);
           else d1_sample_discrete(ld_func, ld_cdf, ld_int, sc.n_lights, su, light_num, light_pdf);
-          const bool ld_empty = MODE == 1 && ps.shadow_sets && RT_SHADOW_KIND(__float_as_uint(light_num == 0 ? ld_r0.w : ld_r1.w)) == RT_SHADOW_EMPTY;
+          const unsigned ld_word = (MODE == 1 && ps.shadow_sets) ? __float_as_uint(light_num == 0 ? ld_r0.w : ld_r1.w) : 0u;
+          const bool ld_empty = MODE == 1 && RT_SHADOW_KIND(ld_word) == RT_SHADOW_EMPTY;
           RT_STAMP(3);
           if (light_pdf != 0.0f) {
             f2 u_light = smp.get_2d();
@@ -457,10 +458,11 @@
               mi_c[i] = make_float4(beta.r, beta.g, beta.b, spdf2);
               mi_flags[i] = (want_shadow ? RT_PEND_SHADOW : 0u) | 2u | ((unsigned)light_num << 2) | (mis_occlusion_only ? RT_PEND_MIS_ANY : 0u);
               if (!want_shadow || no_walk) ps.occ_sh[i] = no_walk ? (unsigned char)0 : (unsigned char)1;
+              else if (MODE == 1 && ps.shadow_sets) reinterpret_cast<unsigned*>(sraw(ps.sh.add) + i)[3] = ld_word;
             } else if (want_shadow) {
               rgb3 add = beta * vdiv(mkc(0, 0, 0) + ld1, light_pdf);
               if (no_walk) { const float4 l4 = ps.lacc[pid]; ps.lacc[pid] = make_float4(l4.x + add.r, l4.y + add.g, l4.z + add.b, l4.w); }
-              else sh_add[i] = make_float4(add.r, add.g, add.b, 0.0f);
+              else sh_add[i] = make_float4(add.r, add.g, add.b, __uint_as_float(ld_word));
             }
             if (want_shadow && !no_walk) sh_d[i] = make_float4(sh_dir.x, sh_dir.y, sh_dir.z, __uint_as_float((want_mis ? 0u : 0x80000000u) | pid));
             want_shadow = want_shadow && !no_walk;
diff --git a/rustracer_amd/csrc/rtx_shadow_sets.h b/rustracer_amd/csrc/rtx_shadow_sets.h
--- a/rustracer_amd/csrc/rtx_shadow_sets.h
+++ b/rustracer_amd/csrc/rtx_shadow_sets.h
@@ -2,6 +2,8 @@
 #include <algorithm>
 #include <cmath>
 #include <cstdint>
+#include <cstring>
+#include <map>
 #include <vector>
 
 
@@ -10,7 +12,11 @@
   int n_lights = 0;
   std::vector<uint32_t> word;
   uint64_t pairs = 0, empty = 0;
+  std::vector<uint8_t> lists;
+  uint64_t listed = 0;
+  size_t n_lists() const { return lists.size() / 16; }
 };
+#define RT_SHADOW_LIST_MAX 15
 
 namespace rtss {
 struct D3 { double x, y, z; };
@@ -34,14 +40,17 @@
   }
 }
 
-static void rt_build_shadow_sets(const float* tri_p, uint32_t n_tris, const int32_t* light_prims, int n_lights, const float wb_min[3], const float wb_max[3], RtShadowSets& out) {
+static void rt_build_shadow_sets(const float* tri_p, uint32_t n_tris, const int32_t* light_prims, int n_lights, const float wb_min[3], const float wb_max[3], RtShadowSets& out, bool want_lists = false) {
   using namespace rtss;
   rt_shadow_grid(wb_min, wb_max, out.nvox);
   out.n_lights = n_lights;
   const int nx = out.nvox[0], ny = out.nvox[1], nz = out.nvox[2];
   const size_t total = (size_t)nx * ny * nz;
   out.word.assign(total * 2, RT_SHADOW_WALK);
-  out.pairs = out.empty = 0;
+  out.pairs = out.empty = out.listed = 0; out.lists.clear();
+  if (n_tris > 256) want_lists = false;
+  std::map<std::vector<uint8_t>, uint32_t> list_index;
+  std::vector<uint8_t> cand;
   if (n_lights != 2 || n_tris == 0) return;
   const D3 wmin{wb_min[0], wb_min[1], wb_min[2]}, wmax{wb_max[0], wb_max[1], wb_max[2]};
   const D3 ext = sub(wmax, wmin);
@@ -142,9 +151,19 @@
             }
             return false;
           };
-          bool empty = true;
-          for (uint32_t t = 0; t < n_tris && empty; ++t) if (!behind(t) && !separated(t)) empty = false;
-          if (empty) { out.word[2 * v + l] = RT_SHADOW_EMPTY; out.empty += 1; }
+          cand.clear(); size_t n_cand = 0;
+          for (uint32_t t = 0; t < n_tris && (want_lists || n_cand == 0); ++t)
+            if (!behind(t) && !separated(t)) { n_cand += 1; if (n_cand <= RT_SHADOW_LIST_MAX) cand.push_back((uint8_t)t); }
+          if (n_cand == 0) { out.word[2 * v + l] = RT_SHADOW_EMPTY; out.empty += 1; }
+          else if (want_lists && n_cand <= RT_SHADOW_LIST_MAX) {
+            auto it = list_index.find(cand);
+            if (it == list_index.end()) {
+              it = list_index.emplace(cand, (uint32_t)out.n_lists()).first;
+              uint8_t e[16] = {0}; e[0] = (uint8_t)n_cand; std::memcpy(e + 1, cand.data(), n_cand);
+              out.lists.insert(out.lists.end(), e, e + 16);
+            }
+            out.word[2 * v + l] = RT_SHADOW_LIST | (it->second << 2); out.listed += 1;
+          }
         }
       }
 }
diff --git a/rustracer_amd/host.py b/rustracer_amd/host.py
--- a/rustracer_amd/host.py
+++ b/rustracer_amd/host.py
@@ -80,7 +80,7 @@
         [(n, C.c_double) for n in ("ms_shade_lambert_const", "ms_shade_lambert", "ms_shade_two_lobe", "ms_shade_generic", "ms_shade_bin", "ms_shade_miss")] +
         [("shade_section_cycles", C.c_uint64 * 32)] +
         [(n, C.c_uint64) for n in ("rays_mis_any", "nodes_mis_any", "tris_mis_any")] + [("ms_trace_mis_any", C.c_double), ("ms_gather", C.c_double), ("rays_mis_not_cast", C.c_uint64), ("rays_tail_not_cast", C.c_uint64)] +
-        [(n, C.c_uint64) for n in ("launches_trace_path", "launches_trace_shadow", "launches_trace_mis", "launches_trace_mis_any", "launches_shade", "rays_shadow_not_cast")])
+        [(n, C.c_uint64) for n in ("launches_trace_path", "launches_trace_shadow", "launches_trace_mis", "launches_trace_mis_any", "launches_shade", "rays_shadow_not_cast", "rays_shadow_listed")])
 
     def as_dict(self):
         return {n: (list(getattr(self, n)) if n == "shade_section_cycles" else getattr(self, n)) for n, _ in self._fields_}
@@ -282,6 +282,25 @@
         _check(lib().rtxh_scene_shadow_sets(self.h, _p(words, C.c_uint32), C.c_uint64(words.size), _p(nv, C.c_int32), _p(st, C.c_uint64)), "rtxh_scene_shadow_sets")
         return dict(nvox=tuple(int(x) for x in nv), kind=(words & 3).reshape(int(nv[2]), int(nv[1]), int(nv[0]), 2), pairs=int(st[0]), empty=int(st[1]))
 
+    def shadow_lists(self):
+        nv, st = np.zeros(3, np.int32), np.zeros(4, np.uint64)
+        _check(lib().rtxh_scene_shadow_lists(self.h, None, C.c_uint64(0), None, C.c_uint64(0), _p(nv, C.c_int32), _p(st, C.c_uint64)), "rtxh_scene_shadow_lists")
+        index = np.zeros(2 * int(np.prod(nv)), np.int32)
+        lists = np.zeros((max(int(st[3]), 1), 16), np.uint8)
+        _check(lib().rtxh_scene_shadow_lists(self.h, _p(index, C.c_int32), C.c_uint64(index.size), _p(lists, C.c_uint8), C.c_uint64(lists.shape[0]), _p(nv, C.c_int32), _p(st, C.c_uint64)),
+               "rtxh_scene_shadow_lists")
+        return dict(nvox=tuple(int(x) for x in nv), index=index.reshape(int(nv[2]), int(nv[1]), int(nv[0]), 2), lists=lists[:int(st[3])], pairs=int(st[0]), empty=int(st[1]),
+                    listed=int(st[2]))
+
+    def trace_any_listed(self, rays, words):
+        rays = np.ascontiguousarray(rays, np.float32)
+        words = np.ascontiguousarray(words, np.uint32)
+        n = rays.shape[0]
+        assert words.shape == (n,)
+        occ = np.zeros(n, np.uint8)
+        _check(lib().rtxh_trace_any_listed(self.h, C.c_uint64(n), _p(rays), _p(words, C.c_uint32), _p(occ, C.c_uint8)), "trace_any_listed")
+        return occ > 0
+
     def scene_query(self, what):
         return _check(lib().rtxh_scene_query(self.h, C.c_int32(what)), "scene_query")
 
```

Result: no change. 2097 Msamples/s, median of 6 (+0.8%).
